# NJUVISION/PCGCv2

Hardware: AMD Instinct MI355X
Metric: encode+decode Mpoints/sec at fixed bpp (r3 ckpt), vox10 frame (higher is better)
Workload: dtype f32

## Files before the change

### include/pcgc_hip.h

```cpp
#ifndef PCGC_HIP_H
#define PCGC_HIP_H

#include <stddef.h>
#include <stdint.h>

#ifdef __cplusplus
extern "C" {
#endif

const char* pcgc_last_error(void);
int pcgc_version(void);

int64_t pcgc_hash_capacity(int64_t n);
int pcgc_hash_clear(uint64_t* keys , int32_t* vals , int64_t cap, void* stream);
int pcgc_hash_insert(const int32_t* coords , int64_t n, int32_t stride, uint64_t* keys, int32_t* vals,
                     int64_t cap, void* stream);
int pcgc_hash_insert_policy(const int32_t* coords, int64_t n, int32_t stride, uint64_t* keys, int32_t* vals, int64_t cap,
                            int keep_last, void* stream);
int pcgc_hash_first_mask(const int32_t* coords, int64_t n, int32_t stride, const uint64_t* keys, const int32_t* vals,
                         int64_t cap, uint8_t* keep , int32_t* first_row , void* stream);

int pcgc_coords_check_order(const int32_t* coords , int64_t n, int32_t* out2 , void* stream);

int pcgc_coords_quantize(const int32_t* coords, int64_t n, int32_t stride_out, int32_t* out , void* stream);
// ... 17 lines not shown
int pcgc_kmap_k3_prune(const int32_t* cand_nbr , int64_t n_cand, const uint8_t* mask, const int32_t* prefix,
                       const int32_t* orig , int64_t n_out, int32_t* nbr , void* stream);
int pcgc_kmap_k3_prune_parent(const int32_t* parent_nbr , int64_t n_parent, const uint8_t* mask,
                              const int32_t* prefix, const int32_t* orig, int64_t n_out, int32_t* nbr , void* stream);
int pcgc_kmap_k3_from_coarse(const int32_t* fine , int64_t n_fine, int32_t stride_fine,
                             const int32_t* parent_of , const int32_t* coarse_nbr ,
                             const int32_t* down , int64_t n_coarse, int32_t* nbr ,
                             void* stream);
int pcgc_down_maps(const int32_t* fine, const int32_t* first_row, const int32_t* prefix, int64_t n_fine, int32_t stride_fine,
                   int64_t n_coarse, int32_t* parent_of , int32_t* down , void* stream);
int pcgc_down_prepare(const int32_t* fine , int64_t n, int32_t stride_fine, int32_t* q ,
                      uint64_t* keys, int32_t* vals, int64_t cap, uint8_t* keep , int32_t* first_row ,
                      int32_t* prefix , int32_t* total , void* scan_ws, size_t scan_ws_bytes, void* stream);
int pcgc_down_finish(const int32_t* fine, const int32_t* q, const uint8_t* keep, const int32_t* first_row, const int32_t* prefix,
                     int64_t n, int32_t stride_fine, int64_t n_coarse, int32_t* coarse ,
                     int32_t* parent_of , int32_t* down , void* stream);
int pcgc_down_level(const int32_t* fine , int64_t n, int32_t stride_fine, int32_t* q, uint64_t* keys, int32_t* vals,
                    int64_t cap, uint8_t* keep, int32_t* first_row, int32_t* prefix, int32_t* total, void* scan_ws,
                    size_t scan_ws_bytes, int32_t* coarse , int32_t* parent_of ,
                    int32_t* down , int64_t* n_coarse_out , void* stream);
size_t pcgc_pyramid_scratch_bytes(int64_t n, int levels);
int pcgc_pyramid(const int32_t* fine , int64_t n, int32_t stride, int levels, void* scratch, size_t scratch_bytes,
                 int32_t* const* coarse, int32_t* const* parent_of, int32_t* const* down, int64_t* counts , void* stream);
int pcgc_compact_index(const uint8_t* mask, const int32_t* prefix, int64_t n, int32_t* orig , void* stream);

int pcgc_conv_gather(const int32_t* nbr, int K, int64_t n_out, const float* in, int64_t n_in , int Cin,
                     int in_ld, int in_coff, const float* W, const float* bias, const float* residual, int res_ld,
                     int res_coff, int relu, float* out, int Cout, int out_ld, int out_coff, void* stream);
int pcgc_last_conv_impl(void);
int pcgc_conv_gather_unit(const int32_t* nbr , int K, int64_t n_out, const float* W, const float* bias, int relu,
                          float* out, int Cout, int out_ld, void* stream);
int pcgc_conv_unit_from_coarse(const int32_t* fine , int64_t n_fine, int32_t stride_fine, const int32_t* parent_of,
                               const int32_t* coarse_nbr , const int32_t* down , int64_t n_coarse,
                               const float* W , const float* bias, int relu, float* out, int Cout, int out_ld, void* stream);
int pcgc_set_conv_impl(int impl);
int pcgc_set_up2_impl(int mfma);
int pcgc_irn_block(const int32_t* nbr , int64_t n, const float* x , int C, int x_ld,
                   const float* const* params, float* t_scratch, float* out, int out_ld, void* stream);
int pcgc_irn_pass(const int32_t* nbr, int64_t n, const float* x, int C, int x_ld, const float* const* params,
                  float* t_scratch, float* out, int out_ld, int pass, void* stream);
int pcgc_conv_up2(int64_t n_in, const float* in, int Cin, int in_ld, const float* W , const float* bias,
                  int relu, float* out , int Cout, void* stream);
int pcgc_conv_up2_gather(int64_t n_in, const float* in, int Cin, int in_ld, const int32_t* rows, const float* W ,
                         const float* bias, int relu, float* out , int Cout, void* stream);

int pcgc_conv_child(const int32_t* parent_nbr , int64_t n_parent, const float* in ,
                    int Cin, int in_ld, const float* table , int64_t table_bytes,
                    const float* bias, const float* residual, int res_ld, int relu, float* out, int Cout, int out_ld, void* stream);
int pcgc_irn_child_pass(const int32_t* parent_nbr, int64_t n_parent, int C, int pass, const float* in, int in_ld,
                        const float* table, int64_t table_bytes, const float* b0, const float* b1, const float* b2,
                        const float* x, int x_ld, float* out, int out_ld, void* stream);
int pcgc_irn_child_q4(const int32_t* parent_nbr, int64_t n_parent, int C, int pass, const float* in, int in_ld,
                      const float* table, int64_t table_bytes, const float* b0, const float* b1, const float* b2,
                      const float* x, int x_ld, float* out, int out_ld, void* stream);
int pcgc_cls_child_q4(const int32_t* parent_nbr, int64_t n_parent, const float* in, int Cin, int in_ld, const float* table,
                      int64_t table_bytes, const float* bias, float* out, void* stream);
int pcgc_irn_rows_pass(const int32_t* nbr, int64_t n, int C, int pass, const float* in, int in_ld, const float* table,
                       int64_t table_bytes, const float* b0, const float* b1, const float* b2, const float* x, int x_ld, float* out,
                       int out_ld, void* stream);
int pcgc_irn_rows_q4_pass(const int32_t* nbr, int64_t n, int C, int pass, const float* in, int in_ld, const float* table,
                          int64_t table_bytes, const float* b0, const float* b1, const float* b2, const float* x, int x_ld, float* out,
                          int out_ld, void* stream);
int pcgc_set_rows_q4_variant(int v);
int pcgc_conv_rows(const int32_t* nbr, int64_t n, const float* in, int Cin, int in_ld, const float* table, int64_t table_bytes,
                   const float* bias, const float* residual, int res_ld, int relu, float* out, int Cout, int out_ld, void* stream);
int pcgc_conv_down_rows(const int32_t* down, int64_t n_coarse, const float* in, int64_t n_in, int Cin, int in_ld, const float* table,
                        int64_t table_bytes, const float* bias, int relu, float* out, int Cout, int out_ld, void* stream);

int pcgc_conv_packed64(const int32_t* nbr, int64_t n, const float* in, int in_ld, const float* table, int64_t table_bytes,
                       const float* bias, int relu, float* out, int out_ld, void* stream);
int pcgc_set_packed_tuning(int rows, int waves);

int pcgc_set_convention(int what, int value);

size_t pcgc_topk_workspace_bytes(int64_t n);
int pcgc_topk_mask(const float* logits , int ld, int64_t n, int64_t k, uint8_t* mask ,
                   void* workspace, size_t workspace_bytes, void* stream);
int pcgc_topk_mask_segments(const float* logits, int ld, int nseg, const int64_t* seg_rows, const int64_t* seg_k, uint8_t* mask,
                            void* workspace, size_t workspace_bytes, void* stream);
size_t pcgc_topk_select_workspace_bytes(int64_t n);
int pcgc_topk_select(const float* logits , int ld, int nseg, const int64_t* seg_rows, const int64_t* seg_k,
                     const int32_t* coords, const int32_t* parent_coords, int32_t parent_stride,
                     uint8_t* bits, int32_t* wprefix, int32_t* orig, int32_t* out_coords, void* workspace, size_t workspace_bytes, void* stream);
int pcgc_kmap_k3_prune_sel(const int32_t* cand_nbr , int64_t n_cand, const uint8_t* bits, const int32_t* wprefix,
                           const int32_t* orig , int64_t n_out, int32_t* nbr , void* stream);
int pcgc_kmap_k3_prune_parent_sel(const int32_t* parent_nbr , int64_t n_parent, const uint8_t* bits, const int32_t* wprefix,
                                  const int32_t* orig, int64_t n_out, int32_t* nbr , void* stream);
int pcgc_gather_rows_f32_ld(const float* in, int C, int in_ld, const int32_t* orig, int64_t n_out, float* out , void* stream);
int pcgc_batch_counts(const int32_t* coords , int64_t n, int32_t* counts , void* stream);

size_t pcgc_sort_workspace_bytes(int64_t n);
int pcgc_sort_zyx(const int32_t* coords, int64_t n, int32_t* perm , void* workspace, size_t workspace_bytes,
                  void* stream);
int pcgc_sort_bzyx(const int32_t* coords, int64_t n, int32_t* perm , void* workspace, size_t workspace_bytes, void* stream);
int pcgc_gather_rows_i32x4(const int32_t* in, const int32_t* perm, int64_t n, int32_t* out, void* stream);
int pcgc_gather_rows_f32(const float* in, int C, const int32_t* perm, int64_t n, float* out, void* stream);

int pcgc_relu(const float* in, int64_t count, float* out, void* stream);
int pcgc_add(const float* a, const float* b, int64_t count, float* out, void* stream);

int pcgc_round_minmax(const float* feats, int64_t count, float* minmax , void* stream);
int pcgc_symbolize(const float* feats, int64_t count, float min_v, int16_t* sym , void* stream);
int pcgc_desymbolize(const int16_t* sym, int64_t count, float min_v, float* feats, void* stream);
int pcgc_quantize_symbols(const float* feats, int64_t count, float* minmax , int16_t* sym , void* stream);
int pcgc_quantize_symbols_segments(const float* feats, int C, int nseg, const int64_t* seg_rows, float* minmax, int16_t* sym, void* stream);
int pcgc_cdf_table(const float* params , int C, float min_v, float max_v, uint16_t* cdf_u16 ,
                   float* cdf_f32 , void* stream);


size_t pcgc_loss_workspace_bytes(int64_t elements);
int pcgc_hash_contains(const int32_t* coords , int64_t n, const uint64_t* keys, const int32_t* vals, int64_t cap,
                       const uint8_t* or_mask , uint8_t* mask , void* stream);
int pcgc_eb_likelihood(const float* feats, int ld, int64_t n, int C, const float* params , float bound, float* likelihood,
                       double* bits, void* workspace, size_t workspace_bytes, void* stream);
int pcgc_neg_log2_sum(const float* x, int ld, int64_t n, int C, double* bits , void* workspace, size_t workspace_bytes, void* stream);
int pcgc_bce_logits(const float* logits, int64_t ld, int64_t n, const uint8_t* truth , const uint8_t* pred ,
                    double* bce, int64_t* counts, void* workspace, size_t workspace_bytes, void* stream);

size_t pcgc_conv_wgrad_workspace_bytes(int K, int64_t n_rows, int Cin, int Cout);
int64_t pcgc_conv_wgrad_rows_per_group(int K, int64_t n_rows, int Cin, int Cout);
int pcgc_conv_wgrad(const int32_t* nbr, int K, int64_t n_out, const float* x, int64_t n_in, int Cin, int x_ld, const float* gy, int Cout,
                    int gy_ld, float* gW, float* gb, void* workspace, size_t workspace_bytes, void* stream);
int pcgc_conv_up2_wgrad(int64_t n_in, const float* x, int64_t x_rows, int Cin, int x_ld, const int32_t* rows, const float* gy, int Cout,
                        int gy_ld, float* gW, float* gb, void* workspace, size_t workspace_bytes, void* stream);
int pcgc_kmap_invert(const int32_t* nbr, int K, int64_t n_out, int64_t n_in, int32_t* inv , void* stream);
int pcgc_relu_bwd(const float* g, int g_ld, const float* y, int y_ld, int64_t n, int C, float* out, int out_ld, void* stream);
int pcgc_scatter_rows(const float* gy, int C, int gy_ld, const int32_t* orig, int64_t n_rows, float* gx, int64_t n_out, int gx_ld, void* stream);
int pcgc_bce_logits_bwd(const float* logits, int64_t ld, int64_t n, const uint8_t* truth, double scale, float* g , void* stream);
size_t pcgc_eb_bwd_workspace_bytes(int64_t n, int C);
int pcgc_eb_likelihood_bwd(const float* feats, int ld, int64_t n, int C, const float* params , float bound, double scale,
                           float* gy, float* gparams, void* workspace, size_t workspace_bytes, void* stream);

int64_t pcgc_rc_encode(const uint16_t* cdf , int C, int Lp, const int16_t* sym , int64_t n,
                       uint8_t* out , int64_t cap);
int pcgc_rc_decode(const uint16_t* cdf, int C, int Lp, const uint8_t* in, int64_t nbytes, int16_t* sym, int64_t n);
#define PCGC_RC_CKPT_WORDS 6
int64_t pcgc_rc_encode_indexed(const uint16_t* cdf, int C, int Lp, const int16_t* sym, int64_t n, uint8_t* out, int64_t cap, int n_ckpt,
                               uint32_t* ckpt );
int pcgc_rc_decode_indexed(const uint16_t* cdf, int C, int Lp, const uint8_t* in, int64_t nbytes, int16_t* sym, int64_t n, int n_ckpt,
                           const uint32_t* ckpt);
int pcgc_set_rc_threads(int threads);
int pcgc_set_rc_lanes(int mode);
int pcgc_set_rc_impl(int impl);

int64_t pcgc_oct_encode(const int32_t* xyz , int64_t n, uint8_t* out, int64_t cap);
int64_t pcgc_oct_decode_count(const uint8_t* in, int64_t nbytes);
int pcgc_oct_decode(const uint8_t* in, int64_t nbytes, int32_t* xyz , int64_t n);
int pcgc_set_oct_tiled(int on);
int pcgc_set_oct_model(int model);
int pcgc_oct_warm(void);

int pcgc_d1_nn(const int32_t* a , int64_t na, const uint64_t* b_keys, const int32_t* b_vals, int64_t b_cap,
               const int32_t* offsets , int n_offsets, double* sum , uint64_t* max_d2 ,
               int32_t* unresolved , void* stream);
int pcgc_d1_cell_masks(const int32_t* b , int64_t nb, const uint64_t* cell_keys, const int32_t* cell_vals, int64_t cell_cap,
                       uint64_t* masks , int64_t n_cells, void* stream);
int pcgc_d1_nn_cells(const int32_t* a , int64_t na, const uint64_t* cell_keys, const int32_t* cell_vals, int64_t cell_cap,
                     const uint64_t* masks, const int32_t* offsets , int n_offsets, int32_t reach2, double* sum, uint64_t* max_d2,
                     int32_t* unresolved, void* stream);

int pcgc_d2_runs(const int32_t* qs , int64_t nq, int32_t* runlen , void* stream);
int pcgc_d2_count(const int32_t* p , int64_t n, const int32_t* sel, const uint64_t* cell_keys, const int32_t* cell_vals,
                  int64_t cell_cap, const uint64_t* masks, const uint64_t* keys, const int32_t* vals, int64_t cap, const int32_t* runlen,
                  const int32_t* offsets , int n_offsets, int32_t reach2, int64_t* best , int32_t* cnt ,
                  int32_t* unresolved , int32_t* n_unresolved , void* stream);
int pcgc_d2_fill(const int32_t* p, int64_t n, const int32_t* sel, const uint64_t* cell_keys, const int32_t* cell_vals, int64_t cell_cap,
// ... 90 lines not shown
```

### pcgcv2_amd/_build.py

```python
import os
import subprocess
import sys
from concurrent.futures import ThreadPoolExecutor

HERE = os.path.dirname(os.path.abspath(__file__))
CSRC = os.path.join(HERE, 'csrc')
VARIANT = os.environ.get('PCGC_BUILD_VARIANT', '')
OBJ = os.path.join(CSRC, '_obj' + ('_' + VARIANT if VARIANT else ''))
LIB = os.path.join(HERE, 'libpcgc_hip' + ('_' + VARIANT if VARIANT else '') + '.so')
SOURCES = ['coords.hip', 'select.hip', 'conv.hip', 'child_conv.hip', 'child_conv32.hip', 'child_cls_w.hip', 'child_irn.hip', 'child_irn_a16.hip', 'child_irn_b16.hip',
           'child_irn_a32.hip', 'child_irn_b32.hip', 'child_q4.hip', 'rows_irn.hip', 'rows_q4.hip', 'conv_packed.hip', 'entropy.hip', 'loss.hip', 'grad.hip', 'metric.hip', 'colour.hip', 'normals.hip', 'mesh.hip', 'collate.hip', 'hostcodec.cpp', 'ply.cpp', 'mesh_io.cpp']
HEADERS = [os.path.join(CSRC, 'pcgc_common.h'), os.path.join(CSRC, 'mfma_util.h'), os.path.join(CSRC, 'child_kernels.h'), os.path.join(CSRC, 'child_q4.h'), os.path.join(CSRC, 'q4x.h'), os.path.join(CSRC, 'q4x_sched.h'), os.path.join(CSRC, 'rows_q4_policy.h'), os.path.join(CSRC, 'eb_logits.h'), os.path.join(HERE, '..', 'include', 'pcgc_hip.h')]
FLAGS = ['--offload-arch=gfx950', '-O3', '-std=c++17', '-ffp-contract=off', '-fPIC', '-Wall', '-Wno-unused-result'] + \
        os.environ.get('PCGC_EXTRA_HIPCC_FLAGS', '').split()


def _hipcc():
    for c in (os.environ.get('HIPCC'), '/opt/rocm/bin/hipcc', 'hipcc'):
        if c and (os.path.isabs(c) and os.path.exists(c) or not os.path.isabs(c)):
            return c
    return 'hipcc'


def _stale(target, deps):
    if not os.path.exists(target):
        return True
    t = os.path.getmtime(target)
    return any(os.path.getmtime(d) > t for d in deps)


def build(force=False, verbose=False):
    os.makedirs(OBJ, exist_ok=True)
    if VARIANT:
        import shutil
        base = os.path.join(CSRC, '_obj')
        for src in SOURCES:
            o = src.rsplit('.', 1)[0] + '.o'
            if 'child_kernels.h' not in open(os.path.join(CSRC, src)).read() and os.path.exists(os.path.join(base, o)) \
                    and not os.path.exists(os.path.join(OBJ, o)):
                shutil.copy2(os.path.join(base, o), os.path.join(OBJ, o))
    hipcc = _hipcc()
    jobs = []
    only = [t for t in os.environ.get('PCGC_BUILD_ONLY', '').split(',') if t]
    for src in SOURCES:
        s = os.path.join(CSRC, src)
        o = os.path.join(OBJ, src.rsplit('.', 1)[0] + '.o')
        if only and os.path.exists(o):
            if src.rsplit('.', 1)[0] in only:
                jobs.append((o, [hipcc] + FLAGS + (['-x', 'hip'] if src.endswith('.hip') else []) + ['-c', s, '-o', o]))
            continue
        if force or _stale(o, [s] + HEADERS):
            lang = ['-x', 'hip'] if src.endswith('.hip') else []
            jobs.append((o, [hipcc] + FLAGS + lang + ['-c', s, '-o', o]))

    def run(job):
        o, cmd = job
        if verbose:
            print(' '.join(cmd), file=sys.stderr)
        r = subprocess.run(cmd, capture_output=True, text=True)
        if r.returncode != 0:
            raise RuntimeError('hipcc failed:\n' + ' '.join(cmd) + '\n' + r.stderr[-4000:])
        return o

    with ThreadPoolExecutor(max_workers=max(2, min(8, os.cpu_count() or 4))) as ex:
        list(ex.map(run, jobs))
    objs = [os.path.join(OBJ, s.rsplit('.', 1)[0] + '.o') for s in SOURCES]
    if force or jobs or _stale(LIB, objs):
        cmd = [hipcc, '--offload-arch=gfx950', '-shared', '-fPIC', '-o', LIB] + objs + ['-lz']
        r = subprocess.run(cmd, capture_output=True, text=True)
        if r.returncode != 0:
            raise RuntimeError('link failed:\n' + r.stderr[-4000:])
    if not VARIANT:
        build_reftable(force=force)
    return LIB


REFTABLE_LIB = os.path.join(HERE, 'libpcgc_reftable.so')


def build_reftable(force=False):
    src = os.path.join(CSRC, 'reftable.cpp')
    if not (force or _stale(REFTABLE_LIB, [src])):
        return REFTABLE_LIB
    import torch
    tdir = os.path.dirname(torch.__file__)
    cmd = ['g++', '-O2', '-std=c++17', '-fPIC', '-shared', f'-D_GLIBCXX_USE_CXX11_ABI={int(torch._C._GLIBCXX_USE_CXX11_ABI)}',
           '-I' + os.path.join(tdir, 'include'), '-I' + os.path.join(tdir, 'include', 'torch', 'csrc', 'api', 'include'), src,
           '-o', REFTABLE_LIB, '-L' + os.path.join(tdir, 'lib'), '-ltorch_cpu', '-lc10', '-Wl,-rpath,' + os.path.join(tdir, 'lib')]
    r = subprocess.run(cmd, capture_output=True, text=True)
    if r.returncode != 0:
        raise RuntimeError('g++ failed:\n' + ' '.join(cmd) + '\n' + r.stderr[-4000:])
    return REFTABLE_LIB


if __name__ == '__main__':
# ... 2 lines not shown
```

### pcgcv2_amd/_lib.py

```python
import ctypes as C
import os

_HERE = os.path.dirname(os.path.abspath(__file__))
LIB_PATH = os.environ.get('PCGC_LIB') or os.path.join(_HERE, 'libpcgc_hip.so')

vp, i64, i32, f32, sz = C.c_void_p, C.c_int64, C.c_int32, C.c_float, C.c_size_t
ci = C.c_int

SIGNATURES = {
    'pcgc_last_error': (C.c_char_p, []),
    'pcgc_version': (ci, []),
    'pcgc_hash_capacity': (i64, [i64]),
    'pcgc_hash_clear': (ci, [vp, vp, i64, vp]),
    'pcgc_hash_insert': (ci, [vp, i64, i32, vp, vp, i64, vp]),
    'pcgc_hash_insert_policy': (ci, [vp, i64, i32, vp, vp, i64, ci, vp]),
    'pcgc_set_convention': (ci, [ci, ci]),
    'pcgc_hash_first_mask': (ci, [vp, i64, i32, vp, vp, i64, vp, vp, vp]),
    'pcgc_coords_check_order': (ci, [vp, i64, vp, vp]),
    'pcgc_coords_quantize': (ci, [vp, i64, i32, vp, vp]),
    'pcgc_coords_children': (ci, [vp, i64, i32, vp, vp]),
    'pcgc_coords_scale': (ci, [vp, i64, f32, vp, vp]),
    'pcgc_scan_workspace_bytes': (sz, [i64]),
    'pcgc_mask_scan': (ci, [vp, i64, vp, vp, vp, sz, vp]),
    'pcgc_mask_scan_zeroed': (ci, [vp, i64, vp, vp, vp, sz, vp]),
    'pcgc_compact_coords': (ci, [vp, vp, vp, i64, vp, vp]),
    'pcgc_compact_feats': (ci, [vp, ci, ci, vp, vp, i64, vp, vp]),
    'pcgc_kmap_k3': (ci, [vp, i64, i32, vp, vp, i64, vp, vp]),
    'pcgc_kmap_k3_children': (ci, [vp, i64, vp, vp]),
    'pcgc_kmap_k3_prune': (ci, [vp, i64, vp, vp, vp, i64, vp, vp]),
    'pcgc_kmap_k3_prune_parent': (ci, [vp, i64, vp, vp, vp, i64, vp, vp]),
    'pcgc_kmap_k3_from_coarse': (ci, [vp, i64, i32, vp, vp, vp, i64, vp, vp]),
    'pcgc_down_maps': (ci, [vp, vp, vp, i64, i32, i64, vp, vp, vp]),
    'pcgc_down_prepare': (ci, [vp, i64, i32, vp, vp, vp, i64, vp, vp, vp, vp, vp, sz, vp]),
    'pcgc_down_finish': (ci, [vp, vp, vp, vp, vp, i64, i32, i64, vp, vp, vp, vp]),
    'pcgc_down_level': (ci, [vp, i64, i32, vp, vp, vp, i64, vp, vp, vp, vp, vp, sz, vp, vp, vp, vp, vp]),
    'pcgc_pyramid_scratch_bytes': (sz, [i64, ci]),
    'pcgc_pyramid': (ci, [vp, i64, i32, ci, vp, sz, vp, vp, vp, vp, vp]),
    'pcgc_compact_index': (ci, [vp, vp, i64, vp, vp]),
    'pcgc_conv_gather': (ci, [vp, ci, i64, vp, i64, ci, ci, ci, vp, vp, vp, ci, ci, ci, vp, ci, ci, ci, vp]),
    'pcgc_conv_gather_unit': (ci, [vp, ci, i64, vp, vp, ci, vp, ci, ci, vp]),
    'pcgc_conv_unit_from_coarse': (ci, [vp, i64, i32, vp, vp, vp, i64, vp, vp, ci, vp, ci, ci, vp]),
    'pcgc_set_conv_impl': (ci, [ci]),
    'pcgc_last_conv_impl': (ci, []),
    'pcgc_set_up2_impl': (ci, [ci]),
    'pcgc_irn_block': (ci, [vp, i64, vp, ci, ci, vp, vp, vp, ci, vp]),
    'pcgc_irn_pass': (ci, [vp, i64, vp, ci, ci, vp, vp, vp, ci, ci, vp]),
    'pcgc_conv_child': (ci, [vp, i64, vp, ci, ci, vp, i64, vp, vp, ci, ci, vp, ci, ci, vp]),
    'pcgc_irn_child_pass': (ci, [vp, i64, ci, ci, vp, ci, vp, i64, vp, vp, vp, vp, ci, vp, ci, vp]),
    'pcgc_irn_child_q4': (ci, [vp, i64, ci, ci, vp, ci, vp, i64, vp, vp, vp, vp, ci, vp, ci, vp]),
    'pcgc_cls_child_q4': (ci, [vp, i64, vp, ci, ci, vp, i64, vp, vp, vp]),
    'pcgc_conv_down_rows': (ci, [vp, i64, vp, i64, ci, ci, vp, i64, vp, ci, vp, ci, ci, vp]),
    'pcgc_conv_rows': (ci, [vp, i64, vp, ci, ci, vp, i64, vp, vp, ci, ci, vp, ci, ci, vp]),
    'pcgc_irn_rows_pass': (ci, [vp, i64, ci, ci, vp, ci, vp, i64, vp, vp, vp, vp, ci, vp, ci, vp]),
    'pcgc_irn_rows_q4_pass': (ci, [vp, i64, ci, ci, vp, ci, vp, i64, vp, vp, vp, vp, ci, vp, ci, vp]),
    'pcgc_set_rows_q4_variant': (ci, [ci]),
    'pcgc_conv_packed64': (ci, [vp, i64, vp, ci, vp, i64, vp, ci, vp, ci, vp]),
    'pcgc_set_packed_tuning': (ci, [ci, ci]),
    'pcgc_conv_up2': (ci, [i64, vp, ci, ci, vp, vp, ci, vp, ci, vp]),
    'pcgc_conv_up2_gather': (ci, [i64, vp, ci, ci, vp, vp, vp, ci, vp, ci, vp]),
    'pcgc_topk_workspace_bytes': (sz, [i64]),
    'pcgc_topk_mask': (ci, [vp, ci, i64, i64, vp, vp, sz, vp]),
    'pcgc_topk_mask_segments': (ci, [vp, ci, ci, vp, vp, vp, vp, sz, vp]),
    'pcgc_topk_select_workspace_bytes': (sz, [i64]),
    'pcgc_topk_select': (ci, [vp, ci, ci, vp, vp, vp, vp, i32, vp, vp, vp, vp, vp, sz, vp]),
    'pcgc_kmap_k3_prune_sel': (ci, [vp, i64, vp, vp, vp, i64, vp, vp]),
    'pcgc_kmap_k3_prune_parent_sel': (ci, [vp, i64, vp, vp, vp, i64, vp, vp]),
    'pcgc_gather_rows_f32_ld': (ci, [vp, ci, ci, vp, i64, vp, vp]),
    'pcgc_batch_counts': (ci, [vp, i64, vp, vp]),
    'pcgc_sort_bzyx': (ci, [vp, i64, vp, vp, sz, vp]),
    'pcgc_quantize_symbols_segments': (ci, [vp, ci, ci, vp, vp, vp, vp]),
    'pcgc_sort_workspace_bytes': (sz, [i64]),
    'pcgc_sort_zyx': (ci, [vp, i64, vp, vp, sz, vp]),
    'pcgc_gather_rows_i32x4': (ci, [vp, vp, i64, vp, vp]),
    'pcgc_gather_rows_f32': (ci, [vp, ci, vp, i64, vp, vp]),
    'pcgc_relu': (ci, [vp, i64, vp, vp]),
    'pcgc_add': (ci, [vp, vp, i64, vp, vp]),
    'pcgc_round_minmax': (ci, [vp, i64, vp, vp]),
    'pcgc_symbolize': (ci, [vp, i64, f32, vp, vp]),
    'pcgc_desymbolize': (ci, [vp, i64, f32, vp, vp]),
    'pcgc_quantize_symbols': (ci, [vp, i64, vp, vp, vp]),
    'pcgc_cdf_table': (ci, [vp, ci, f32, f32, vp, vp, vp]),
    'pcgc_loss_workspace_bytes': (sz, [i64]),
    'pcgc_hash_contains': (ci, [vp, i64, vp, vp, i64, vp, vp, vp]),
    'pcgc_eb_likelihood': (ci, [vp, ci, i64, ci, vp, f32, vp, vp, vp, sz, vp]),
    'pcgc_neg_log2_sum': (ci, [vp, ci, i64, ci, vp, vp, sz, vp]),
    'pcgc_bce_logits': (ci, [vp, i64, i64, vp, vp, vp, vp, vp, sz, vp]),
    'pcgc_conv_wgrad_workspace_bytes': (sz, [ci, i64, ci, ci]),
    'pcgc_conv_wgrad_rows_per_group': (i64, [ci, i64, ci, ci]),
    'pcgc_conv_wgrad': (ci, [vp, ci, i64, vp, i64, ci, ci, vp, ci, ci, vp, vp, vp, sz, vp]),
    'pcgc_conv_up2_wgrad': (ci, [i64, vp, i64, ci, ci, vp, vp, ci, ci, vp, vp, vp, sz, vp]),
    'pcgc_kmap_invert': (ci, [vp, ci, i64, i64, vp, vp]),
    'pcgc_relu_bwd': (ci, [vp, ci, vp, ci, i64, ci, vp, ci, vp]),
    'pcgc_scatter_rows': (ci, [vp, ci, ci, vp, i64, vp, i64, ci, vp]),
    'pcgc_bce_logits_bwd': (ci, [vp, i64, i64, vp, C.c_double, vp, vp]),
    'pcgc_eb_bwd_workspace_bytes': (sz, [i64, ci]),
    'pcgc_eb_likelihood_bwd': (ci, [vp, ci, i64, ci, vp, f32, C.c_double, vp, vp, vp, sz, vp]),
    'pcgc_d1_cell_masks': (ci, [vp, i64, vp, vp, i64, vp, i64, vp]),
    'pcgc_d1_nn_cells': (ci, [vp, i64, vp, vp, i64, vp, vp, ci, i32, vp, vp, vp, vp]),
    'pcgc_d1_nn': (ci, [vp, i64, vp, vp, i64, vp, ci, vp, vp, vp, vp]),
    'pcgc_d2_runs': (ci, [vp, i64, vp, vp]),
    'pcgc_d2_count': (ci, [vp, i64, vp, vp, vp, i64, vp, vp, vp, i64, vp, vp, ci, i32, vp, vp, vp, vp, vp]),
    'pcgc_d2_fill': (ci, [vp, i64, vp, vp, vp, i64, vp, vp, vp, i64, vp, vp, vp, ci, i32, vp, vp, vp, vp]),
    'pcgc_d2_exhaustive': (ci, [vp, i64, vp, vp, i64, vp, ci, vp, vp, vp, vp, vp, vp]),
    'pcgc_d2_scan_workspace_bytes': (sz, [i64]),
    'pcgc_d2_scan': (ci, [vp, i64, vp, vp, sz, vp]),
    'pcgc_d2_segment_lowest': (ci, [vp, i64, vp, i32, vp, vp]),
    'pcgc_d2_recv_count': (ci, [vp, vp, i64, vp, i64, vp, vp]),
    'pcgc_d2_recv_fill': (ci, [vp, vp, i64, vp, i64, vp, vp, vp, vp]),
    'pcgc_d2_normals': (ci, [vp, vp, i64, vp, vp, vp, vp, vp, vp]),
    'pcgc_d2_c2p': (ci, [vp, i64, vp, vp, vp, vp, vp, vp, vp]),
    'pcgc_d2_reduce_workspace_bytes': (sz, []),
    'pcgc_d2_reduce': (ci, [vp, vp, i64, vp, vp, vp, sz, vp]),
    'pcgc_attr_transfer_workspace_bytes': (sz, [i64, i64, ci]),
    'pcgc_attr_transfer': (ci, [vp, vp, vp, i64, vp, vp, vp, i64, vp, ci, vp, vp, sz, vp]),
    'pcgc_colour_dist': (ci, [vp, i64, vp, i64, vp, vp, vp, vp, vp, vp]),
    'pcgc_colour_reduce_workspace_bytes': (sz, []),
    'pcgc_colour_reduce': (ci, [vp, vp, i64, vp, vp, sz, vp]),
    'pcgc_normals_ball_masks': (i64, [i32, vp]),
    'pcgc_normals_workspace_bytes': (sz, [i64]),
    'pcgc_normals_estimate': (ci, [vp, i64, vp, vp, vp, vp, i64, vp, vp, vp, i64, vp, vp, i32, ci, vp, vp, vp, vp, vp, vp, vp, sz, vp]),
    'pcgc_set_normals_mapping': (ci, [ci]),
    'pcgc_rc_encode': (i64, [vp, ci, ci, vp, i64, vp, i64]),
    'pcgc_rc_decode': (ci, [vp, ci, ci, vp, i64, vp, i64]),
    'pcgc_set_rc_impl': (ci, [ci]),
    'pcgc_rc_encode_indexed': (i64, [vp, ci, ci, vp, i64, vp, i64, ci, vp]),
    'pcgc_rc_decode_indexed': (ci, [vp, ci, ci, vp, i64, vp, i64, ci, vp]),
    'pcgc_set_rc_threads': (ci, [ci]),
    'pcgc_set_rc_lanes': (ci, [ci]),
    'pcgc_set_oct_tiled': (ci, [ci]),
    'pcgc_set_oct_model': (ci, [ci]),
    'pcgc_oct_warm': (ci, []),
    'pcgc_oct_encode': (i64, [vp, i64, vp, i64]),
    'pcgc_oct_decode_count': (i64, [vp, i64]),
    'pcgc_oct_decode': (ci, [vp, i64, vp, i64]),
    'pcgc_items_encode': (ci, [ci, vp, vp, vp, vp, vp, ci, vp, vp, vp, ci, ci, ci]),
    'pcgc_items_probe': (ci, [ci, vp, vp, vp, vp, vp, vp]),
    'pcgc_items_decode': (ci, [ci, vp, vp, ci, vp, vp, vp, vp, ci, vp, vp, ci, ci, ci]),
    'pcgc_level_prepare_children': (ci, [vp, i64, i32, vp, vp, i64, vp, vp, vp, vp]),
    'pcgc_frame_decode': (ci, [C.c_char_p, ci, vp, vp, ci, ci, i64, vp, vp, vp, vp, ci]),
    'pcgc_frame_decode_begin': (ci, [C.c_char_p, ci, vp, vp, ci, ci, i64, vp, vp, vp, vp, ci]),
    'pcgc_frame_decode_end': (ci, []),
    'pcgc_frame_worker_test': (ci, [ci]),
    'pcgc_table_cache': (ci, [ci]),
    'pcgc_crc32': (C.c_uint32, [C.c_uint32, vp, i64]),
    'pcgc_ply_read_ascii_geo': (i64, [C.c_char_p, vp, i64]),
    'pcgc_ply_write_ascii_geo': (ci, [C.c_char_p, vp, i64]),
    'pcgc_ply_write_ascii_geo_rgb': (ci, [C.c_char_p, vp, vp, i64]),
# ... 58 lines not shown
```

### pcgcv2_amd/autoencoder.py

```python
import torch

from . import dispatch, ops
from .nn import MinkowskiConvolution as Conv, MinkowskiGenerativeConvolutionTranspose as UpConv, MinkowskiPruning
from .sparse import CoordMap, SparseTensor


class InceptionResNet(torch.nn.Module):

    def __init__(self, channels):
        super().__init__()
        c = channels
        self.conv0_0 = Conv(c, c // 4, 3)
        self.conv0_1 = Conv(c // 4, c // 2, 3)
        self.conv1_0 = Conv(c, c // 4, 1)
        self.conv1_1 = Conv(c // 4, c // 4, 3)
        self.conv1_2 = Conv(c // 4, c // 2, 1)

    def forward(self, x):
        c = x.F.shape[1]
        children = x.cmap.origin is not None and x.cmap.origin[0] == 'children'
        fam = dispatch.select('irn', (c,), x.F.shape[0], 'children' if children else 'plain', extent=x.F.shape[0] * max(c, x.F.stride(0)) * 4,
                              contiguous=x.F.is_contiguous()).family
        if fam != 'unfused':
            params = [p for m in (self.conv0_0, self.conv0_1, self.conv1_0, self.conv1_1, self.conv1_2) for p in (m.kernel, m.bias)]
            if fam == 'rows64':
                y = ops.irn_block_rows64(x.cmap.k3, x.F, params, self._tables('child', ops.child_irn_tables, params))
            elif fam == 'child':
                big = x.F.shape[0] >= 8 * ops.PATH.CHILD_Q4_MIN_PARENTS
                q4 = self._tables('q4', ops.child_q4_tables, params) if (c == 16 and ops.PATH.CHILD_Q4 and big) else None
                y = ops.irn_block_child(x.cmap.origin[1].k3, x.F, params, self._tables('child', ops.child_irn_tables, params), q4_table=q4)
            elif fam == 'rows32q4':
                y = ops.irn_block_rows32_q4(x.cmap.k3, x.F, params, self._tables('rows_q4', ops.rows_q4_tables, params))
            elif fam == 'rows32':
                y = ops.irn_block_rows32(x.cmap.k3, x.F, params, self._tables('rows32', ops.rows_irn32_tables, params))
            else:
                y = ops.irn_block(x.cmap.k3, x.F, params)
            return SparseTensor(y, coordinate_map=x.cmap)
        out = torch.empty_like(x.F)
        a = self.conv0_0(x, relu=True)
        self.conv0_1(a, out=out[:, :c // 2], residual=x.F[:, :c // 2])
        b = self.conv1_1(self.conv1_0(x, relu=True), relu=True)
        self.conv1_2(b, out=out[:, c // 2:], residual=x.F[:, c // 2:])
        return SparseTensor(out, coordinate_map=x.cmap)

    def _tables(self, kind, build, params):
        stamp = tuple((p.data_ptr(), p._version) for p in params)
        cache = self.__dict__.setdefault('_derived', {})
        if cache.get(kind, (None, None))[0] != stamp:
            cache[kind] = (stamp, build(params))
        return cache[kind][1]


def make_layer(block, block_layers, channels):
    return torch.nn.Sequential(*[block(channels=channels) for _ in range(block_layers)])


class Encoder(torch.nn.Module):

    def __init__(self, channels=[1, 16, 32, 64, 32, 8]):
        super().__init__()
        ch = channels
        self.conv0 = Conv(ch[0], ch[1], 3)
        self.down0 = Conv(ch[1], ch[2], 2, 2)
        self.block0 = make_layer(InceptionResNet, 3, ch[2])
        self.conv1 = Conv(ch[2], ch[2], 3)
        self.down1 = Conv(ch[2], ch[3], 2, 2)
        self.block1 = make_layer(InceptionResNet, 3, ch[3])
        self.conv2 = Conv(ch[3], ch[3], 3)
        self.down2 = Conv(ch[3], ch[4], 2, 2)
        self.block2 = make_layer(InceptionResNet, 3, ch[4])
        self.conv3 = Conv(ch[4], ch[5], 3)

    def forward(self, x):
        out0 = self.block0(self.down0(self.conv0(x, relu=True), relu=True))
        out1 = self.block1(self.down1(self.conv1(out0, relu=True), relu=True))
        out2 = self.block2(self.down2(self.conv2(out1, relu=True), relu=True))
        out2 = self.conv3(out2)
        return [out2, out1, out0]


class Decoder(torch.nn.Module):

    def __init__(self, channels=[8, 64, 32, 16]):
        super().__init__()
        ch = channels
        for l in range(3):
            setattr(self, f'up{l}', UpConv(ch[l], ch[l + 1], 2, 2))
            setattr(self, f'conv{l}', Conv(ch[l + 1], ch[l + 1], 3))
            setattr(self, f'block{l}', make_layer(InceptionResNet, 3, ch[l + 1]))
            setattr(self, f'conv{l}_cls', Conv(ch[l + 1], 1, 3))
        self.pruning = MinkowskiPruning()

    def prune_voxel(self, data, data_cls, nums, ground_truth=None, training=False):
        if training:
            return self._prune_voxel_training(data, data_cls, nums, ground_truth)
        cand = data.cmap
        rows = [len(data_cls)] if len(nums) == 1 else cand.batch_rows
        if len(rows) != len(nums):
            raise ValueError(f'prune_voxel: {len(nums)} budgets for a batch of {len(rows)} items')
        keep = [int(min(r, max(int(n), 0))) for r, n in zip(rows, nums)]
        if dispatch.select('prune', (data.F.shape[1],), len(data_cls)).family != 'select':
            mask = ops.topk_mask(data_cls.F, keep[0]) if len(nums) == 1 else ops.topk_mask_segments(data_cls.F, rows, keep)
            return self.pruning(data, mask, n_keep=sum(keep), keep_per_item=None if len(nums) == 1 else keep)
        if cand._C is None and cand.origin is not None and cand.origin[0] == 'children':
            parent = cand.origin[1]
            bits, wprefix, orig, coords = ops.topk_select(data_cls.F, rows, keep, parent_coords=parent.C, parent_stride=parent.stride)
        else:
            bits, wprefix, orig, coords = ops.topk_select(data_cls.F, rows, keep, coords=cand.C)
        cmap = CoordMap(coords, cand.stride, unique=True, origin=('selected', cand, bits, wprefix, orig))
        if len(nums) > 1:
            cmap._batch_rows = list(keep)
        src = data.F
        out = SparseTensor(lambda: ops.gather_rows(src, orig), coordinate_map=cmap)
        out._F_rows = (src, orig)
        return out

    def _prune_voxel_training(self, data, data_cls, nums, ground_truth):
        if ground_truth is None:
            raise ValueError('prune_voxel(training=True) needs the ground truth of the level')
        from .data_utils import isin_mask
        cand = data.cmap
        rows = [len(data_cls)] if len(nums) == 1 else cand.batch_rows
        if len(rows) != len(nums):
            raise ValueError(f'prune_voxel: {len(nums)} budgets for a batch of {len(rows)} items')
        keep = [int(min(r, max(int(n), 0))) for r, n in zip(rows, nums)]
        topk = ops.topk_mask(data_cls.F, keep[0]) if len(nums) == 1 else ops.topk_mask_segments(data_cls.F, rows, keep)
        mask = isin_mask(cand.C, ground_truth, or_mask=topk)
        return self.pruning(data, mask)

    def forward(self, x, nums_list, ground_truth_list=(None, None, None), training=False):
        out, cls_list = x, []
        for l in range(3):
            out = getattr(self, f'up{l}')(out, relu=True)
            out = getattr(self, f'conv{l}')(out, relu=True)
            out = getattr(self, f'block{l}')(out)
            cls = getattr(self, f'conv{l}_cls')(out)
            cls_list.append(cls)
            out = self.prune_voxel(out, cls, nums_list[l], ground_truth_list[l], training)
        return cls_list, out
```

### pcgcv2_amd/csrc/child_cls_w.hip

```cpp
#include "child_kernels.h"

#define DEF_CONV_LAUNCH(NAME) int NAME(const int32_t* parent_nbr, int64_t n_parent, const float* in, int in_ld, const float* table, \
                                       int table_bytes, const ChildEpi& ep, hipStream_t s)
DEF_CONV_LAUNCH(pcgc_child_cls32) { return launch_child_cls<2, 16, 4>(parent_nbr, n_parent, in, in_ld, table, table_bytes, ep, s); }
DEF_CONV_LAUNCH(pcgc_child_cls64) { return launch_child_cls<4, 7, 4>(parent_nbr, n_parent, in, in_ld, table, table_bytes, ep, s); }
CHILD_TIMING_READER(pcgc_child_timing_cls_w)
```

### pcgcv2_amd/csrc/child_conv.hip

```cpp
#include "child_kernels.h"


#define DECL_CONV_LAUNCH(NAME) int NAME(const int32_t* parent_nbr, int64_t n_parent, const float* in, int in_ld, const float* table, \
                                        int table_bytes, const ChildEpi& ep, hipStream_t s)
DECL_CONV_LAUNCH(pcgc_child_conv32); DECL_CONV_LAUNCH(pcgc_child_cls32); DECL_CONV_LAUNCH(pcgc_child_cls64);


extern "C" int pcgc_conv_child(const int32_t* parent_nbr, int64_t n_parent, const float* in, int Cin, int in_ld,
                               const float* table, int64_t table_bytes, const float* bias,
                               const float* residual, int res_ld, int relu, float* out, int Cout, int out_ld, void* stream) {
    CHILD_COMMON_CHECKS(in_ld)
    PCGC_REQUIRE(out != nullptr, "null output");
    PCGC_REQUIRE(Cout == 1 || ((out_ld & 3) == 0 && (((uintptr_t)out) & 15) == 0), "output rows must be 16-byte aligned");
    PCGC_REQUIRE(residual == nullptr, "conv_child: no residual form");
    (void)res_ld;
    hipStream_t s = S(stream);
    int rc = -2;
    const int tb = (int)table_bytes;
    if (Cout == 1 && (Cin == 16 || Cin == 32 || Cin == 64)) {
        PCGC_REQUIRE(table_bytes == (int64_t)(125 * ((Cin / 16) * 64 + 16) + 1023) / 1024 * 1024, "cls table size");
        PCGC_REQUIRE(residual == nullptr && !relu, "cls head has no fused epilogue");
        ChildEpi ep{bias, nullptr, 0, 0, out, out_ld, 0};
        if (Cin == 64) rc = pcgc_child_cls64(parent_nbr, n_parent, in, in_ld, table, tb, ep, s);
        else if (Cin == 16) rc = launch_child_cls<1, 8, 4>(parent_nbr, n_parent, in, in_ld, table, tb, ep, s);
        else rc = pcgc_child_cls32(parent_nbr, n_parent, in, in_ld, table, tb, ep, s);
    } else {
        PCGC_REQUIRE(table_bytes == (int64_t)27 * Cin * Cout * 4, "table size");
        ChildEpi ep{bias, nullptr, 0, relu, out, out_ld, Cout / 16};
        if (Cin == 16 && Cout == 16) {
            rc = launch_child_conv<1, 1, 4, 4>(parent_nbr, n_parent, in, in_ld, table, tb, ep, s);
        } else if (Cin == 32 && Cout == 32) {
            rc = pcgc_child_conv32(parent_nbr, n_parent, in, in_ld, table, tb, ep, s);
        } else {
            pcgc_set_error("conv_child: unsupported shape %d -> %d (16->16, 32->32, 16->1, 32->1, 64->1)", Cin, Cout);
            return -2;
        }
    }
    if (rc) return rc;
    PCGC_CHECK_LAUNCH("conv_child");
    return 0;
}


#ifdef PCGC_CHILD_TIMING
extern "C" int pcgc_child_timing(unsigned long long* out8, int reset) {
    hipDeviceSynchronize();
    if (out8) hipMemcpyFromSymbol(out8, HIP_SYMBOL(g_child_dbg), 8 * sizeof(unsigned long long));
    if (reset) { unsigned long long z[8] = {0}; hipMemcpyToSymbol(HIP_SYMBOL(g_child_dbg), z, sizeof(z)); }
    return 0;
}
#endif
```

### pcgcv2_amd/csrc/child_kernels.h

```cpp
#pragma once
#include "pcgc_common.h"
#include "mfma_util.h"
#include <type_traits>

#ifdef PCGC_CHILD_TIMING
static __device__ unsigned long long g_child_dbg[8];
#define CHILD_T(var) const unsigned long long var = __builtin_amdgcn_s_memtime()
#define CHILD_TADD(slot, a, b) do { child_dbg[slot] += (b) - (a); } while (0)
#define CHILD_DBG_DECL unsigned long long child_dbg[8] = {0, 0, 0, 0, 0, 0, 0, 0};
#define CHILD_DBG_PARAM , unsigned long long (&child_dbg)[8]
#define CHILD_DBG_ARG , child_dbg
#define CHILD_TFLUSH do { if ((threadIdx.x & 63) == 0) { for (int q_ = 0; q_ < 8; ++q_) if (child_dbg[q_]) atomicAdd(&g_child_dbg[q_], child_dbg[q_]); } } while (0)
#define CHILD_TIMING_READER(NAME)                                                                                      \
    extern "C" int NAME(unsigned long long* out8, int reset) {                                                         \
        (void)hipDeviceSynchronize();                                                                                  \
        if (out8) (void)hipMemcpyFromSymbol(out8, HIP_SYMBOL(g_child_dbg), 8 * sizeof(unsigned long long));           \
        if (reset) { unsigned long long z[8] = {0}; (void)hipMemcpyToSymbol(HIP_SYMBOL(g_child_dbg), z, sizeof(z)); }  \
        return 0;                                                                                                      \
    }
#else
#define CHILD_T(var)
#define CHILD_TADD(slot, a, b)
#define CHILD_DBG_DECL
#define CHILD_DBG_PARAM
#define CHILD_DBG_ARG
#define CHILD_TFLUSH
#define CHILD_TIMING_READER(NAME)
#endif

struct ChildEpi {
    const float* bias;
    const float* res;
    int res_ld;
    int relu;
    float* out;
    int out_ld;
    int nt;
};
struct IrnEpi {
    const float* b0;
    const float* b1;
    const float* b2;
    const float* x;
    int x_ld;
    float* out;
    int out_ld;
};
namespace {


constexpr int halo_p1(int c) { return c == 0 ? 0 : (c == 3 ? 2 : 1); }
constexpr int halo_bit(int c) { return (c == 0 || c == 2) ? 1 : 0; }
constexpr int cell_kp(int c) { return halo_p1(c >> 4) * 9 + halo_p1((c >> 2) & 3) * 3 + halo_p1(c & 3); }
constexpr int cell_child(int c) { return halo_bit(c & 3) + 2 * halo_bit((c >> 2) & 3) + 4 * halo_bit(c >> 4); }
constexpr bool axis_reach(int c, int jb) { return c - jb >= 0 && c - jb <= 2; }
constexpr unsigned cell_reach(int c) {
    unsigned m = 0;
    for (int j = 0; j < 8; ++j)
        if (axis_reach(c & 3, j & 1) && axis_reach((c >> 2) & 3, (j >> 1) & 1) && axis_reach(c >> 4, j >> 2)) m |= 1u << j;
    return m;
}
constexpr int cell_k(int c, int j) {
    return ((c >> 4) - (j >> 2)) * 9 + (((c >> 2) & 3) - ((j >> 1) & 1)) * 3 + ((c & 3) - (j & 1));
}
constexpr int cz_of(int c) { return c >> 4; }
constexpr int cy_of(int c) { return (c >> 2) & 3; }
constexpr int cx_of(int c) { return c & 3; }
constexpr bool in02(int v) { return v >= 0 && v <= 2; }

struct HaloGeometry {
    static constexpr int NCELLS = 64, ROW_MUL = 8, NMAP = 27;
    static constexpr int kp(int c) { return cell_kp(c); }
    static constexpr int child(int c) { return cell_child(c); }
    static constexpr int byte_off(int) { return 0; }
};

template <int NB_, int NT, int HZ = -1>
struct PlainConv : HaloGeometry {
    static constexpr int NB = NB_, ROWCHUNKS = 4, T = 8 * NT, KS = 4;
    static constexpr int Z_HALF = HZ;
    static constexpr bool HALF = false;
    static constexpr int kfirst(int) { return 0; }
    static constexpr bool active(int c, int t) { return (HZ < 0 || (((t / NT) >> 2) & 1) == HZ) && ((cell_reach(c) >> (t / NT)) & 1); }
    static constexpr int frag(int c, int t) { return cell_k(c, t / NT) * NT + t % NT; }
    static constexpr bool uses_block(int, int) { return true; }
// ... 366 lines not shown
        if (res) {
            const float4 x = *(const float4*)(res + row * res_ld + 4 * c4);
            v.x = v.x + x.x; v.y = v.y + x.y; v.z = v.z + x.z; v.w = v.w + x.w;
        }
        if (relu) { v.x = fmaxf(v.x, 0.0f); v.y = fmaxf(v.y, 0.0f); v.z = fmaxf(v.z, 0.0f); v.w = fmaxf(v.w, 0.0f); }
        *(float4*)(out + row * out_ld + 4 * c4) = v;
    }
}

#define CHILD_IN_ROWS(V, n_p) (V::ROW_MUL * (n_p))
#define CHILD_KERNEL_PROLOGUE(V, NW, D, RING_FLOAT4)                                                                          \
    CHILD_DBG_DECL                                                                                                            \
    extern __shared__ __attribute__((aligned(16))) unsigned char lds_raw[];                                                   \
    const int lane = threadIdx.x & 63, mi = lane & 15, mq = lane >> 4;                                                        \
    const int wave = __builtin_amdgcn_readfirstlane(threadIdx.x >> 6);                                                        \
    float4* ring = (float4*)(lds_raw + table_bytes) + wave * (RING_FLOAT4);                                                   \
    child_stage_table<NW>(table, table_bytes, lds_raw);                                                                        \
    const __amdgpu_buffer_rsrc_t rs_in = __builtin_amdgcn_make_buffer_rsrc((void*)in, 0, (int)(CHILD_IN_ROWS(V, n_p) * in_ld * 4), 0x00020000); \
    const int64_t ntiles = (n_p + 15) >> 4;

template <class T_> struct child_type_tag { using type = T_; };
template <int NB, int NT, int NW, int D, bool SPLIT = false, int MT = 1, bool RES = false>
__global__ void __launch_bounds__(NW * 64)
k_child_conv(const int32_t* __restrict__ pnbr, int64_t n_p, const float* __restrict__ in, int in_ld,
             const float* __restrict__ table, int table_bytes, ChildEpi ep) {
    using V = PlainConv<NB, NT>;
    CHILD_KERNEL_PROLOGUE(V, NW, D, D * NB * 64 * MT)
    float bvs[NT];
#pragma unroll
    for (int n = 0; n < NT; ++n) bvs[n] = ep.bias ? ep.bias[16 * n + mi] : 0.0f;
    auto unit = [&](auto tag, const int64_t pu) {
        using VV = typename decltype(tag)::type;
        constexpr int HZ = VV::Z_HALF;
        f32x4 acc[MT][VV::T];
        child_tile_mainloop_mt<VV, D, MT>(pnbr, n_p, pu, rs_in, in_ld, lds_raw, ring, acc CHILD_DBG_ARG);
        constexpr int W = 16 * NT, CH = (64 * W * 4 <= D * NB * 1024 * MT) ? 64 : 32, PPC = CH / 8, MQC = PPC / 4;
        float* scratch = (float*)ring;
#pragma unroll
        for (int m = 0; m < MT; ++m) {
            const int64_t p0 = pu + 16 * m;
            if (m > 0 && p0 >= n_p) break;
#pragma unroll
            for (int h = 0; h < 128 / CH; ++h) {
                ChildResidual<W, RES ? CH : 1> rr;
                if constexpr (RES) child_flush_prefetch<W, CH>(rr, 8 * p0 + h * CH, 8 * n_p, ep.res, ep.res_ld, lane, HZ);
                if (mq / MQC == h) {
#pragma unroll
                    for (int t = 0; t < VV::T; ++t) {
                        const int j = t / NT, n = t % NT;
                        if (HZ >= 0 && ((j >> 2) & 1) != HZ) continue;
#pragma unroll
                        for (int r = 0; r < 4; ++r) {
                            float v = acc[m][t][r];
                            if (ep.bias) v = v + bvs[n];
                            scratch[(8 * (4 * (mq % MQC) + r) + j) * W + 16 * n + mi] = v;
                        }
                    }
                }
                wave_lds_sync();
                if constexpr (RES) child_flush<W, CH>(scratch, rr, true, 8 * p0 + h * CH, 8 * n_p, ep.out, ep.out_ld, ep.relu, lane, HZ);
                else child_flush<W, CH>(scratch, 8 * p0 + h * CH, 8 * n_p, ep.out, ep.out_ld, ep.relu, lane, HZ);
                wave_lds_sync();
            }
        }
    };
    const int64_t nunits = (SPLIT ? 2 : 1) * ((n_p + 16 * MT - 1) / (16 * MT));
    for (int i = 0;; ++i) {
        const int64_t u = child_tile<NW>(i, wave, nunits);
        if (u < 0) break;
        CHILD_T(t_it0);
        if constexpr (SPLIT) {
            if (u & 1) unit(child_type_tag<PlainConv<NB, NT, 1>>{}, (u >> 1) * (16 * MT));
            else unit(child_type_tag<PlainConv<NB, NT, 0>>{}, (u >> 1) * (16 * MT));
        } else {
            unit(child_type_tag<V>{}, u * (16 * MT));
        }
#ifdef PCGC_CHILD_TIMING
        { CHILD_T(t_dr0); asm volatile("s_waitcnt vmcnt(0)" ::: "memory"); CHILD_T(t_it1); CHILD_TADD(5, t_dr0, t_it1); CHILD_TADD(4, t_it0, t_it1); }
#endif
    }
    CHILD_TFLUSH;
}

template <int NB, int NW, int D, int MT = 1>
__global__ void __launch_bounds__(NW * 64)
k_child_cls(const int32_t* __restrict__ pnbr, int64_t n_p, const float* __restrict__ in, int in_ld,
            const float* __restrict__ table, int table_bytes, ChildEpi ep) {
    using V = ClsHead<NB>;
    CHILD_KERNEL_PROLOGUE(V, NW, D, D * NB * 64 * MT)
    const float bv = ep.bias ? ep.bias[0] : 0.0f;
    const int64_t nunits = (n_p + 16 * MT - 1) / (16 * MT);
    for (int i = 0;; ++i) {
        const int64_t tile = child_tile<NW>(i, wave, nunits);
        if (tile < 0) break;
        const int64_t pu = tile * (16 * MT);
        CHILD_T(t_it0);
        f32x4 acc[MT][1];
        child_tile_mainloop_mt<V, D, MT>(pnbr, n_p, pu, rs_in, in_ld, lds_raw, ring, acc CHILD_DBG_ARG);
        if (mi < 8) {
#pragma unroll
            for (int m = 0; m < MT; ++m) {
#pragma unroll
                for (int r = 0; r < 4; ++r) {
                    const int64_t p = pu + 16 * m + 4 * mq + r;
                    if (p >= n_p) continue;
                    float v = acc[m][0][r];
                    if (ep.bias) v = v + bv;
                    ep.out[(8 * p + mi) * ep.out_ld] = v;
                }
            }
        }
#ifdef PCGC_CHILD_TIMING
        { CHILD_T(t_dr0); asm volatile("s_waitcnt vmcnt(0)" ::: "memory"); CHILD_T(t_it1); CHILD_TADD(5, t_dr0, t_it1); CHILD_TADD(4, t_it0, t_it1); }
#endif
    }
    CHILD_TFLUSH;
}



template <int C, int NW, int D, bool SPLIT = false, int MT = 1>
__global__ void __launch_bounds__(NW * 64)
k_child_irn_a(const int32_t* __restrict__ pnbr, int64_t n_p, const float* __restrict__ in, int in_ld,
              const float* __restrict__ table, int table_bytes, IrnEpi ep) {
    using V = PassA<C>;
    constexpr int Q = V::Q, CPT = V::CPT, TH = V::TH;
    static_assert(!SPLIT || CPT <= 2, "half units: tiles of one or two children");
    CHILD_KERNEL_PROLOGUE(V, NW, D, D * V::NB * 64 * MT)
    const int co = mi % Q, sub = mi / Q;
    const float b00 = ep.b0[co], b10 = ep.b1[co];
    auto unit = [&](auto tag, const int64_t pu) {
        using VV = typename decltype(tag)::type;
        constexpr int HZ = VV::Z_HALF;
        f32x4 acc[MT][VV::T];
        child_tile_mainloop_mt<VV, D, MT>(pnbr, n_p, pu, rs_in, in_ld, lds_raw, ring, acc CHILD_DBG_ARG);
        constexpr int W = 2 * Q, CH = (64 * W * 4 <= D * V::NB * 1024 * MT) ? 64 : 32, MQC = CH / 32;
        float* scratch = (float*)ring;
#pragma unroll
        for (int m = 0; m < MT; ++m) {
            const int64_t p0 = pu + 16 * m;
            if (m > 0 && p0 >= n_p) break;
#pragma unroll
            for (int h = 0; h < 128 / CH; ++h) {
                if (mq / MQC == h) {
#pragma unroll
                    for (int t = 0; t < TH; ++t) {
                        if (HZ >= 0 && (((t * CPT) >> 2) & 1) != HZ) continue;
                        const int j = t * CPT + sub;
#pragma unroll
                        for (int r = 0; r < 4; ++r) {
                            float* y = scratch + (8 * (4 * (mq % MQC) + r) + j) * W;
                            y[co] = fmaxf(acc[m][t][r] + b00, 0.0f);
                            y[Q + co] = fmaxf(acc[m][TH + t][r] + b10, 0.0f);
                        }
                    }
                }
                wave_lds_sync();
                child_flush<W, CH>(scratch, 8 * p0 + h * CH, 8 * n_p, ep.out, W, 0, lane, HZ);
                wave_lds_sync();
            }
        }
    };
    const int64_t nunits = (SPLIT ? 2 : 1) * ((n_p + 16 * MT - 1) / (16 * MT));
    for (int i = 0;; ++i) {
        const int64_t u = child_tile<NW>(i, wave, nunits);
        if (u < 0) break;
        CHILD_T(t_it0);
        if constexpr (SPLIT) {
            if (u & 1) unit(child_type_tag<PassA<C, 1>>{}, (u >> 1) * (16 * MT));
            else unit(child_type_tag<PassA<C, 0>>{}, (u >> 1) * (16 * MT));
        } else {
            unit(child_type_tag<V>{}, u * (16 * MT));
        }
#ifdef PCGC_CHILD_TIMING
        { CHILD_T(t_dr0); asm volatile("s_waitcnt vmcnt(0)" ::: "memory"); CHILD_T(t_it1); CHILD_TADD(5, t_dr0, t_it1); CHILD_TADD(4, t_it0, t_it1); }
#endif
    }
    CHILD_TFLUSH;
}

template <int C, int NW, int D, bool SPLIT = false, int MT = 1, bool T2 = false>
__global__ void __launch_bounds__(NW * 64)
k_child_irn_b(const int32_t* __restrict__ pnbr, int64_t n_p, const float* __restrict__ in , int in_ld,
              const float* __restrict__ table, int table_bytes, IrnEpi ep) {
    using V = PassB<C, -1, T2>;
    constexpr int Q = V::Q, H = 2 * Q, KQ = Q / 4, T0 = V::T0, T1 = V::T1, CPT0 = V::CPT0, CPT1 = V::CPT1;
    constexpr int CH = ((128 * Q + 64 * C) * 4 <= D * 1024 * MT) ? 64 : 32, MQC = CH / 32;
    constexpr int NEEDF4 = (128 * Q + CH * C) / 4;
    constexpr int RINGF4 = (D * 64 * MT > NEEDF4) ? D * 64 * MT : NEEDF4;
    CHILD_KERNEL_PROLOGUE(V, NW, D, RINGF4)
    float* us = (float*)ring;
    float* stage = us + 128 * Q;
    float w12[KQ];
#pragma unroll
    for (int jj = 0; jj < KQ; ++jj) w12[jj] = ((const float*)lds_raw)[V::FRAG_W12 * frag_floats<V>() + lane * KQ + jj];
    const int c1 = mi % Q, sub1 = mi / Q, c0 = mi % H, sub0 = mi / H;
    const float b11 = ep.b1[c1], b01 = ep.b0[c0], b12 = mi < H ? ep.b2[mi] : 0.0f;
    auto unit = [&](auto tag, const int64_t pu) {
// ... 44 lines not shown
                if (mi < H) {
#pragma unroll
                    for (int gg = 0; gg < CH / 16; ++gg)
#pragma unroll
                        for (int r = 0; r < 4; ++r) stage[(16 * gg + 4 * mq + r) * C + H + mi] = d[gg][r] + b12;
                }
                wave_lds_sync();
                child_flush<C, CH>(stage, rr, ep.x != nullptr, 8 * p0 + h * CH, 8 * n_p, ep.out, ep.out_ld, 0, lane, HZ);
                wave_lds_sync();
            }
        }
        }
    };
    const int64_t nunits = (SPLIT ? 2 : 1) * ((n_p + 16 * MT - 1) / (16 * MT));
    for (int i = 0;; ++i) {
        const int64_t u = child_tile<NW>(i, wave, nunits);
        if (u < 0) break;
        CHILD_T(t_it0);
        if constexpr (SPLIT) {
            if (u & 1) unit(child_type_tag<PassB<C, 1, T2>>{}, (u >> 1) * (16 * MT));
            else unit(child_type_tag<PassB<C, 0, T2>>{}, (u >> 1) * (16 * MT));
        } else {
            unit(child_type_tag<V>{}, u * (16 * MT));
        }
#ifdef PCGC_CHILD_TIMING
        { CHILD_T(t_dr0); asm volatile("s_waitcnt vmcnt(0)" ::: "memory"); CHILD_T(t_it1); CHILD_TADD(5, t_dr0, t_it1); CHILD_TADD(4, t_it0, t_it1); }
#endif
    }
    CHILD_TFLUSH;
}

struct ChildLdsGrant { size_t bytes[16] = {0}; };
template <typename K>
int child_lds_limit(K kern, size_t lds, ChildLdsGrant& granted) {
    if (lds > 160 * 1024) { pcgc_set_error("child kernel: %zu bytes of LDS needed", lds); return -2; }
    int dev = 0;
    (void)hipGetDevice(&dev);
    size_t& g = granted.bytes[dev & 15];
    if (lds > 48 * 1024 && lds > g) {
        hipError_t e = hipFuncSetAttribute((const void*)kern, hipFuncAttributeMaxDynamicSharedMemorySize, (int)lds);
        if (e != hipSuccess) { pcgc_set_error("child kernel: cannot raise the LDS limit to %zu: %s", lds, hipGetErrorString(e)); return -1; }
        g = lds;
    }
    return 0;
}
static unsigned child_grid_units(int64_t n_units, int nw, size_t lds, int max_waves_per_cu = 16) {
    static int cus = 0;
    if (!cus) { hipDeviceProp_t p; int dev = 0; (void)hipGetDevice(&dev); cus = (hipGetDeviceProperties(&p, dev) == hipSuccess && p.multiProcessorCount > 0) ? p.multiProcessorCount : 256; }
    int per_cu = (int)((160 * 1024) / (lds ? lds : 1));
    if (per_cu > max_waves_per_cu / nw) per_cu = max_waves_per_cu / nw;
    if (per_cu < 1) per_cu = 1;
    int64_t want = (n_units + nw - 1) / nw;
    int64_t g = (int64_t)cus * per_cu;
    if (g > want) g = want;
    g = (g + 7) / 8 * 8;
    return (unsigned)g;
}
static unsigned child_grid(int64_t n_p, int nw, size_t lds, int units_per_tile = 1) {
    return child_grid_units(((n_p + 15) / 16) * units_per_tile, nw, lds);
}
#define CHILD_LAUNCH_EX(KERN, NW, RINGBYTES, EP, MT_, UPT)                                                                     \
    do {                                                                                                                       \
        const size_t lds = (size_t)table_bytes + (size_t)(NW) * (RINGBYTES);                                                   \
        auto kern = KERN;                                                                                                      \
        static ChildLdsGrant granted;                                                                                          \
        if (int rc = child_lds_limit(kern, lds, granted)) return rc;                                                           \
        const int64_t units = ((n_p + 16 * (MT_) - 1) / (16 * (MT_))) * (UPT);                                                 \
        hipLaunchKernelGGL(kern, dim3(child_grid_units(units, NW, lds)), dim3((NW) * 64), lds, s, pnbr, n_p, in, in_ld, table, table_bytes, EP); \
        return 0;                                                                                                              \
    } while (0)
#define CHILD_LAUNCH(KERN, NW, RINGBYTES, EP) CHILD_LAUNCH_EX(KERN, NW, RINGBYTES, EP, 1, 1)
#define CHILD_LAUNCH_SPLIT(KERN, NW, RINGBYTES, EP) CHILD_LAUNCH_EX(KERN, NW, RINGBYTES, EP, 1, 2)

template <int NB, int NT, int NW, int D, int MT = 1>
int launch_child_conv(const int32_t* pnbr, int64_t n_p, const float* in, int in_ld, const float* table, int table_bytes,
                      const ChildEpi& ep, hipStream_t s) {
    CHILD_LAUNCH_EX((k_child_conv<NB, NT, NW, D, false, MT, false>), NW, D * NB * 1024 * MT, ep, MT, 1);
}
template <int NB, int NT, int NW, int D>
int launch_child_conv_split(const int32_t* pnbr, int64_t n_p, const float* in, int in_ld, const float* table, int table_bytes,
                            const ChildEpi& ep, hipStream_t s) {
    CHILD_LAUNCH_EX((k_child_conv<NB, NT, NW, D, true, 1, false>), NW, D * NB * 1024, ep, 1, 2);
}
template <int NB, int NW, int D, int MT = 1, int WPC = 16>
int launch_child_cls(const int32_t* pnbr, int64_t n_p, const float* in, int in_ld, const float* table, int table_bytes,
                     const ChildEpi& ep, hipStream_t s) {
    const size_t lds = (size_t)table_bytes + (size_t)NW * (D * NB * 1024 * MT);
    auto kern = k_child_cls<NB, NW, D, MT>;
    static ChildLdsGrant granted;
    if (int rc = child_lds_limit(kern, lds, granted)) return rc;
    const int64_t units = (n_p + 16 * MT - 1) / (16 * MT);
    hipLaunchKernelGGL(kern, dim3(child_grid_units(units, NW, lds, WPC)), dim3(NW * 64), lds, s, pnbr, n_p, in, in_ld, table, table_bytes, ep);
    return 0;
}
template <int C, int NW, int D, int MT = 1>
int launch_child_irn_a(const int32_t* pnbr, int64_t n_p, const float* in, int in_ld, const float* table, int table_bytes,
                       const IrnEpi& ep, hipStream_t s) {
    CHILD_LAUNCH_EX((k_child_irn_a<C, NW, D, false, MT>), NW, D * (C / 16) * 1024 * MT, ep, MT, 1);
}
template <int C, int NW, int D>
int launch_child_irn_a_split(const int32_t* pnbr, int64_t n_p, const float* in, int in_ld, const float* table, int table_bytes,
                             const IrnEpi& ep, hipStream_t s) {
    CHILD_LAUNCH_SPLIT((k_child_irn_a<C, NW, D, true>), NW, D * (C / 16) * 1024, ep);
}
template <int C, int NW, int D, int MT = 1, bool T2 = false>
int launch_child_irn_b(const int32_t* pnbr, int64_t n_p, const float* in, int in_ld, const float* table, int table_bytes,
                       const IrnEpi& ep, hipStream_t s) {
    constexpr int Q = C / 4, CH = ((128 * Q + 64 * C) * 4 <= D * 1024 * MT) ? 64 : 32;
    constexpr int need = (128 * Q + CH * C) * 4;
    constexpr int ringb = (D * 1024 * MT > need) ? D * 1024 * MT : need;
    CHILD_LAUNCH_EX((k_child_irn_b<C, NW, D, false, MT, T2>), NW, ringb, ep, MT, 1);
}
template <int C, int NW, int D>
int launch_child_irn_b_split(const int32_t* pnbr, int64_t n_p, const float* in, int in_ld, const float* table, int table_bytes,
                             const IrnEpi& ep, hipStream_t s) {
    constexpr int Q = C / 4, CH = ((128 * Q + 64 * C) * 4 <= D * 1024) ? 64 : 32;
    constexpr int need = (128 * Q + CH * C) * 4;
    constexpr int ringb = (D * 1024 > need) ? D * 1024 : need;
    CHILD_LAUNCH_SPLIT((k_child_irn_b<C, NW, D, true>), NW, ringb, ep);
}

}

#define CHILD_COMMON_CHECKS(ROWS_LD)                                                                                           \
    PCGC_REQUIRE(parent_nbr && in && table, "null argument");                                                                  \
    PCGC_REQUIRE(((ROWS_LD) & 3) == 0 && (((uintptr_t)in | (uintptr_t)table) & 15) == 0, "unaligned input");                 \
    PCGC_REQUIRE(8 * n_parent * (int64_t)(ROWS_LD) * 4 < (int64_t)0xF0000000, "tensor too large for 32-bit buffer offsets"); \
    PCGC_REQUIRE(table_bytes % 16 == 0, "table size");                                                                         \
    if (n_parent == 0) return 0;
```

### pcgcv2_amd/csrc/child_q4.h

```cpp
#pragma once
#include "child_kernels.h"

namespace {

struct Q4Group {
    int cell, child, kind;
    int k;
    bool first, last;
    bool fin;
};
struct Q4Sched {
    int n;
    Q4Group g[232];
    int vm_wait[232];
    int pend[232];
};
constexpr int Q4_PASS_A = 0, Q4_CLS = 1;
template <int KIND, int MT, int D = 2>
constexpr Q4Sched q4_sched() {
    Q4Sched S{};
    for (int c = 0; c < 64; ++c) {
        const int n0 = S.n;
        if (KIND == Q4_CLS) {
            for (int h = 0; h < 2; ++h)
                if (in02(cz_of(c) - h)) { S.g[S.n] = Q4Group{c, h, 0, S.n, false, false, false}; S.n++; }
        } else {
            for (int j = 0; j < 8; ++j) {
                if (!((cell_reach(c) >> j) & 1)) continue;
                const int k = cell_k(c, j);
                S.g[S.n++] = Q4Group{c, j, 0, k, false, false, k == 26};
                if (k == 13) S.g[S.n++] = Q4Group{c, j, 1, 27, false, false, false};
            }
        }
        S.g[n0].first = true;
        S.g[S.n - 1].last = true;
    }
    int ops = 0, pending = 0;
    int gather_end[64 + 16] = {};
    for (int c = 0; c < D; ++c) { ops += 4 * MT; gather_end[c] = ops; }
    for (int n = 0; n < S.n; ++n) {
        const Q4Group& G = S.g[n];
        if (G.last && G.cell + 1 < 64) S.vm_wait[n] = ops - gather_end[G.cell + 1];
        if (G.first && G.cell + D < 64) { ops += 4 * MT; gather_end[G.cell + D] = ops; }
        S.pend[n] = pending;
        ops += pending;
        pending = (KIND == Q4_PASS_A && ((G.kind == 1) || G.fin) && (G.child & 3) == 3) ? 4 * MT : 0;
    }
    return S;
}

typedef unsigned u32x4 __attribute__((ext_vector_type(4)));
__device__ __forceinline__ void q4_store(const f32x4& v, const __amdgpu_buffer_rsrc_t& rs, unsigned voff) {
    u32x4 u = {__float_as_uint(v[0]), __float_as_uint(v[1]), __float_as_uint(v[2]), __float_as_uint(v[3])};
#ifndef Q4_STORE_AUX
#define Q4_STORE_AUX 0
#endif
    __builtin_amdgcn_raw_buffer_store_b128(u, rs, (int)voff, 0, Q4_STORE_AUX);
}

template <int KIND, int NW, int MT, int D = 2>
__global__ void __launch_bounds__(NW * 64)
k_child_q4(const int32_t* __restrict__ pnbr, int64_t n_p, const float* __restrict__ in, int in_ld,
           const float* __restrict__ table, int table_bytes, IrnEpi ep) {
    constexpr int TP = 64 * MT, SLOT_F4 = MT * 256;
    constexpr Q4Sched S = q4_sched<KIND, MT, D>();
    constexpr int NACC = KIND == Q4_CLS ? 2 : 8, OUT_ROW_BYTES = KIND == Q4_CLS ? 4 : 32;
    extern __shared__ __attribute__((aligned(16))) unsigned char lds_raw[];
    const int lane = threadIdx.x & 63;
    const int wave = __builtin_amdgcn_readfirstlane(threadIdx.x >> 6);
    float4* ring = (float4*)(lds_raw + table_bytes) + wave * (D * SLOT_F4);
    child_stage_table<NW>(table, table_bytes, lds_raw);
    const __amdgpu_buffer_rsrc_t rs_in = __builtin_amdgcn_make_buffer_rsrc((void*)in, 0, (int)(8 * n_p * in_ld * 4), 0x00020000);
    const __amdgpu_buffer_rsrc_t rs_out = __builtin_amdgcn_make_buffer_rsrc((void*)ep.out, 0, (int)(8 * n_p * OUT_ROW_BYTES), 0x00020000);
    const int co = lane & 3;
    float b00[4], b10[4];
#pragma unroll
    for (int r = 0; r < 4; ++r) { b00[r] = KIND == Q4_CLS ? (ep.b0 ? ep.b0[0] : 0.0f) : ep.b0[r]; b10[r] = KIND == Q4_CLS ? 0.0f : ep.b1[r]; }
    const unsigned tab_lane = (unsigned)(uintptr_t)(lds_void_ptr)((const float*)lds_raw + co * 16);
    const unsigned a_row = (unsigned)(uintptr_t)(lds_void_ptr)((const float*)ring + lane * 16 + (((lane >> 2) & 3) << 2));
    const unsigned row_bytes = (unsigned)in_ld * 4u;
    const unsigned lane_off = (unsigned)(((lane & 3) ^ ((lane >> 4) & 3)) * 16);
    constexpr unsigned ABSENT = 0xF0000000u;
    const int64_t ntiles = (n_p + TP - 1) / TP;

    for (int it = 0;; ++it) {
#ifdef Q4_EXP_TILE_ORDER
        int64_t tile;
        {
            const int64_t S = (ntiles + 7) >> 3;
            const int64_t l = ((int64_t)(blockIdx.x >> 3) + (int64_t)(gridDim.x >> 3) * it) * NW + wave;
            tile = (blockIdx.x & 7) * S + l;
            if (!(l < S && tile < ntiles)) tile = -1;
        }
#else
        const int64_t tile = child_tile<NW>(it, wave, ntiles);
#endif
        if (tile < 0) break;
        const int64_t p_base = tile * TP;
        unsigned rowb[MT][27];
        bool ok[MT];
#pragma unroll
        for (int m = 0; m < MT; ++m) {
            const int64_t rho = p_base + 64 * m + 16 * (lane & 3) + (lane >> 2);
            ok[m] = rho < n_p;
#pragma unroll
            for (int kp = 0; kp < 27; ++kp) rowb[m][kp] = (unsigned)pnbr[(int64_t)kp * n_p + (ok[m] ? rho : 0)];
        }
        asm volatile("s_waitcnt vmcnt(0)" ::: "memory");
#pragma unroll
        for (int m = 0; m < MT; ++m)
#pragma unroll
            for (int kp = 0; kp < 27; ++kp)
#ifdef Q4_KO_GATHER
                rowb[m][kp] = ((int)rowb[m][kp] == 0x7FFFFFF1) ? rowb[m][kp] * (8u * row_bytes) : ABSENT;
#else
                rowb[m][kp] = (ok[m] && (int)rowb[m][kp] >= 0) ? rowb[m][kp] * (8u * row_bytes) : ABSENT;
#endif
        auto ovq = [&](int m) { return (unsigned)((p_base + 64 * m + (lane & ~3)) * 256 + (lane & 3) * 16); };
#ifdef Q4_KO_STORE
        f32x4 sink = (f32x4){0.f, 0.f, 0.f, 0.f};
#endif

        f32x4 acc0[MT][NACC], c1[MT][KIND == Q4_CLS ? 1 : 4];
#pragma unroll
        for (int m = 0; m < MT; ++m)
#pragma unroll
            for (int j = 0; j < NACC; ++j) acc0[m][j] = (f32x4){0.f, 0.f, 0.f, 0.f};
        f32x4 a[MT][4], b[2][4];

        auto gather = [&](auto ic) {
            constexpr int c = decltype(ic)::value, kp = cell_kp(c), ch = cell_child(c), slot = c % D;
            const unsigned cell_off = (unsigned)ch * row_bytes + lane_off;
#pragma unroll
            for (int m = 0; m < MT; ++m) {
                const int rb = (int)rowb[m][kp];
                const unsigned v0 = (unsigned)__builtin_amdgcn_update_dpp(0, rb, 0x00, 0xF, 0xF, true) + cell_off;
                const unsigned v1 = (unsigned)__builtin_amdgcn_update_dpp(0, rb, 0x55, 0xF, 0xF, true) + cell_off;
                const unsigned v2 = (unsigned)__builtin_amdgcn_update_dpp(0, rb, 0xAA, 0xF, 0xF, true) + cell_off;
                const unsigned v3 = (unsigned)__builtin_amdgcn_update_dpp(0, rb, 0xFF, 0xF, 0xF, true) + cell_off;
                float4* dst = ring + slot * SLOT_F4 + m * 256;
                __builtin_amdgcn_raw_ptr_buffer_load_lds(rs_in, (lds_void_ptr)(dst), 16, (int)v0, 0, 0, 0);
                __builtin_amdgcn_raw_ptr_buffer_load_lds(rs_in, (lds_void_ptr)(dst + 64), 16, (int)v1, 0, 0, 0);
                __builtin_amdgcn_raw_ptr_buffer_load_lds(rs_in, (lds_void_ptr)(dst + 128), 16, (int)v2, 0, 0, 0);
                __builtin_amdgcn_raw_ptr_buffer_load_lds(rs_in, (lds_void_ptr)(dst + 192), 16, (int)v3, 0, 0, 0);
            }
            asm volatile("" ::: "memory");
        };
        auto load_a = [&](auto ic, auto ie) {
            constexpr int c = decltype(ic)::value, e = decltype(ie)::value, slot = c % D;
            static_for<0, MT>([&](auto im) {
                constexpr int m = decltype(im)::value;
                a[m][e] = lds_ld128_off<(slot * MT + m) * 4096>(a_row ^ (unsigned)(e << 4));
            });
// ... 32 lines not shown
                        }
                    }
#pragma unroll
                    for (int r = 0; r < 4; ++r) W[r] = (f32x4){0.f, 0.f, 0.f, 0.f};
#pragma unroll
                    for (int k = 0; k < 4; ++k)
#pragma unroll
                        for (int r = 0; r < 4; ++r) W[r] = __builtin_amdgcn_mfma_f32_4x4x1f32(V[k][r], onehot[k], W[r], 0, 0, 0);
#pragma unroll
                    for (int t = 0; t < 4; ++t) {
                        const f32x4 v = {W[0][t], W[1][t], W[2][t], W[3][t]};
#ifdef Q4_KO_STORE
                        sink = sink + v;
#else
                        q4_store(v, rs_out, ovq(m) + (unsigned)(t * 256 + h * 128 + (G.kind == 1 ? 64 : 0)));
#endif
                    }
                });
            }
        };

        using I0 = std::integral_constant<int, 0>;
        static_for<0, D>(gather);
        wait_vmcnt<4 * MT * (D - 1)>();
        load_b(I0{}, I0{});
        static_for<0, 4>([&](auto ie) { load_a(I0{}, ie); });

        static_for<0, S.n>([&](auto in_) {
            constexpr int n = decltype(in_)::value, cur = n & 1;
            constexpr Q4Group G = S.g[n];
            constexpr bool has_next = n + 1 < S.n, next_cell = G.cell + 1 < 64;
            if constexpr (G.first) wait_lgkmcnt<3 * MT>(); else wait_lgkmcnt<0>();
            static_for<0, 4>([&](auto ie) { lds_tie(b[cur][decltype(ie)::value]); });
            if constexpr (G.first) static_for<0, MT>([&](auto im) { lds_tie(a[decltype(im)::value][0]); });
            if constexpr (has_next) load_b(std::integral_constant<int, has_next ? n + 1 : n>{}, std::integral_constant<int, cur ^ 1>{});
            if constexpr (G.last && next_cell) wait_vmcnt<S.vm_wait[n]>();
            if constexpr (G.kind == 1) static_for<0, MT>([&](auto im) { c1[decltype(im)::value][G.child & 3] = (f32x4){0.f, 0.f, 0.f, 0.f}; });
            static_for<0, 4>([&](auto ie) {
                constexpr int e = decltype(ie)::value;
                if constexpr (G.first && e > 0) {
                    __builtin_amdgcn_sched_barrier(0);
                    wait_lgkmcnt<(3 - e) * MT + (has_next ? 4 : 0) + ((G.last && next_cell) ? e * MT : 0)>();
                    static_for<0, MT>([&](auto im) { lds_tie(a[decltype(im)::value][e]); });
                }
                static_for<0, 4>([&](auto iu) {
                    constexpr int u = decltype(iu)::value;
                    static_for<0, MT>([&](auto im) {
                        constexpr int m = decltype(im)::value;
#ifdef Q4_KO_MFMA
                        if constexpr (u == 0) { if constexpr (G.kind == 1) c1[m][G.child & 3][0] += a[m][e][0] * b[cur][e][0]; else acc0[m][G.child][0] += a[m][e][0] * b[cur][e][0]; }
#else
                        if constexpr (G.kind == 1) c1[m][G.child & 3] = __builtin_amdgcn_mfma_f32_4x4x1f32(b[cur][e][u], a[m][e][u], c1[m][G.child & 3], 0, 0, 0);
                        else acc0[m][G.child] = __builtin_amdgcn_mfma_f32_4x4x1f32(b[cur][e][u], a[m][e][u], acc0[m][G.child], 0, 0, 0);
#endif
                    });
                });
                if constexpr (G.last && next_cell) {
                    __builtin_amdgcn_sched_barrier(0);
                    load_a(std::integral_constant<int, next_cell ? G.cell + 1 : G.cell>{}, ie);
                }
            });
            __builtin_amdgcn_sched_barrier(0);
            if constexpr (G.first && G.cell + D < 64) gather(std::integral_constant<int, (G.cell + D < 64) ? G.cell + D : 0>{});
            if constexpr (KIND == Q4_PASS_A && n > 0) epi(std::integral_constant<int, (n > 0 ? n - 1 : 0)>{});
        });
        if constexpr (KIND == Q4_PASS_A) {
            epi(std::integral_constant<int, S.n - 1>{});
        } else {
            static_for<0, MT>([&](auto im) {
                constexpr int m = decltype(im)::value;
                const unsigned ov = (unsigned)((p_base + 64 * m + lane) * 32);
#pragma unroll
                for (int h = 0; h < 2; ++h) {
                    f32x4 v = acc0[m][h];
                    if (ep.b0) {
#pragma unroll
                        for (int r = 0; r < 4; ++r) v[r] = v[r] + b00[r];
                    }
#ifdef Q4_KO_STORE
                    sink = sink + v;
#else
                    q4_store(v, rs_out, ov + (unsigned)(h * 16));
#endif
                }
            });
        }
#ifdef Q4_KO_STORE
        q4_store(sink, rs_out, ovq(0));
#endif
    }
}

template <int KIND, int NW, int MT, int D = 2>
int launch_child_q4(const int32_t* pnbr, int64_t n_p, const float* in, int in_ld, const float* table, int table_bytes,
                    const IrnEpi& ep, hipStream_t s) {
    const size_t lds = (size_t)table_bytes + (size_t)NW * (D * MT * 4096);
    auto kern = k_child_q4<KIND, NW, MT, D>;
    static ChildLdsGrant granted;
    if (int rc = child_lds_limit(kern, lds, granted)) return rc;
    const int64_t units = (n_p + 64 * MT - 1) / (64 * MT);
    hipLaunchKernelGGL(kern, dim3(child_grid_units(units, NW, lds)), dim3(NW * 64), lds, s, pnbr, n_p, in, in_ld, table, table_bytes, ep);
    return 0;
}

}
```

### pcgcv2_amd/csrc/child_q4.hip

```cpp
#include "child_q4.h"

extern "C" int pcgc_irn_child_q4(const int32_t* parent_nbr, int64_t n_parent, int C, int pass, const float* in, int in_ld,
                                 const float* table, int64_t table_bytes, const float* b0, const float* b1, const float* b2,
                                 const float* x, int x_ld, float* out, int out_ld, void* stream) {
    CHILD_COMMON_CHECKS(in_ld)
    PCGC_REQUIRE(C == 16, "the quad-block kernels serve C = 16");
    PCGC_REQUIRE(pass == 1 || pass == 2, "pass must be 1 (A) or 2 (B)");
    PCGC_REQUIRE(out && b0 && b1 && (pass == 1 || (b2 && x)), "null argument");
    PCGC_REQUIRE((out_ld & 3) == 0 && (((uintptr_t)out) & 15) == 0 && (pass == 1 || ((x_ld & 3) == 0 && (((uintptr_t)x) & 15) == 0)),
                 "rows must be 16-byte aligned");
    hipStream_t s = S(stream);
    IrnEpi ep{b0, b1, b2, x, x_ld, out, out_ld};
    int rc;
    if (pass == 1) {
        PCGC_REQUIRE(out_ld == C / 2, "pass A writes a dense [rows, C/2] tensor");
        PCGC_REQUIRE(table_bytes == 28 * 64 * 4, "pass A table size");
        rc = launch_child_q4<Q4_PASS_A, 8, 2>(parent_nbr, n_parent, in, in_ld, table, (int)table_bytes, ep, s);
    } else {
        PCGC_REQUIRE(in_ld == C / 2, "pass B reads the dense [rows, C/2] tensor of pass A");
        PCGC_REQUIRE(table_bytes == 85 * 64 * 4, "pass B table size");
        rc = launch_child_irn_b<16, 16, 8, 1, true>(parent_nbr, n_parent, in, in_ld, table, (int)table_bytes, ep, s);
    }
    if (rc) return rc;
    PCGC_CHECK_LAUNCH("irn_child_q4");
    return 0;
}

extern "C" int pcgc_cls_child_q4(const int32_t* parent_nbr, int64_t n_parent, const float* in, int Cin, int in_ld,
                                 const float* table, int64_t table_bytes, const float* bias, float* out, void* stream) {
    CHILD_COMMON_CHECKS(in_ld)
    PCGC_REQUIRE(Cin == 16, "the quad-block classification head serves C = 16");
    PCGC_REQUIRE(out && (((uintptr_t)out) & 15) == 0, "the output must be 16-byte aligned");
    PCGC_REQUIRE(table_bytes == 96 * 64 * 4, "cls table size");
    IrnEpi ep{bias, nullptr, nullptr, nullptr, 0, out, 1};
    const int rc = launch_child_q4<Q4_CLS, 8, 2>(parent_nbr, n_parent, in, in_ld, table, (int)table_bytes, ep, S(stream));
    if (rc) return rc;
    PCGC_CHECK_LAUNCH("cls_child_q4");
    return 0;
}
```

### pcgcv2_amd/csrc/select.hip

```cpp
#include <algorithm>
#include <cstring>
#include "pcgc_common.h"
#include <rocprim/rocprim.hpp>

constexpr int SCAN_TILE = 2048;

__device__ static inline int block_exclusive_scan_256(int v, int* total_out) {
    __shared__ int wave_sums[4];
    int lane = threadIdx.x & 63, w = threadIdx.x >> 6;
    int incl = v;
#pragma unroll
    for (int d = 1; d < 64; d <<= 1) { int t = __shfl_up(incl, d, 64); if (lane >= d) incl += t; }
    if (lane == 63) wave_sums[w] = incl;
    __syncthreads();
    int base = 0, tot = 0;
#pragma unroll
    for (int i = 0; i < 4; ++i) { int s = wave_sums[i]; if (i < w) base += s; tot += s; }
    __syncthreads();
    if (total_out) *total_out = tot;
    return base + incl - v;
}

__device__ static inline int load_mask8(const uint8_t* mask, int64_t n, int64_t base, uint8_t m[8]) {
    int cnt = 0;
    if (base + 8 <= n && ((uintptr_t)(mask + base) & 7) == 0) {
        uint64_t w = *(const uint64_t*)(mask + base);
#pragma unroll
        for (int j = 0; j < 8; ++j) { m[j] = ((w >> (8 * j)) & 0xff) ? 1 : 0; cnt += m[j]; }
    } else {
#pragma unroll
        for (int j = 0; j < 8; ++j) { m[j] = (base + j < n && mask[base + j]) ? 1 : 0; cnt += m[j]; }
    }
    return cnt;
}

constexpr uint64_t SCAN_AGG = 1ull << 62, SCAN_INCL = 2ull << 62;
__global__ void __launch_bounds__(256) k_scan_lookback(const uint8_t* __restrict__ mask, int64_t n, int64_t n_tiles,
                                                       unsigned long long* desc, int32_t* ticket, int32_t* __restrict__ prefix,
                                                       int32_t* total, const uint32_t* enable) {
    if (enable && *enable == 0) return;
    __shared__ int tile_s, excl_s;
    if (threadIdx.x == 0) tile_s = atomicAdd(ticket, 1);
    __syncthreads();
    const int64_t tile = tile_s;
    uint8_t m[8];
    const int64_t base = tile * SCAN_TILE + threadIdx.x * 8;
    const int cnt = load_mask8(mask, n, base, m);
    int tot;
    int ex = block_exclusive_scan_256(cnt, &tot);
    if (threadIdx.x < 64) {
        const int lane = threadIdx.x;
        int excl = 0;
        if (tile == 0) {
            if (lane == 0) __hip_atomic_store(&desc[0], SCAN_INCL | (uint64_t)(uint32_t)tot, __ATOMIC_RELAXED, __HIP_MEMORY_SCOPE_AGENT);
        } else {
            if (lane == 0) __hip_atomic_store(&desc[tile], SCAN_AGG | (uint64_t)(uint32_t)tot, __ATOMIC_RELAXED, __HIP_MEMORY_SCOPE_AGENT);
            for (int64_t j = tile - 1;; j -= 64) {
                const int64_t idx = j - lane;
                unsigned long long d = SCAN_INCL;
                if (idx >= 0) {
                    do { d = __hip_atomic_load(&desc[idx], __ATOMIC_RELAXED, __HIP_MEMORY_SCOPE_AGENT); } while ((d >> 62) == 0);
                }
                const unsigned long long incl = __ballot((d >> 62) == 2);
                const int first = incl ? (int)__ffsll((long long)incl) - 1 : 63;
                int v = lane <= first ? (int)(uint32_t)d : 0;
#pragma unroll
                for (int o = 32; o > 0; o >>= 1) v += __shfl_xor(v, o, 64);
                excl += v;
                if (incl) break;
            }
            if (lane == 0) __hip_atomic_store(&desc[tile], SCAN_INCL | (uint64_t)(uint32_t)(excl + tot), __ATOMIC_RELAXED, __HIP_MEMORY_SCOPE_AGENT);
        }
        if (lane == 0) { excl_s = excl; if (tile == n_tiles - 1) *total = excl + tot; }
    }
    __syncthreads();
    ex += excl_s;
#pragma unroll
    for (int j = 0; j < 8; ++j) { if (base + j < n) prefix[base + j] = ex; ex += m[j]; }
}

static int64_t scan_tiles(int64_t n) { return (n + SCAN_TILE - 1) / SCAN_TILE; }
extern "C" size_t pcgc_scan_workspace_bytes(int64_t n) { return (size_t)(scan_tiles(n) + 2) * sizeof(uint64_t); }

static void launch_scan(const uint8_t* mask, int64_t n, int32_t* prefix, int32_t* total, void* workspace, const uint32_t* enable, hipStream_t s) {
    const int64_t tiles = scan_tiles(n);
    unsigned long long* desc = (unsigned long long*)workspace;
    hipLaunchKernelGGL(k_scan_lookback, dim3((unsigned)tiles), dim3(256), 0, s, mask, n, tiles, desc, (int32_t*)(desc + tiles), prefix, total, enable);
}
extern "C" int pcgc_mask_scan_zeroed(const uint8_t* mask, int64_t n, int32_t* prefix, int32_t* total, void* workspace,
                                     size_t workspace_bytes, void* stream) {
    PCGC_REQUIRE(workspace_bytes >= pcgc_scan_workspace_bytes(n), "workspace too small");
    PCGC_REQUIRE(((uintptr_t)workspace & 7) == 0, "workspace must be 8-byte aligned");
    if (n == 0) return 0;
    launch_scan(mask, n, prefix, total, workspace, nullptr, S(stream));
    PCGC_CHECK_LAUNCH("mask_scan");
    return 0;
}
extern "C" int pcgc_mask_scan(const uint8_t* mask, int64_t n, int32_t* prefix, int32_t* total, void* workspace,
                              size_t workspace_bytes, void* stream) {
    PCGC_REQUIRE(workspace_bytes >= pcgc_scan_workspace_bytes(n), "workspace too small");
    PCGC_REQUIRE(((uintptr_t)workspace & 7) == 0, "workspace must be 8-byte aligned");
    if (n == 0) { (void)hipMemsetAsync(total, 0, 4, S(stream)); return 0; }
    (void)hipMemsetAsync(workspace, 0, pcgc_scan_workspace_bytes(n), S(stream));
    launch_scan(mask, n, prefix, total, workspace, nullptr, S(stream));
    PCGC_CHECK_LAUNCH("mask_scan");
    return 0;
}

__global__ void k_compact_coords(const int4* __restrict__ in, const uint8_t* __restrict__ mask,
                                 const int32_t* __restrict__ prefix, int64_t n, int4* __restrict__ out) {
    int64_t i = (int64_t)blockIdx.x * blockDim.x + threadIdx.x;
    if (i < n && mask[i]) out[prefix[i]] = in[i];
}
__global__ void k_compact_feats4(const float* __restrict__ in, int C4, int in_ld, const uint8_t* __restrict__ mask,
                                 const int32_t* __restrict__ prefix, int64_t n, float* __restrict__ out) {
    int64_t t = (int64_t)blockIdx.x * blockDim.x + threadIdx.x;
    int64_t i = t / C4; int c = (int)(t % C4);
    if (i < n && mask[i])
        *(float4*)(out + (int64_t)prefix[i] * (C4 * 4) + 4 * c) = *(const float4*)(in + i * in_ld + 4 * c);
}
__global__ void k_compact_feats1(const float* __restrict__ in, int C, int in_ld, const uint8_t* __restrict__ mask,
                                 const int32_t* __restrict__ prefix, int64_t n, float* __restrict__ out) {
    int64_t t = (int64_t)blockIdx.x * blockDim.x + threadIdx.x;
    int64_t i = t / C; int c = (int)(t % C);
    if (i < n && mask[i]) out[(int64_t)prefix[i] * C + c] = in[i * in_ld + c];
}
extern "C" int pcgc_compact_coords(const int32_t* coords, const uint8_t* mask, const int32_t* prefix, int64_t n,
                                   int32_t* out, void* stream) {
    if (n == 0) return 0;
    hipLaunchKernelGGL(k_compact_coords, dim3(grid_for(n, 256)), dim3(256), 0, S(stream), (const int4*)coords, mask, prefix,
                       n, (int4*)out);
    PCGC_CHECK_LAUNCH("compact_coords");
    return 0;
}
extern "C" int pcgc_compact_feats(const float* in, int C, int in_ld, const uint8_t* mask, const int32_t* prefix, int64_t n,
                                  float* out, void* stream) {
    if (n == 0) return 0;
    if (C % 4 == 0 && in_ld % 4 == 0 && (((uintptr_t)in | (uintptr_t)out) & 15) == 0)
        hipLaunchKernelGGL(k_compact_feats4, dim3(grid_for(n * (C / 4), 256)), dim3(256), 0, S(stream), in, C / 4, in_ld, mask,
                           prefix, n, out);
    else
        hipLaunchKernelGGL(k_compact_feats1, dim3(grid_for(n * C, 256)), dim3(256), 0, S(stream), in, C, in_ld, mask, prefix,
                           n, out);
    PCGC_CHECK_LAUNCH("compact_feats");
    return 0;
}

struct TopkState { uint32_t prefix; uint32_t tie; int64_t k_remaining; uint32_t done; uint32_t count_eq; };
constexpr int TOPK_MAX_SEGS = 16;
struct TopkSegs { int n; long long off[TOPK_MAX_SEGS + 1]; long long k[TOPK_MAX_SEGS]; };

__device__ static inline uint32_t order_key(float f) {
    f = f + 0.0f;
    uint32_t b = __float_as_uint(f);
    return (b & 0x80000000u) ? ~b : (b | 0x80000000u);
}
constexpr int TOPK_PASSES = 3, TOPK_BINS = 2048;
__host__ __device__ static inline int topk_shift(int pass) { return pass == 0 ? 21 : (pass == 1 ? 10 : 0); }
__host__ __device__ static inline int topk_bits(int pass) { return pass == 2 ? 10 : 11; }
__global__ void __launch_bounds__(256) k_topk_init(TopkState* st, uint32_t* hist, TopkSegs segs, unsigned long long* scan_ws, int64_t scan_words, uint32_t* any_tie) {
    const int y = blockIdx.x;
    if (threadIdx.x == 0) { st[y].prefix = 0; st[y].tie = 0; st[y].k_remaining = segs.k[y]; st[y].done = 0; st[y].count_eq = 0; }
    for (int b = threadIdx.x; b < TOPK_BINS; b += blockDim.x) hist[TOPK_BINS * y + b] = 0;
    if (y == 0) {
        if (threadIdx.x == 0) *any_tie = 0;
        for (int64_t i = threadIdx.x; i < scan_words; i += blockDim.x) scan_ws[i] = 0;
    }
}
__global__ void __launch_bounds__(256) k_topk_hist(const float* __restrict__ v_all, int ld, TopkSegs segs, TopkState* st_all,
                                                   int pass, uint32_t* hist_all, uint32_t* any_tie) {
    __shared__ uint32_t h[TOPK_BINS];
    __shared__ int64_t S[257];
    __shared__ bool last_s;
    __shared__ int pick_s;
    const int t = threadIdx.x, y = blockIdx.y;
    const float* __restrict__ v = v_all + segs.off[y] * ld;
    const int64_t n = segs.off[y + 1] - segs.off[y];
    TopkState* st = st_all + y;
    uint32_t* hist = hist_all + TOPK_BINS * y;
    const int shift = topk_shift(pass), nb = 1 << topk_bits(pass);
    const uint32_t dmask = (uint32_t)nb - 1u;
    for (int b = t; b < nb; b += 256) h[b] = 0;
    __syncthreads();
    const uint32_t prefix = st->prefix;
    const uint32_t pmask = pass == 0 ? 0u : (0xFFFFFFFFu << (shift + topk_bits(pass)));
    const int64_t step = (int64_t)gridDim.x * blockDim.x;
    int64_t i = (int64_t)blockIdx.x * blockDim.x + t;
    for (; i + 7 * step < n; i += 8 * step) {
        float f[8];
#pragma unroll
        for (int u = 0; u < 8; ++u) f[u] = v[(i + u * step) * ld];
#pragma unroll
        for (int u = 0; u < 8; ++u) {
            const uint32_t key = order_key(f[u]);
            if ((key & pmask) == prefix) atomicAdd(&h[(key >> shift) & dmask], 1u);
        }
    }
    for (; i < n; i += step) {
        uint32_t key = order_key(v[i * ld]);
        if ((key & pmask) == prefix) atomicAdd(&h[(key >> shift) & dmask], 1u);
    }
    __syncthreads();
    uint32_t seen = 0;
    for (int b = t; b < nb; b += 256) if (h[b]) seen += atomicAdd(&hist[b], h[b]);
    asm volatile("s_waitcnt vmcnt(0)" : "+v"(seen) :: "memory");
    __syncthreads();
    if (t == 0) last_s = atomicAdd(&st->done, 1u) == gridDim.x - 1;
    __syncthreads();
    if (!last_s) return;
    const int PER = nb >> 8;
    uint32_t mine[TOPK_BINS / 256];
    int64_t gsum = 0;
#pragma unroll
    for (int e = 0; e < TOPK_BINS / 256; ++e) {
        mine[e] = e < PER ? __hip_atomic_load(&hist[t * PER + e], __ATOMIC_RELAXED, __HIP_MEMORY_SCOPE_AGENT) : 0u;
        gsum += mine[e];
    }
    S[t] = gsum;
    if (t == 0) { S[256] = 0; pick_s = -1; }
    __syncthreads();
    for (int off = 1; off < 256; off <<= 1) {
        const int64_t add = t + off < 256 ? S[t + off] : 0;
        __syncthreads();
        S[t] += add;
        __syncthreads();
    }
    const int64_t need = st->k_remaining;
    __syncthreads();
    const bool group_hit = t == 0 ? (S[1] < need) : (S[t] >= need && (S[t + 1] < need || t == 255));
    if (group_hit) {
        int64_t above = S[t + 1];
        int d = t * PER;
        uint32_t cnt = mine[0];
        bool found = false;
#pragma unroll
        for (int e = TOPK_BINS / 256 - 1; e >= 0; --e) {
            if (e < PER && !found) {
                if (above + mine[e] >= need || (t == 0 && e == 0)) { d = t * PER + e; cnt = mine[e]; found = true; }
                else above += mine[e];
            }
        }
        const int64_t rem = need - above;
        st->prefix = prefix | ((uint32_t)d << shift);
        st->k_remaining = rem;
        st->done = 0;
        if (pass == TOPK_PASSES - 1) {
            st->count_eq = cnt;
            st->tie = rem < (int64_t)cnt ? 1u : 0u;
            if (rem < (int64_t)cnt) atomicOr(any_tie, 1u);
        }
    }
    for (int b = t; b < nb; b += 256) hist[b] = 0;
}
__global__ void k_topk_mask(const float* __restrict__ v, int ld, TopkSegs segs, const TopkState* st_all, uint8_t* mask, uint8_t* eq) {
    const int y = blockIdx.y;
    const int64_t i = (int64_t)blockIdx.x * blockDim.x + threadIdx.x, n = segs.off[y + 1] - segs.off[y];
    if (i >= n) return;
    const int64_t g = segs.off[y] + i;
    const TopkState* st = st_all + y;
    const uint32_t key = order_key(v[g * ld]), T = st->prefix;
    const bool tie = st->tie != 0;
    mask[g] = (key > T) || (key == T && !tie);
    eq[g] = tie && key == T;
}
__global__ void k_topk_tie_fix(const TopkState* st_all, TopkSegs segs, const uint8_t* __restrict__ eq, const int32_t* __restrict__ eq_rank,
                               int tie_high, uint8_t* mask) {
    const int y = blockIdx.y;
    const TopkState* st = st_all + y;
    if (st->tie == 0) return;
    const int64_t i = (int64_t)blockIdx.x * blockDim.x + threadIdx.x, n = segs.off[y + 1] - segs.off[y];
    if (i >= n) return;
    const int64_t g = segs.off[y] + i;
    if (!eq[g]) return;
    const int64_t need = st->k_remaining, r = (int64_t)eq_rank[g] - (int64_t)eq_rank[segs.off[y]];
    mask[g] = tie_high ? r >= (int64_t)st->count_eq - need : r < need;
}
static int g_topk_tie_high = 0;
extern "C" int pcgc_set_convention(int what, int value) {
    if (what == 0) { g_topk_tie_high = value ? 1 : 0; return 0; }
    pcgc_set_error("set_convention: unknown convention %d", what);
    return -2;
}
static size_t align256(size_t v) { return (v + 255) & ~(size_t)255; }
extern "C" size_t pcgc_topk_workspace_bytes(int64_t n) {
    return 1024 + (size_t)TOPK_MAX_SEGS * TOPK_BINS * 4 + align256((size_t)n) + align256((size_t)n * 4) + 256 + align256(pcgc_scan_workspace_bytes(n));
}
static int topk_segments(const float* logits, int ld, const TopkSegs& segs, uint8_t* mask, void* workspace, size_t workspace_bytes, void* stream) {
    const int64_t n = segs.off[segs.n];
    PCGC_REQUIRE(workspace_bytes >= pcgc_topk_workspace_bytes(n), "workspace too small");
    PCGC_REQUIRE(((uintptr_t)workspace & 7) == 0, "workspace must be 8-byte aligned");
    if (n == 0) return 0;
    char* ws = (char*)workspace;
    TopkState* st = (TopkState*)ws;
    uint32_t* any_tie = (uint32_t*)(ws + 768); ws += 1024;
    uint32_t* hist = (uint32_t*)ws; ws += (size_t)TOPK_MAX_SEGS * TOPK_BINS * 4;
    uint8_t* eq = (uint8_t*)ws; ws += align256((size_t)n);
    int32_t* rank = (int32_t*)ws; ws += align256((size_t)n * 4);
    int32_t* total = (int32_t*)ws; ws += 256;
    void* scan_ws = ws;
    int64_t nmax = 0;
    for (int b = 0; b < segs.n; ++b) nmax = std::max<int64_t>(nmax, segs.off[b + 1] - segs.off[b]);
    unsigned g = grid_for(nmax, 256 * 8); if (g > 256) g = 256; if (g < 1) g = 1;
    hipLaunchKernelGGL(k_topk_init, dim3(segs.n), dim3(256), 0, S(stream), st, hist, segs, (unsigned long long*)scan_ws,
                       (int64_t)(pcgc_scan_workspace_bytes(n) / 8), any_tie);
    for (int pass = 0; pass < TOPK_PASSES; ++pass)
        hipLaunchKernelGGL(k_topk_hist, dim3(g, segs.n), dim3(256), 0, S(stream), logits, ld, segs, st, pass, hist, any_tie);
    hipLaunchKernelGGL(k_topk_mask, dim3(grid_for(nmax, 256), segs.n), dim3(256), 0, S(stream), logits, ld, segs, st, mask, eq);
    launch_scan(eq, n, rank, total, scan_ws, any_tie, S(stream));
    hipLaunchKernelGGL(k_topk_tie_fix, dim3(grid_for(nmax, 256), segs.n), dim3(256), 0, S(stream), st, segs, eq, rank, g_topk_tie_high, mask);
    PCGC_CHECK_LAUNCH("topk_mask");
    return 0;
}
extern "C" int pcgc_topk_mask(const float* logits, int ld, int64_t n, int64_t k, uint8_t* mask, void* workspace,
                              size_t workspace_bytes, void* stream) {
    if (n == 0) return 0;
    if (k >= n) { (void)hipMemsetAsync(mask, 1, (size_t)n, S(stream)); return 0; }
    if (k <= 0) { (void)hipMemsetAsync(mask, 0, (size_t)n, S(stream)); return 0; }
    TopkSegs segs{};
    segs.n = 1; segs.off[0] = 0; segs.off[1] = n; segs.k[0] = k;
    return topk_segments(logits, ld, segs, mask, workspace, workspace_bytes, stream);
}

extern "C" int pcgc_topk_mask_segments(const float* logits, int ld, int nseg, const int64_t* seg_rows, const int64_t* seg_k,
                                       uint8_t* mask, void* workspace, size_t workspace_bytes, void* stream) {
    PCGC_REQUIRE(nseg >= 0 && nseg <= TOPK_MAX_SEGS && (nseg == 0 || (seg_rows && seg_k)), "at most 16 segments");
    if (nseg == 0) return 0;
    TopkSegs segs{};
    segs.n = nseg; segs.off[0] = 0;
    for (int b = 0; b < nseg; ++b) {
        PCGC_REQUIRE(seg_rows[b] >= 0, "negative segment");
        segs.off[b + 1] = segs.off[b] + seg_rows[b];
        segs.k[b] = seg_k[b] < 0 ? 0 : (seg_k[b] > seg_rows[b] ? seg_rows[b] : seg_k[b]);
    }
    return topk_segments(logits, ld, segs, mask, workspace, workspace_bytes, stream);
}

struct SelSeg { uint32_t T; int64_t need, thr, K0, G0, E0; };
__device__ static inline int4 child_coords(const int4* __restrict__ parent, int64_t g, int32_t h) {
    const int4 c = parent[g >> 3]; const int k = (int)(g & 7);
    return make_int4(c.x, c.y + (k & 1) * h, c.z + ((k >> 1) & 1) * h, c.w + (k >> 2) * h);
}
__global__ void __launch_bounds__(256) k_topk_select(const float* __restrict__ v, int ld, TopkSegs segs, const TopkState* __restrict__ st_all,
                                                     const int4* __restrict__ coords, const int4* __restrict__ parent, int32_t half,
                                                     int tie_high, int64_t n, int64_t n_tiles, unsigned long long* desc, int32_t* ticket,
                                                     uint8_t* __restrict__ bits, int32_t* __restrict__ wprefix,
                                                     int32_t* __restrict__ orig, int4* __restrict__ out_coords) {
    __shared__ SelSeg seg[TOPK_MAX_SEGS];
    __shared__ int tile_s, exg_s, exe_s;
    const int t = threadIdx.x;
    if (t == 0) {
        tile_s = atomicAdd(ticket, 1);
        int64_t K0 = 0, G0 = 0, E0 = 0;
        for (int b = 0; b < segs.n; ++b) {
            const TopkState s = st_all[b];
            const int64_t need = s.k_remaining < (int64_t)s.count_eq ? s.k_remaining : (int64_t)s.count_eq;
            seg[b].T = s.prefix; seg[b].need = need; seg[b].thr = (int64_t)s.count_eq - need;
            seg[b].K0 = K0; seg[b].G0 = G0; seg[b].E0 = E0;
            K0 += segs.k[b]; G0 += segs.k[b] - need; E0 += s.count_eq;
        }
    }
    __syncthreads();
    const int64_t tile = tile_s;
    const int64_t base = tile * SCAN_TILE + t * 8;
    uint32_t key[8];
    if (ld == 1 && base + 8 <= n && ((uintptr_t)(v + base) & 15) == 0) {
        const float4 a = *(const float4*)(v + base), b4 = *(const float4*)(v + base + 4);
        key[0] = order_key(a.x); key[1] = order_key(a.y); key[2] = order_key(a.z); key[3] = order_key(a.w);
        key[4] = order_key(b4.x); key[5] = order_key(b4.y); key[6] = order_key(b4.z); key[7] = order_key(b4.w);
    } else {
#pragma unroll
        for (int j = 0; j < 8; ++j) key[j] = base + j < n ? order_key(v[(base + j) * ld]) : 0u;
    }
    int b0 = 0;
    while (b0 + 1 < segs.n && base >= segs.off[b0 + 1]) ++b0;
    uint32_t gt = 0, eq = 0;
    {
        int b = b0;
#pragma unroll
        for (int j = 0; j < 8; ++j) {
            const int64_t g = base + j;
            while (b + 1 < segs.n && g >= segs.off[b + 1]) ++b;
            if (g < n) {
                const uint32_t T = seg[b].T;
                gt |= (uint32_t)(key[j] > T) << j;
                eq |= (uint32_t)(key[j] == T) << j;
            }
        }
    }
    int tot;
// ... 11 lines not shown
                const int64_t idx = j - lane;
                unsigned long long d = SCAN_INCL;
                if (idx >= 0) {
                    do { d = __hip_atomic_load(&desc[idx], __ATOMIC_RELAXED, __HIP_MEMORY_SCOPE_AGENT); } while ((d >> 62) == 0);
                }
                const unsigned long long incl = __ballot((d >> 62) == 2);
                const int first = incl ? (int)__ffsll((long long)incl) - 1 : 63;
                int vg = lane <= first ? (int)((d >> 31) & 0x7FFFFFFFull) : 0, ve = lane <= first ? (int)(d & 0x7FFFFFFFull) : 0;
#pragma unroll
                for (int o = 32; o > 0; o >>= 1) { vg += __shfl_xor(vg, o, 64); ve += __shfl_xor(ve, o, 64); }
                exg += vg; exe += ve;
                if (incl) break;
            }
            if (lane == 0) {
                const unsigned long long inc = ((unsigned long long)(uint32_t)(exg + (tot & 0xFFFF)) << 31) | (unsigned long long)(uint32_t)(exe + (tot >> 16));
                __hip_atomic_store(&desc[tile], SCAN_INCL | inc, __ATOMIC_RELAXED, __HIP_MEMORY_SCOPE_AGENT);
            }
        }
        if (lane == 0) { exg_s = exg; exe_s = exe; }
    }
    __syncthreads();
    int64_t G = (int64_t)exg_s + (ex & 0xFFFF), E = (int64_t)exe_s + (ex >> 16);
    uint32_t keep = 0;
    int b = b0;
    int64_t first_out = 0;
#pragma unroll
    for (int j = 0; j < 8; ++j) {
        const int64_t g = base + j;
        while (b + 1 < segs.n && g >= segs.off[b + 1]) ++b;
        const SelSeg sg = seg[b];
        const int64_t r = E - sg.E0;
        const int64_t eq_kept = tie_high ? (r > sg.thr ? r - sg.thr : 0) : (r < sg.need ? r : sg.need);
        const int64_t out = sg.K0 + (G - sg.G0) + eq_kept;
        if (j == 0) first_out = out;
        const bool is_gt = (gt >> j) & 1u, is_eq = (eq >> j) & 1u;
        const bool kept = is_gt || (is_eq && (tie_high ? r >= sg.thr : r < sg.need));
        if (kept) {
            keep |= 1u << j;
            orig[out] = (int32_t)g;
            out_coords[out] = coords ? coords[g] : child_coords(parent, g, half);
        }
        G += is_gt; E += is_eq;
    }
    const int64_t n64 = (n + 63) & ~(int64_t)63;
    if (base < n64) {
        bits[base >> 3] = (uint8_t)keep;
        if ((t & 7) == 0) wprefix[base >> 6] = (int32_t)first_out;
    }
}
extern "C" size_t pcgc_topk_select_workspace_bytes(int64_t n) {
    return 1024 + (size_t)TOPK_MAX_SEGS * TOPK_BINS * 4 + align256(pcgc_scan_workspace_bytes(n));
}
extern "C" int pcgc_topk_select(const float* logits, int ld, int nseg, const int64_t* seg_rows, const int64_t* seg_k,
                                const int32_t* coords, const int32_t* parent_coords, int32_t parent_stride,
                                uint8_t* bits, int32_t* wprefix, int32_t* orig, int32_t* out_coords,
                                void* workspace, size_t workspace_bytes, void* stream) {
    PCGC_REQUIRE(nseg >= 1 && nseg <= TOPK_MAX_SEGS && seg_rows && seg_k, "1 to 16 segments");
    PCGC_REQUIRE((coords != nullptr) != (parent_coords != nullptr), "exactly one of coords / parent_coords");
    PCGC_REQUIRE(!parent_coords || (parent_stride >= 2 && (parent_stride & 1) == 0), "parent stride must be even");
    PCGC_REQUIRE(((uintptr_t)bits & 7) == 0 && ((uintptr_t)workspace & 7) == 0, "bits and workspace must be 8-byte aligned");
    TopkSegs segs{};
    segs.n = nseg; segs.off[0] = 0;
    for (int b = 0; b < nseg; ++b) {
        PCGC_REQUIRE(seg_rows[b] >= 0, "negative segment");
        segs.off[b + 1] = segs.off[b] + seg_rows[b];
        segs.k[b] = seg_k[b] < 0 ? 0 : (seg_k[b] > seg_rows[b] ? seg_rows[b] : seg_k[b]);
    }
    const int64_t n = segs.off[nseg];
    PCGC_REQUIRE(n < (1ll << 31), "too many rows");
    PCGC_REQUIRE(!parent_coords || (n & 7) == 0, "a children level has 8 rows per parent");
    PCGC_REQUIRE(workspace_bytes >= pcgc_topk_select_workspace_bytes(n), "workspace too small");
    if (n == 0) return 0;
    char* ws = (char*)workspace;
    TopkState* st = (TopkState*)ws;
    uint32_t* any_tie = (uint32_t*)(ws + 768); ws += 1024;
    uint32_t* hist = (uint32_t*)ws; ws += (size_t)TOPK_MAX_SEGS * TOPK_BINS * 4;
    unsigned long long* desc = (unsigned long long*)ws;
    const int64_t tiles = scan_tiles(n);
    int64_t nmax = 0;
    for (int b = 0; b < nseg; ++b) nmax = std::max<int64_t>(nmax, segs.off[b + 1] - segs.off[b]);
    unsigned g = grid_for(nmax, 256 * 8); if (g > 256) g = 256; if (g < 1) g = 1;
    hipLaunchKernelGGL(k_topk_init, dim3(nseg), dim3(256), 0, S(stream), st, hist, segs, desc, (int64_t)(pcgc_scan_workspace_bytes(n) / 8), any_tie);
    for (int pass = 0; pass < TOPK_PASSES; ++pass)
        hipLaunchKernelGGL(k_topk_hist, dim3(g, nseg), dim3(256), 0, S(stream), logits, ld, segs, st, pass, hist, any_tie);
    hipLaunchKernelGGL(k_topk_select, dim3((unsigned)tiles), dim3(256), 0, S(stream), logits, ld, segs, st, (const int4*)coords,
                       (const int4*)parent_coords, parent_stride / 2, g_topk_tie_high, n, tiles, desc, (int32_t*)(desc + tiles),
                       bits, wprefix, orig, (int4*)out_coords);
    PCGC_CHECK_LAUNCH("topk_select");
    return 0;
}
__global__ void k_gather_rows_f32x4(const float* __restrict__ in, int C4, int in_ld, const int32_t* __restrict__ orig, int64_t n_out,
                                    float* __restrict__ out) {
    const int64_t t = (int64_t)blockIdx.x * blockDim.x + threadIdx.x;
    const int64_t r = t / C4; const int c = (int)(t % C4);
    if (r < n_out) *(float4*)(out + r * (C4 * 4) + 4 * c) = *(const float4*)(in + (int64_t)orig[r] * in_ld + 4 * c);
}
extern "C" int pcgc_gather_rows_f32_ld(const float* in, int C, int in_ld, const int32_t* orig, int64_t n_out, float* out, void* stream) {
    PCGC_REQUIRE(C > 0 && (C & 3) == 0 && (in_ld & 3) == 0 && ((uintptr_t)in & 15) == 0 && ((uintptr_t)out & 15) == 0, "rows of 4-float chunks, 16-byte aligned");
    if (n_out == 0) return 0;
    hipLaunchKernelGGL(k_gather_rows_f32x4, dim3(grid_for(n_out * (C / 4), 256)), dim3(256), 0, S(stream), in, C / 4, in_ld, orig, n_out, out);
    PCGC_CHECK_LAUNCH("gather_rows_f32_ld");
    return 0;
}

__global__ void k_batch_counts(const int4* __restrict__ coords, int64_t n, int32_t* __restrict__ counts) {
    __shared__ int h[16];
    if (threadIdx.x < 16) h[threadIdx.x] = 0;
    __syncthreads();
    for (int64_t i = (int64_t)blockIdx.x * blockDim.x + threadIdx.x; i < n; i += (int64_t)gridDim.x * blockDim.x) {
        const int b = coords[i].x;
        if ((unsigned)b < 16u) atomicAdd(&h[b], 1);
    }
    __syncthreads();
    if (threadIdx.x < 16 && h[threadIdx.x]) atomicAdd(&counts[threadIdx.x], h[threadIdx.x]);
}
extern "C" int pcgc_batch_counts(const int32_t* coords, int64_t n, int32_t* counts, void* stream) {
    PCGC_REQUIRE(counts != nullptr, "null argument");
    hipError_t e = hipMemsetAsync(counts, 0, 16 * sizeof(int32_t), S(stream));
    if (e != hipSuccess) { pcgc_set_error("batch_counts: %s", hipGetErrorString(e)); return -1; }
    if (n == 0) return 0;
    unsigned g = grid_for(n, 256 * 16); if (g > 512) g = 512; if (g < 1) g = 1;
    hipLaunchKernelGGL(k_batch_counts, dim3(g), dim3(256), 0, S(stream), (const int4*)coords, n, counts);
    PCGC_CHECK_LAUNCH("batch_counts");
    return 0;
}

__global__ void k_zyx_keys(const int4* __restrict__ coords, int64_t n, uint64_t* keys, int32_t* idx, int batch_major) {
    int64_t i = (int64_t)blockIdx.x * blockDim.x + threadIdx.x;
    if (i >= n) return;
    int4 c = coords[i];
    keys[i] = batch_major ? (((uint64_t)(uint32_t)c.x << 60) | ((uint64_t)(uint32_t)c.w << 40) | ((uint64_t)(uint32_t)c.z << 20) | (uint64_t)(uint32_t)c.y)
                          : (((uint64_t)(uint32_t)c.w << 44) | ((uint64_t)(uint32_t)c.z << 24) | ((uint64_t)(uint32_t)c.y << 4) | (uint64_t)(uint32_t)c.x);
    idx[i] = (int32_t)i;
}
static size_t sort_temp_bytes(int64_t n) {
    size_t tmp = 0;
    (void)rocprim::radix_sort_pairs((void*)nullptr, tmp, (uint64_t*)nullptr, (uint64_t*)nullptr, (int32_t*)nullptr, (int32_t*)nullptr,
                              (size_t)n, 0, 64, (hipStream_t)0);
    return tmp;
}
extern "C" size_t pcgc_sort_workspace_bytes(int64_t n) {
    if (n < 1) n = 1;
    return align256((size_t)n * 8) * 2 + align256((size_t)n * 4) + align256(sort_temp_bytes(n));
}
static int sort_coords(const int32_t* coords, int64_t n, int32_t* perm, void* workspace, size_t workspace_bytes, void* stream, int batch_major);
extern "C" int pcgc_sort_zyx(const int32_t* coords, int64_t n, int32_t* perm, void* workspace, size_t workspace_bytes,
                             void* stream) {
    return sort_coords(coords, n, perm, workspace, workspace_bytes, stream, 0);
}
extern "C" int pcgc_sort_bzyx(const int32_t* coords, int64_t n, int32_t* perm, void* workspace, size_t workspace_bytes,
                              void* stream) {
    return sort_coords(coords, n, perm, workspace, workspace_bytes, stream, 1);
}
static int sort_coords(const int32_t* coords, int64_t n, int32_t* perm, void* workspace, size_t workspace_bytes, void* stream, int batch_major) {
    PCGC_REQUIRE(workspace_bytes >= pcgc_sort_workspace_bytes(n), "workspace too small");
    if (n == 0) return 0;
    char* ws = (char*)workspace;
    uint64_t* kin = (uint64_t*)ws; ws += align256((size_t)n * 8);
    uint64_t* kout = (uint64_t*)ws; ws += align256((size_t)n * 8);
    int32_t* idx = (int32_t*)ws; ws += align256((size_t)n * 4);
    size_t tmp = sort_temp_bytes(n);
    hipLaunchKernelGGL(k_zyx_keys, dim3(grid_for(n, 256)), dim3(256), 0, S(stream), (const int4*)coords, n, kin, idx, batch_major);
    hipError_t e = rocprim::radix_sort_pairs((void*)ws, tmp, kin, kout, idx, perm, (size_t)n, 0, 64, S(stream));
    if (e != hipSuccess) { pcgc_set_error("sort_zyx: %s", hipGetErrorString(e)); return -1; }
    PCGC_CHECK_LAUNCH("sort_zyx");
    return 0;
}

__global__ void k_gather_i32x4(const int4* __restrict__ in, const int32_t* __restrict__ perm, int64_t n, int4* out) {
    int64_t i = (int64_t)blockIdx.x * blockDim.x + threadIdx.x;
    if (i < n) out[i] = in[perm[i]];
// ... 19 lines not shown
```

### pcgcv2_amd/dispatch.py

```python
from collections import namedtuple

from . import ops

LIMIT = 0xF0000000

Rule = namedtuple('Rule', 'op shape level rows_min rows_max switch family kernel why')
INF = 1 << 62

TABLE = (
    Rule('conv3', ((16, 16), (32, 32), (16, 1), (32, 1), (64, 1)), 'children', 8192, INF, 'CHILD_MFMA', 'child',
         'k_child_conv<1,1> / k_child_conv<2,2,split> / k_child_cls<NB>; 16->1 with CHILD_Q4: k_child_q4<cls> (quad-block 4x4x1 MFMA)',
         'halo gather through the parent map, packed-N fp32 MFMA: conv 16->16 436 -> 259 us on 2.05 M rows, cls 16->1 209 -> 85 (quad-block form: 83)'),
    Rule('conv3', ((1, 16),), None, 0, INF, 'UNIT_INPUT_CONV', 'unit', 'k_conv_unit<16> / k_conv_unit_coarse<16>',
         'all-ones occupancy input (x.has_unit_features()): sum of kernel slices over the present offsets, no feature gathers: 88 -> 55 us'),
    Rule('conv3', ((32, 32),), None, 'ROWS_CONV_MIN', INF, 'ROWS_CONV', 'rows', 'k_rows_conv<2,2>',
         'LDS-resident fragment table, one wave per 16-row tile: 34 vs 51 us at 1-18 k rows, 127 vs 159 at 256 k'),
    Rule('conv3', ((64, 64),), None, 'PACKED_CONV64_MIN', INF, 'PACKED_CONV64', 'packed', 'k_conv_packed64',
         'present rows packed per workgroup tile and offset, accumulators in LDS, B fragments in registers: conv2 (71 k rows) 215 -> 118 us, conv0 (150 k) 335 -> 306 (profiles/r04_conv_packed.md)'),
    Rule('conv3', None, None, 0, INF, None, 'gather', 'pcgc_conv_gather (see GATHER below)', 'every other shape / size'),
    Rule('irn', (16, 32), 'children', 8192, INF, 'CHILD_MFMA', 'child',
         'k_child_irn_a<C> + k_child_irn_b<C> (C = 32: half units); C = 16 with CHILD_Q4: k_child_q4<pass A> (quad-block 4x4x1 MFMA) + k_child_irn_b<16, T2 gather>',
         'packed-N MFMA passes through the parent map: C = 16 212/170 -> 118/102 us on 2.05 M rows (quad-block pass A: 97/110), C = 32 174/130 -> 100/81 on 570 k'),
    Rule('irn', (64,), None, 'ROWS_IRN64_MIN', INF, 'ROWS_IRN64', 'rows64', 'k_rows_irn_a64<.., RowsPassA64H> + k_rows_irn_b64',
         "through the level's own map, plain or children level (the decoder's 64 -> 64 conv has built it): 65 vs 135 us per block at 1-18 k rows, 103 vs 198 at 71 k; "
         'on the 150 k-row children level 171 vs 197 us for the parent-map form (removed in round 5)'),
    Rule('irn', (32,), None, 'ROWS_Q4_MIN', 'ROWS_IRN32_MAX+1', 'ROWS_Q4', 'rows32q4', 'k_rows_q4_a32 + k_rows_q4_b32',
         'quad-block form (4x4x1 fp32 MFMA, lane = row, no zero column: issued / algorithmic 3.9 -> 2.1 in pass A): 120 -> 88 us per block at 256 k rows; '
         'below ~150 k rows the 64-row tiles are one round of lone waves and the packed-N kernels stay ahead (40 vs 46 us at 71 k)'),
    Rule('irn', (32,), None, 'ROWS_IRN32_MIN', 'ROWS_IRN32_MAX+1', 'ROWS_IRN32', 'rows32', 'k_rows_irn_a32 + k_rows_irn_b32',
         'plain level: 47 vs 74 us per block at 49 k rows, 119 vs 127 at 256 k'),
    Rule('irn', (16, 32, 64), None, 0, INF, 'FUSE_IRN', 'valu', 'k_irn_a_split<C> + k_irn_b_split<C> (C = 16, 32), k_irn_a<64,16> + k_irn_b<64,16>',
         'two fused gather passes on the VALU, 16-row tiles: levels below 1024 rows, children levels below 8192'),
    Rule('irn', None, None, 0, INF, None, 'unfused', 'five MinkowskiConvolution calls + fused epilogues', 'any other channel count'),
    Rule('down', ((16, 32), (32, 64), (64, 32)), None, 'ROWS_DOWN_MIN', INF, 'ROWS_DOWN', 'rows_down', 'k_rows_down<NB,NT>',
         'tile = 16 coarse rows walking the 8 child offsets: 121 -> ~65 us for the three down convs of a vox10 frame (rows = COARSE rows)'),
    Rule('down', None, None, 0, INF, None, 'gather', 'pcgc_conv_gather, K = 8', 'other shapes / tiny levels'),
    Rule('conv1', None, None, 0, INF, None, 'gather', 'pcgc_conv_gather, K = 1 (k_conv_gather_valu)', 'k1 convs outside fused blocks'),
    Rule('prune', (8, 16, 32, 64), None, 0, INF, 'ONE_SWEEP_PRUNE', 'select', 'k_topk_init + 3 x k_topk_hist + k_topk_select',
         'thresholds by radix select, then ONE scan writes coordinates, survivor rows and a rank bitmap: 10 -> 5 launches per decoder stage'),
    Rule('prune', None, None, 0, INF, None, 'mask', 'pcgc_topk_mask(_segments) + pcgc_mask_scan + pcgc_compact_*', 'byte mask + int32 prefix per row'),
    Rule('up', None, None, 0, INF, None, 'up2', 'k_conv_up2_mfma<64,32> / <32,16>, k_conv_up2_rows otherwise', 'generative transpose, one kernel per shape'),
)

GATHER_IMPL_NAMES = {0: 'k_conv_gather_valu', 2: 'k_conv_gather_mfma', 6: 'k_conv_gather_split (row-split)'}
GATHER_GATES = {'mfma_min_rows': 512, 'split_below_cout16': 40000}


def gather_impl(K, cin, cout, rows, aligned=True):
    g = GATHER_GATES
    dma = aligned and K <= 27 and cin in (8, 16, 32, 64)
    split_shape = dma and K == 27 and cin <= 32 and cout in (4, 8, 16)
    split_first = split_shape and (cout <= 8 or rows < g['split_below_cout16'])
    if dma and cin in (16, 32, 64) and cout in (16, 32, 64) and not split_first and rows >= g['mfma_min_rows']:
        return 2
    if split_first:
        return 6
    return 0


def _value(v, cfg):
    if isinstance(v, str):
        name, plus, inc = v.partition('+')
        return getattr(cfg, name) + (int(inc) if plus else 0)
    return v


def _switch_on(rule, cfg):
    if rule.switch is None:
        return True
    return bool(getattr(cfg, rule.switch))


def select(op, shape, rows, level='plain', extent=None, contiguous=True, unit_input=False, plain_output=True, cfg=None):
    cfg = ops.PATH if cfg is None else cfg
    width = shape[0]
    extent = rows * 4 * width if extent is None else extent
    key = tuple(shape) if len(shape) > 1 else shape[0]
    for rule in TABLE:
        if rule.op != op or (rule.shape is not None and key not in rule.shape):
            continue
        if not (_value(rule.rows_min, cfg) <= rows < _value(rule.rows_max, cfg)) or not _switch_on(rule, cfg):
            continue
        if rule.level is not None and level != 'children':
            continue
        fam = rule.family
        if fam in ('packed', 'child') and op == 'conv3' and not plain_output:
            continue
        if fam in ('child', 'rows', 'rows64', 'rows32', 'rows32q4', 'rows_down', 'packed') and extent >= LIMIT:
            continue
        if op == 'irn' and fam != 'unfused' and (not cfg.FUSE_IRN or rows * 4 * width >= 0xFFFFFFF0):
            continue
        if fam == 'child' and op == 'irn' and not contiguous:
            continue
        if fam == 'unit' and not (unit_input and plain_output):
            continue
        if fam == 'rows_down' and not plain_output:
            continue
        return rule
    raise ops.PcgcError(f'dispatch: no kernel for {op} {shape} on a {level} level of {rows} rows')


def entries(cfg=None):
    cfg = ops.PATH if cfg is None else cfg
    out = []
    for rule in TABLE:
        lo, hi = _value(rule.rows_min, cfg), _value(rule.rows_max, cfg)
        out.append((rule, [r for r in (lo, hi - 1) if 0 < r < INF]))
    return out


def describe(cfg=None):
    cfg = ops.PATH if cfg is None else cfg
    lines = []
    for r in TABLE:
        lo, hi = _value(r.rows_min, cfg), _value(r.rows_max, cfg)
        rng = f'{lo}..' + ('' if hi >= INF else str(hi - 1))
        lines.append(f'{r.op:6s} {str(r.shape or "any"):48s} {str(r.level or "any"):18s} rows {rng:16s} -> {r.family:9s} {r.kernel}')
    return '\n'.join(lines)
```

### pcgcv2_amd/nn.py

```python
import math
import torch

from . import dispatch, ops
from .sparse import SparseTensor


class _ConvBase(torch.nn.Module):
    def __init__(self, in_channels, out_channels, kernel_size, stride=1, bias=True, dimension=3):
        super().__init__()
        assert dimension == 3
        self.in_channels, self.out_channels = in_channels, out_channels
        self.kernel_size, self.stride = kernel_size, stride
        vol = kernel_size ** 3
        shape = (in_channels, out_channels) if vol == 1 else (vol, in_channels, out_channels)
        self.kernel = torch.nn.Parameter(torch.empty(shape, dtype=torch.float32))
        self.bias = torch.nn.Parameter(torch.empty((1, out_channels), dtype=torch.float32)) if bias else None
        bound = 1.0 / math.sqrt(vol * in_channels)
        with torch.no_grad():
            self.kernel.uniform_(-bound, bound)
            if self.bias is not None:
                self.bias.zero_()

    def extra_repr(self):
        return f'in={self.in_channels}, out={self.out_channels}, kernel_size={self.kernel_size}, stride={self.stride}'


class MinkowskiConvolution(_ConvBase):

    def forward(self, x, relu=False, out=None, residual=None):
        k, s = self.kernel_size, self.stride
        cin, cout = self.in_channels, self.out_channels
        plain_out = out is None and residual is None
        if k == 3 and s == 1:
            level = 'children' if x.cmap.origin is not None and x.cmap.origin[0] == 'children' else 'plain'
            fam = dispatch.select('conv3', (cin, cout), x.F.shape[0], level, extent=x.F.shape[0] * x.F.stride(0) * 4,
                                  unit_input=cin == 1 and x.has_unit_features(), plain_output=plain_out).family
            if fam == 'child':
                if cout == 1 and cin == 16 and ops.PATH.CHILD_Q4 and plain_out and not relu and x.F.shape[0] >= 8 * ops.PATH.CHILD_Q4_MIN_PARENTS:
                    y = ops.cls_child_q4(x.cmap.origin[1].k3, x.F, self._table(ops.child_q4_cls_table), self.bias)
                    return SparseTensor(y, coordinate_map=x.cmap)
                table = self._table(ops.child_cls_table if cout == 1 else ops.child_conv_table)
                y = ops.conv_child(x.cmap.origin[1].k3, x.F, table, self.bias, cout, out=out, residual=residual, relu=relu)
                return SparseTensor(y, coordinate_map=x.cmap)
            if fam == 'unit':
                cm = x.cmap
                if cm.mapless_unit_conv() and cout in (4, 8, 16) and not ops.PROFILE.counting:
                    coarse, down = cm.down()
                    y = ops.conv_unit_from_coarse(cm.C, cm.stride, cm._parent_of, coarse.k3, down, self.kernel, self.bias, relu=relu)
                    return SparseTensor(y, coordinate_map=cm)
                return SparseTensor(ops.conv_gather_unit(cm.k3, self.kernel, self.bias, relu=relu), coordinate_map=cm)
            if fam == 'packed':
                y = ops.conv_packed64(x.cmap.k3, x.F, self._table(ops.child_conv_table), self.bias, relu=relu)
                return SparseTensor(y, coordinate_map=x.cmap)
            if fam == 'rows':
                y = ops.conv_rows(x.cmap.k3, x.F, self._table(ops.child_conv_table), self.bias, cout, out=out, residual=residual, relu=relu)
                return SparseTensor(y, coordinate_map=x.cmap)
            cmap, nbr = x.cmap, x.cmap.k3
        elif k == 1 and s == 1:
            cmap, nbr = x.cmap, None
        elif k == 2 and s == 2:
            cmap, nbr = x.cmap.down()
            fam = dispatch.select('down', (cin, cout), nbr.shape[1], extent=max(x.F.shape[0] * x.F.stride(0), nbr.shape[1] * cout) * 4,
                                  plain_output=plain_out).family
            if fam == 'rows_down':
                y = ops.conv_down_rows(nbr, x.F, self._table(ops.child_conv_table), self.bias, cout, relu=relu)
                return SparseTensor(y, coordinate_map=cmap)
        else:
            raise NotImplementedError(f'MinkowskiConvolution(kernel_size={k}, stride={s}) is not on the PCGCv2 path')
        y = ops.conv_gather(nbr, x.F, self.kernel, self.bias, out=out, residual=residual, relu=relu)
        return SparseTensor(y, coordinate_map=cmap)

    def _table(self, build):
        stamp = (self.kernel.data_ptr(), self.kernel._version)
        slots = self.__dict__.setdefault('_child_tables', {})
        hit = slots.get(build.__name__)
        if hit is None or hit[0] != stamp:
            hit = slots[build.__name__] = (stamp, build(self.kernel))
        return hit[1]


class MinkowskiGenerativeConvolutionTranspose(_ConvBase):
    def forward(self, x, relu=False):
        assert self.kernel_size == 2 and self.stride == 2
        src = x.pending_rows()
        if src is not None:
            y = ops.conv_up2(src[0], self.kernel, self.bias, relu=relu, rows=src[1])
        else:
            y = ops.conv_up2(x.F, self.kernel, self.bias, relu=relu)
        return SparseTensor(y, coordinate_map=x.cmap.up())


class MinkowskiPruning(torch.nn.Module):

    def forward(self, x, mask, n_keep=None, keep_per_item=None):
        from .sparse import CoordMap
        prefix, total = ops.mask_scan(mask)
        n = int(total.item()) if n_keep is None else int(n_keep)
        coords = ops.compact_coords(x.C, mask, prefix, n)
        src = x.F
        feats = lambda: ops.compact_feats(src, mask, prefix, n)
        cmap = CoordMap(coords, x.cmap.stride, unique=True, origin=('pruned', x.cmap, mask, prefix))
        if keep_per_item is not None:
            cmap._batch_rows = [int(k) for k in keep_per_item]
        return SparseTensor(feats, coordinate_map=cmap)
```

### pcgcv2_amd/ops.py

```python
import os as _os

import numpy as np
import torch

from ._lib import lib, check, PcgcError


def _stream(t=None):
    if t is None:
        return torch.cuda.current_stream().cuda_stream
    return torch.cuda.current_stream(t.device).cuda_stream


def _p(t):
    return None if t is None else t.data_ptr()


def _dev(t, dtype, what):
    if not t.is_cuda:
        raise PcgcError(f'{what}: expected a ROCm device tensor, got {t.device} (no CPU fallback exists)')
    if t.dtype != dtype:
        raise PcgcError(f'{what}: expected {dtype}, got {t.dtype}')
    if not t.is_contiguous():
        raise PcgcError(f'{what}: tensor must be contiguous')
# ... 720 lines not shown
                cells.append((kp, jc, reach))
    assert sum(len(r) for _, _, r in cells) == 216
    return cells


def child_conv_table(W):
    K, Cin, Cout = W.shape
    NB, NT = Cin // 16, Cout // 16
    return W.detach().reshape(K, NB, 4, 4, NT, 16).permute(0, 4, 1, 3, 5, 2).contiguous().reshape(-1)


def _fragment(col_weights, NB, KS=4, k0=0, half=False):
    ncol = 8 if half else 16
    out = np.full((NB, 4, ncol, KS), -1, np.int64)
    for mi, w in enumerate(col_weights):
        if w is None:
            continue
        for cb in range(NB):
            for jj in range(KS):
                for mq in range(4):
                    ch = 16 * cb + 4 * (k0 + jj) + mq
                    if ch < len(w):
                        out[cb, mq, mi, jj] = w[ch]
    return out.reshape(NB, -1)


_TABLE_INDEX = {}


def _gather_table(index, flat):
    return torch.where(index >= 0, flat[index.clamp(min=0)], torch.zeros((), dtype=flat.dtype, device=flat.device)).contiguous()


def _cls_index(C):
    nb = C // 16
    rowf = nb * 16 + 4
    idx = np.full(((125 * rowf * 4 + 1023) // 1024 * 256,), -1, np.int64)
    for kz in range(3):
        for ky in range(3):
            for kx in range(3):
                r = 25 * (kz + 1) + 5 * (ky + 1) + (kx + 1)
                k = 9 * kz + 3 * ky + kx
                for cb in range(nb):
                    for mq in range(4):
                        for jj in range(4):
                            idx[r * rowf + cb * 16 + mq * 4 + jj] = k * C + 16 * cb + 4 * jj + mq
    return idx


def child_cls_table(W):
    C = W.shape[1]
    key = ('cls', C, W.device)
    if key not in _TABLE_INDEX:
        _TABLE_INDEX[key] = torch.from_numpy(_cls_index(C)).to(W.device)
    return _gather_table(_TABLE_INDEX[key], W.detach().reshape(-1))


def _q4_cls_index(C):
    W = np.arange(27 * C, dtype=np.int64).reshape(27, C)
    frags = []
    for c, (kp, jc, reach) in enumerate(_halo_cells()):
        cz = c >> 4
        kof = dict(reach)
        for h in range(2):
            if not 0 <= cz - h <= 2:
                continue
            f = np.full((4, C), -1, np.int64)
            for sidx in range(4):
                if 4 * h + sidx in kof:
                    f[sidx] = W[kof[4 * h + sidx]]
            frags.append(f.reshape(-1))
    assert len(frags) == 96
    return np.concatenate(frags)


def child_q4_cls_table(W):
    C = W.shape[1]
    key = ('q4cls', C, W.device)
    if key not in _TABLE_INDEX:
        _TABLE_INDEX[key] = torch.from_numpy(_q4_cls_index(C)).to(W.device)
    return _gather_table(_TABLE_INDEX[key], W.detach().reshape(-1))


def cls_child_q4(parent_nbr, x, table, bias):
    _f32(x, 'x')
    n_p = parent_nbr.shape[1]
    if x.shape[0] != 8 * n_p:
        raise PcgcError('cls_child_q4: feature rows must be 8 x the parent level')
    Cin = x.shape[1]
    n = 8 * n_p
    out = torch.empty((n, 1), dtype=torch.float32, device=x.device)
    key = ('child_conv', Cin, 1, n)
    prof = PROFILE.want(key)
    if prof:
        e0, e1 = PROFILE.bracket(key, f'k_child_q4<1, 8, 2> (k3 {Cin}->1 on a children level, parent-map halo gather + quad-block 4x4x1 fp32 MFMA)', n,
                                 lambda P, a=Cin: P * a * 4 + P * 8 + n * 4, lambda P, a=Cin: 2 * P * a,
                                 compulsory=n * Cin * 4 + 27 * n_p * 4 + n * 4, mfma_issued=((n_p + 63) // 64) * 96 * 16 * 512)
        e0.record()
    check(lib().pcgc_cls_child_q4(_p(parent_nbr), n_p, _p(x), Cin, _ld(x), _p(table), table.numel() * 4, _p(bias), _p(out), _stream(x)), 'cls_child_q4')
    if prof:
        e1.record()
    elif PROFILE.counting:
        PROFILE.count_children(parent_nbr)
    return out


def _irn_index(C):
    Q, NB = C // 4, C // 16
    shapes = [(27, C, Q), (27, Q, 2 * Q), (C, Q), (27, Q, Q), (Q, 2 * Q)]
    off, Ws = 0, []
    for shp in shapes:
        n = int(np.prod(shp))
        Ws.append(np.arange(off, off + n, dtype=np.int64).reshape(shp))
        off += n
    W00, W01, W10, W11, W12 = Ws
    cpt = 16 // Q

    def packed(Wk3, width, kz, ky, cy, cx):
        cols = []
        nchild = 16 // width
        for sub in range(nchild):
            if ky is None:
                jy, jx = sub >> 1, sub & 1
                kyy = cy - jy
            else:
                jx, kyy = sub, ky
            kxx = cx - jx
            ok = 0 <= kyy <= 2 and 0 <= kxx <= 2
            for co in range(width):
                cols.append(Wk3[kz * 9 + kyy * 3 + kxx][:, co] if ok else None)
        return cols

    fa = []
    if cpt == 1:
        for k in range(27):
            fa.append(_fragment([W00[k][:, co] for co in range(16)], NB))
        fa.append(_fragment([W10[:, co] for co in range(16)], NB))
        fb = []
        for k in range(27):
            for n2 in range(2):
                fb.append(_fragment([W01[k][:, 16 * n2 + co] for co in range(16)], 1))
        for k in range(27):
            fb.append(_fragment([W11[k][:, co] for co in range(16)], 1))
        for n2 in range(2):
            fb.append(_fragment([W12[:, 16 * n2 + co] for co in range(16)], 1))
        return np.concatenate([f.reshape(-1) for f in fa]), np.concatenate([f.reshape(-1) for f in fb])
    if cpt == 4:
        for kz in range(3):
            for cy in range(4):
                for cx in range(4):
                    fa.append(_fragment(packed(W00, Q, kz, None, cy, cx), NB))
        for vy in range(2):
            for vx in range(2):
                fa.append(_fragment([W10[:, co] if sub == vy * 2 + vx else None for sub in range(4) for co in range(Q)], NB))
    else:
        for kz in range(3):
            for ky in range(3):
                for cx in range(4):
                    fa.append(_fragment(packed(W00, Q, kz, ky, None, cx), NB))
        for vx in range(2):
            fa.append(_fragment([W10[:, co] if sub == vx else None for sub in range(2) for co in range(Q)], NB))
    table_a = np.concatenate([f.reshape(-1) for f in fa])
    KS = Q // 4
    H = 2 * Q
    fb = []
    pad = lambda w, lo: np.concatenate([np.full(lo, -1, np.int64), w])
    if H == 16:
        for k in range(27):
            fb.append(_fragment([W01[k][:, co] for co in range(16)], 1, KS=KS, k0=0))
    else:
        for kz in range(3):
            for ky in range(3):
                for cx in range(4):
                    fb.append(_fragment(packed(W01, H, kz, ky, None, cx), 1, KS=KS, k0=0))
    W11p = np.stack([np.stack([pad(W11[k][:, co], Q) for co in range(Q)], 1) for k in range(27)])
    if cpt == 2:
        for kz in range(3):
            for ky in range(3):
                for cx in range(4):
                    fb.append(_fragment(packed(W11p, Q, kz, ky, None, cx), 1, KS=KS, k0=KS))
    else:
        for kz in range(3):
            for cy in range(4):
                for cx in range(4):
                    fb.append(_fragment(packed(W11p, Q, kz, None, cy, cx), 1, KS=KS, k0=KS))
    fb.append(_fragment([W12[:, co] if co < H else None for co in range(16)], 1, KS=KS, k0=0))
    table_b = np.concatenate([f.reshape(-1) for f in fb])
    return table_a, table_b


def child_irn_tables(params):
    W00, b00, W01, b01, W10, b10, W11, b11, W12, b12 = params
    C = W00.shape[1]
    key = ('irn', C, W00.device)
    if key not in _TABLE_INDEX:
        ia, ib = _irn_index(C)
        _TABLE_INDEX[key] = (torch.from_numpy(ia).to(W00.device), None if ib is None else torch.from_numpy(ib).to(W00.device))
    flat = torch.cat([w.detach().reshape(-1) for w in (W00, W01, W10, W11, W12)])
    ia, ib = _TABLE_INDEX[key]
    return _gather_table(ia, flat), (None if ib is None else _gather_table(ib, flat))




def child_q4_tables(params):
    W00, W10 = params[0], params[4]
    C = W00.shape[1]
    return torch.cat([W00.detach().reshape(27, C, C // 4).permute(0, 2, 1).reshape(-1),
                      W10.detach().reshape(C, C // 4).t().reshape(-1)]).contiguous()




def irn_block_child(parent_nbr, x, params, tables, q4_table=None):
    _f32(x, 'x')
    n_p = parent_nbr.shape[1]
    n, C = x.shape
    if n != 8 * n_p:
        raise PcgcError('irn_block_child: feature rows must be 8 x the parent level')
    ta, tb = tables
    t = torch.empty((n, C // 2), dtype=torch.float32, device=x.device)
    out = torch.empty((n, C), dtype=torch.float32, device=x.device)
    P = [p.data_ptr() for p in params]
    s = _stream(x)
    if PROFILE.counting:
        PROFILE.count_children(parent_nbr)
    tiles = (n_p + 15) // 16
    per_tile = {16: (416, 248), 32: (1216, 736)}[C]
    names = (f'k_child_irn_a<{C}>', f'k_child_irn_b<{C}>')
    q4 = PATH.CHILD_Q4 and C == 16 and q4_table is not None
    if q4:
        per_tile = ((216 + 8) * 16 // 4 // 4 + 128 // 8 // 4, per_tile[1])
        names = ('k_child_q4<0, 8, 2>', 'k_child_irn_b<16>')
    forms = _irn_pass_formulas(n, C, 27 * n_p * 4, names)
    if q4:
        calls = (lambda: lib().pcgc_irn_child_q4(_p(parent_nbr), n_p, C, 1, _p(x), _ld(x), _p(q4_table), q4_table.numel() * 4, P[1], P[5], None,
                                                 None, 0, _p(t), C // 2, s),
                 lambda: lib().pcgc_irn_child_q4(_p(parent_nbr), n_p, C, 2, _p(t), C // 2, _p(tb), tb.numel() * 4, P[3], P[7], P[9], _p(x), _ld(x),
                                                 _p(out), C, s))
    else:
        calls = (lambda: lib().pcgc_irn_child_pass(_p(parent_nbr), n_p, C, 1, _p(x), _ld(x), _p(ta), ta.numel() * 4, P[1], P[5], None, None, 0,
                                                   _p(t), C // 2, s),
                 lambda: lib().pcgc_irn_child_pass(_p(parent_nbr), n_p, C, 2, _p(t), C // 2, _p(tb), tb.numel() * 4, P[3], P[7], P[9], _p(x), _ld(x),
                                                   _p(out), C, s))
    for (ps, name, bf, ff, comp), call, mf in zip(forms, calls, per_tile):
        prof = PROFILE.want((name, n))
        if prof:
            e0, e1 = PROFILE.bracket((name, n), name + ' (fused InceptionResNet pass on a children level, packed-N fp32 MFMA)', n, bf, ff,
                                     compulsory=comp, mfma_issued=tiles * mf * 2048)
            e0.record()
        check(call(), 'irn_child_pass')
        if prof:
            e1.record()
    return out


def conv_child(parent_nbr, x, table, bias, Cout, out=None, residual=None, relu=False):
    _f32(x, 'x')
    n_p = parent_nbr.shape[1]
    if x.shape[0] != 8 * n_p:
        raise PcgcError('conv_child: feature rows must be 8 x the parent level')
    Cin = x.shape[1]
    if out is None:
        out = torch.empty((8 * n_p, Cout), dtype=torch.float32, device=x.device)
    res_p, res_ld = (None, 0) if residual is None else (_p(_f32(residual)), _ld(residual))
    n = 8 * n_p
    key = ('child_conv', Cin, Cout, n)
    prof = PROFILE.want(key)
    if prof:
        tiles = (n_p + 15) // 16
        per_tile = 64 * (Cin // 16) * 4 if Cout == 1 else 216 * (Cin // 16) * (Cout // 16) * 4
        name = f'k_child_cls<{Cin // 16}>' if Cout == 1 else f'k_child_conv<{Cin // 16}, {Cout // 16}>'
        e0, e1 = PROFILE.bracket(key, name + f' (k3 {Cin}->{Cout} on a children level, parent-map halo gather + fp32 MFMA)', n,
                                 lambda P, a=Cin, b=Cout: P * a * 4 + P * 8 + n * b * 4, lambda P, a=Cin, b=Cout: 2 * P * a * b,
                                 compulsory=n * Cin * 4 + 27 * n_p * 4 + n * Cout * 4 + (0 if residual is None else n * Cout * 4),
                                 mfma_issued=tiles * per_tile * 2048)
        e0.record()
    check(lib().pcgc_conv_child(_p(parent_nbr), n_p, _p(x), Cin, _ld(x), _p(table), table.numel() * 4, _p(bias), res_p, res_ld,
                                int(relu), _p(out), Cout, _ld(out), _stream(x)), 'conv_child')
    if prof:
        e1.record()
    elif PROFILE.counting:
        PROFILE.count_children(parent_nbr)
    return out




def conv_rows(nbr, x, table, bias, Cout, out=None, residual=None, relu=False):
    _f32(x, 'x')
    n, Cin = x.shape
    if out is None:
        out = torch.empty((n, Cout), dtype=torch.float32, device=x.device)
    res_p, res_ld = (None, 0) if residual is None else (_p(_f32(residual)), _ld(residual))
    key = ('conv', Cin, Cout, n)
    prof = PROFILE.want(key)
    if prof:
        e0, e1 = PROFILE.bracket(key, f'k_rows_conv<{Cin // 16}, {Cout // 16}> (k3 {Cin}->{Cout} on a plain level, LDS-resident table + per-wave row ring, fp32 MFMA)', n,
                                 lambda P, a=Cin, b=Cout: P * a * 4 + P * 8 + n * b * 4, lambda P, a=Cin, b=Cout: 2 * P * a * b,
                                 compulsory=n * Cin * 4 + 27 * n * 4 + n * Cout * 4 + (0 if residual is None else n * Cout * 4),
                                 mfma_issued=2 * 27 * ((n + 15) // 16 * 16) * Cin * Cout)
        e0.record()
    check(lib().pcgc_conv_rows(_p(nbr), n, _p(x), Cin, _ld(x), _p(table), table.numel() * 4, _p(bias), res_p, res_ld, int(relu), _p(out), Cout,
                               _ld(out), _stream(x)), 'conv_rows')
    if prof:
        e1.record()
    elif PROFILE.counting:
        PROFILE.count(nbr)
    return out




def conv_packed64(nbr, x, table, bias, relu=False):
    _f32(x, 'x')
    n = x.shape[0]
    out = torch.empty((n, 64), dtype=torch.float32, device=x.device)
    key = ('conv', 64, 64, n)
    prof = PROFILE.want(key)
    if prof:
        e0, e1 = PROFILE.bracket(key, 'k_conv_packed64 (k3 64->64, present-row packing: accumulators in LDS, B fragments in registers, fp32 MFMA)', n,
                                 lambda P, n=n: P * 64 * 4 + P * 8 + n * 64 * 4, lambda P: 2 * P * 64 * 64,
                                 compulsory=n * 64 * 4 + 27 * n * 4 + n * 64 * 4,
                                 mfma_issued=lambda P, n=n: 2 * (P + 8 * 27 * ((n + 95) // 96)) * 64 * 64)
        e0.record()
    check(lib().pcgc_conv_packed64(_p(nbr), n, _p(x), _ld(x), _p(table), table.numel() * 4, _p(bias), int(relu), _p(out), 64, _stream(x)),
          'conv_packed64')
    if prof:
        e1.record()
    elif PROFILE.counting:
        PROFILE.count(nbr)
    return out




def conv_down_rows(down, x, table, bias, Cout, relu=False):
    _f32(x, 'x')
    n_in, Cin = x.shape
    n_c = down.shape[1]
    out = torch.empty((n_c, Cout), dtype=torch.float32, device=x.device)
    key = ('down', Cin, Cout, n_c)
    prof = PROFILE.want(key)
    if prof:
        e0, e1 = PROFILE.bracket(key, f'k_rows_down<{Cin // 16}, {Cout // 16}> (k2 s2 {Cin}->{Cout} through the down map, LDS-resident table, fp32 MFMA)', n_c,
                                 lambda P, a=Cin, b=Cout: P * a * 4 + n_c * b * 4, lambda P, a=Cin, b=Cout: 2 * P * a * b,
                                 compulsory=n_in * Cin * 4 + 8 * n_c * 4 + n_c * Cout * 4,
                                 mfma_issued=2 * 8 * ((n_c + 15) // 16 * 16) * Cin * Cout, pairs=n_in)
        e0.record()
    check(lib().pcgc_conv_down_rows(_p(down), n_c, _p(x), n_in, Cin, _ld(x), _p(table), table.numel() * 4, _p(bias), int(relu), _p(out), Cout,
                                    _ld(out), _stream(x)), 'conv_down_rows')
    if prof:
        e1.record()
    return out


def conv_up2(x, W, bias, relu=False, rows=None):
    _f32(x, 'x'); _f32(W, 'W')
    K, Cin, Cout = W.shape
    n_in = x.shape[0] if rows is None else rows.shape[0]
    key = ('up2', Cin, Cout, 8 * n_in)
    prof = PROFILE.want(key)
    if prof:
        mfma = (Cin, Cout) in ((64, 32), (32, 16))
        e0, e1 = PROFILE.bracket(key, f'k_conv_up2<{Cin}, {Cout}> (generative transpose k2 s2, ' + ('eight GEMMs sharing the A fragments, fp32 MFMA)' if mfma else
                                 'one thread per (row, 16-byte chunk), VALU)'), 8 * n_in,
                                 lambda P, a=Cin, b=Cout: P * (a + b) * 4, lambda P, a=Cin, b=Cout: 2 * P * a * b,
                                 compulsory=n_in * Cin * 4 + 8 * n_in * Cout * 4 + (0 if rows is None else n_in * 4),
                                 mfma_issued=(2 * 8 * ((n_in + 15) // 16 * 16) * Cin * Cout) if mfma else None, pairs=8 * n_in)
        e0.record()
    try:
        if rows is not None:
            out = torch.empty((8 * rows.shape[0], Cout), dtype=torch.float32, device=x.device)
            rc = lib().pcgc_conv_up2_gather(rows.shape[0], _p(x), Cin, _ld(x), _p(rows), _p(W), _p(bias), int(relu), _p(out), Cout, _stream(x))
            if rc == 0:
                return out
            if rc != -3:
                check(rc, 'conv_up2_gather')
            x = gather_rows(x, rows)
        out = torch.empty((8 * x.shape[0], Cout), dtype=torch.float32, device=x.device)
        check(lib().pcgc_conv_up2(x.shape[0], _p(x), Cin, _ld(x), _p(W), _p(bias), int(relu), _p(out), Cout, _stream(x)), 'conv_up2')
        return out
    finally:
        if prof:
            e1.record()


def topk_mask(logits, k):
    _f32(logits, 'logits')
    n = logits.shape[0]
    ld = logits.stride(0)
    mask = torch.empty(n, dtype=torch.uint8, device=logits.device)
    ws_bytes = int(lib().pcgc_topk_workspace_bytes(n))
    ws = torch.empty(ws_bytes, dtype=torch.uint8, device=logits.device)
    check(lib().pcgc_topk_mask(_p(logits), ld, n, int(k), _p(mask), _p(ws), ws_bytes, _stream(logits)), 'topk_mask')
    return mask


def sort_zyx(coords, batch_major=False):
    n = coords.shape[0]
    perm = torch.empty(n, dtype=torch.int32, device=coords.device)
    ws_bytes = int(lib().pcgc_sort_workspace_bytes(n))
    ws = torch.empty(ws_bytes, dtype=torch.uint8, device=coords.device)
    fn = lib().pcgc_sort_bzyx if batch_major else lib().pcgc_sort_zyx
    check(fn(_p(_i32(coords)), n, _p(perm), _p(ws), ws_bytes, _stream(coords)), 'sort_zyx')
    return perm


def batch_counts(coords):
    counts = torch.empty(16, dtype=torch.int32, device=coords.device)
    check(lib().pcgc_batch_counts(_p(_i32(coords)), coords.shape[0], _p(counts), _stream(coords)), 'batch_counts')
    c = counts.cpu().tolist()
    while len(c) > 1 and c[-1] == 0:
        c.pop()
    return c


def _i64_array(values):
    import ctypes
    return (ctypes.c_int64 * len(values))(*[int(v) for v in values])


def topk_mask_segments(logits, seg_rows, seg_k):
    _f32(logits, 'logits')
    n = logits.shape[0]
    if sum(seg_rows) != n:
        raise PcgcError(f'topk_mask_segments: segments cover {sum(seg_rows)} of {n} rows')
    mask = torch.empty(n, dtype=torch.uint8, device=logits.device)
    ws_bytes = int(lib().pcgc_topk_workspace_bytes(n))
    ws = torch.empty(ws_bytes, dtype=torch.uint8, device=logits.device)
    check(lib().pcgc_topk_mask_segments(_p(logits), logits.stride(0), len(seg_rows), _i64_array(seg_rows), _i64_array(seg_k), _p(mask), _p(ws),
                                        ws_bytes, _stream(logits)), 'topk_mask_segments')
    return mask




def topk_select(logits, seg_rows, seg_k, coords=None, parent_coords=None, parent_stride=0):
    _f32(logits, 'logits')
    n = logits.shape[0]
    if sum(seg_rows) != n:
        raise PcgcError(f'topk_select: segments cover {sum(seg_rows)} of {n} rows')
    if len(seg_rows) > 16:
        raise PcgcError('topk_select: at most 16 segments')
    K = sum(int(min(max(k, 0), r)) for r, k in zip(seg_rows, seg_k))
    dev = logits.device
    words = (n + 63) // 64
    bits = torch.empty(words * 8, dtype=torch.uint8, device=dev)
    wprefix = torch.empty(words, dtype=torch.int32, device=dev)
    orig = torch.empty(K, dtype=torch.int32, device=dev)
    out = torch.empty((K, 4), dtype=torch.int32, device=dev)
    ws_bytes = int(lib().pcgc_topk_select_workspace_bytes(n))
    ws = torch.empty(ws_bytes, dtype=torch.uint8, device=dev)
    check(lib().pcgc_topk_select(_p(logits), logits.stride(0), len(seg_rows), _i64_array(seg_rows), _i64_array(seg_k),
                                 _p(None if coords is None else _i32(coords)), _p(None if parent_coords is None else _i32(parent_coords)),
                                 int(parent_stride), _p(bits), _p(wprefix), _p(orig), _p(out), _p(ws), ws_bytes, _stream(logits)), 'topk_select')
    return bits, wprefix, orig, out


def kmap_k3_prune_sel(cand_nbr, bits, wprefix, orig):
    n_out = orig.shape[0]
    nbr = torch.empty((27, n_out), dtype=torch.int32, device=cand_nbr.device)
    check(lib().pcgc_kmap_k3_prune_sel(_p(cand_nbr), cand_nbr.shape[1], _p(bits), _p(wprefix), _p(orig), n_out, _p(nbr), _stream(cand_nbr)),
          'kmap_k3_prune_sel')
    return nbr


def kmap_k3_prune_parent_sel(parent_nbr, bits, wprefix, orig):
    n_out = orig.shape[0]
    nbr = torch.empty((27, n_out), dtype=torch.int32, device=parent_nbr.device)
    check(lib().pcgc_kmap_k3_prune_parent_sel(_p(parent_nbr), parent_nbr.shape[1], _p(bits), _p(wprefix), _p(orig), n_out, _p(nbr),
                                              _stream(parent_nbr)), 'kmap_k3_prune_parent_sel')
    return nbr


def gather_rows(feats, orig):
    _f32(feats)
    C = feats.shape[1]
    out = torch.empty((orig.shape[0], C), dtype=torch.float32, device=feats.device)
    check(lib().pcgc_gather_rows_f32_ld(_p(feats), C, _ld(feats), _p(orig), orig.shape[0], _p(out), _stream(feats)), 'gather_rows_f32_ld')
    return out


def gather_coords(coords, perm):
    out = torch.empty_like(coords)
    check(lib().pcgc_gather_rows_i32x4(_p(_i32(coords)), _p(perm), coords.shape[0], _p(out), _stream(coords)), 'gather_rows_i32x4')
    return out


def gather_feats(feats, perm):
    feats = _f32(feats).contiguous()
    out = torch.empty_like(feats)
    check(lib().pcgc_gather_rows_f32(_p(feats), feats.shape[1], _p(perm), feats.shape[0], _p(out), _stream(feats)), 'gather_rows_f32')
    return out


def relu(x, inplace=False):
    x = _f32(x).contiguous()
    out = x if inplace else torch.empty_like(x)
    check(lib().pcgc_relu(_p(x), x.numel(), _p(out), _stream(x)), 'relu')
    return out


def add(a, b):
    a, b = _f32(a).contiguous(), _f32(b).contiguous()
    if a.shape != b.shape:
        raise PcgcError(f'add: shapes {tuple(a.shape)} and {tuple(b.shape)} differ')
    out = torch.empty_like(a)
    check(lib().pcgc_add(_p(a), _p(b), a.numel(), _p(out), _stream(a)), 'add')
    return out


def round_minmax(feats):
    feats = _f32(feats).contiguous()
    mm = torch.empty(2, dtype=torch.float32, device=feats.device)
    check(lib().pcgc_round_minmax(_p(feats), feats.numel(), _p(mm), _stream(feats)), 'round_minmax')
    return mm


def symbolize(feats, min_v):
    feats = _f32(feats).contiguous()
    sym = torch.empty(feats.shape, dtype=torch.int16, device=feats.device)
    check(lib().pcgc_symbolize(_p(feats), feats.numel(), float(min_v), _p(sym), _stream(feats)), 'symbolize')
    return sym


def desymbolize(sym, min_v):
    out = torch.empty(sym.shape, dtype=torch.float32, device=sym.device)
    check(lib().pcgc_desymbolize(_p(_dev(sym, torch.int16, 'sym')), sym.numel(), float(min_v), _p(out), _stream(sym)), 'desymbolize')
    return out


def check_symbol_range(min_v, max_v, what='latent'):
    lo, hi = float(min_v), float(max_v)
    if not (np.isfinite(lo) and np.isfinite(hi)):
        raise PcgcError(f'{what}: the rounded values range from {lo} to {hi}: a latent that is not finite cannot be coded')
# ... 770 lines not shown
```

### pcgcv2_amd/pathconfig.py

```python
import dataclasses
import os


def _env(name, default='1'):
    return os.environ.get(name, default) != '0'


@dataclasses.dataclass(frozen=True)
class PathConfig:
    UNIT_INPUT_CONV: bool = True
    UNIT_CONV_MAPLESS: bool = True
    FUSE_IRN: bool = True
    ROWS_IRN64: bool = True
    ROWS_IRN64_MIN: int = 1024
    ROWS_IRN32: bool = True
    ROWS_IRN32_MIN: int = 1024
    ROWS_IRN32_MAX: int = 0xF0000000 // (32 * 4) - 1
    ROWS_Q4: bool = True
    ROWS_Q4_MIN: int = 150_000
    CHILD_MFMA: bool = True
    CHILD_Q4: bool = True
    CHILD_Q4_MIN_PARENTS: int = 200_000
    ROWS_CONV: bool = True
    ROWS_CONV_MIN: int = 1024
    PACKED_CONV64: bool = True
    PACKED_CONV64_MIN: int = 512
    ROWS_DOWN: bool = True
    ROWS_DOWN_MIN: int = 1024
    ONE_SWEEP_PRUNE: bool = True
    D1_CELLS: bool = True

    @classmethod
    def from_env(cls):
        off = {f.name: False for f in dataclasses.fields(cls) if f.type in (bool, 'bool') and not _env('PCGC_' + f.name)}
        return cls(**off)

    def replace(self, **changes):
        unknown = set(changes) - FIELDS
        if unknown:
            raise AttributeError(f'PathConfig has no field(s) {sorted(unknown)}')
        return dataclasses.replace(self, **changes)

    def switches(self):
        return {f.name: getattr(self, f.name) for f in dataclasses.fields(self) if isinstance(getattr(self, f.name), bool)}


FIELDS = frozenset(f.name for f in dataclasses.fields(PathConfig))
```

Measured before the change: 141.2.

## Fuse first top-k radix histogram into classification head epilogue

The classification head kernels (child cls 32/64 and q4 cls) gain a templated epilogue that builds the first-digit radix histogram of the logits in LDS and flushes it to a persistent per-stream state buffer. A new topk_select_hist0 entry point starts from that histogram, so the decoder skips the init pass and one histogram pass over the logits for single-cloud inference. The cost is extra LDS and atomics in the head kernels, plus a state buffer that must be zeroed and reused correctly across calls.

After: 142.0 (median of 2 runs). No clear change (+0.5%).

```diff
diff --git a/include/pcgc_hip.h b/include/pcgc_hip.h
--- a/include/pcgc_hip.h
+++ b/include/pcgc_hip.h
@@ -123,6 +123,19 @@
 int pcgc_topk_select(const float* logits , int ld, int nseg, const int64_t* seg_rows, const int64_t* seg_k,
                      const int32_t* coords, const int32_t* parent_coords, int32_t parent_stride,
                      uint8_t* bits, int32_t* wprefix, int32_t* orig, int32_t* out_coords, void* workspace, size_t workspace_bytes, void* stream);
+int pcgc_set_topk_fused(int on);
+int pcgc_topk_fused_enabled(void);
+size_t pcgc_topk_fused_state_bytes(void);
+size_t pcgc_topk_fused_hist0_offset(void);
+size_t pcgc_topk_select_hist0_workspace_bytes(int64_t n);
+int pcgc_topk_select_hist0(const float* logits , int ld, int64_t n, int64_t k,
+                           const int32_t* coords, const int32_t* parent_coords, int32_t parent_stride,
+                           uint8_t* bits, int32_t* wprefix, int32_t* orig, int32_t* out_coords,
+                           void* state, size_t state_bytes, void* workspace, size_t workspace_bytes, void* stream);
+int pcgc_cls_child_hist(const int32_t* parent_nbr, int64_t n_parent, const float* in, int Cin, int in_ld, const float* table,
+                        int64_t table_bytes, const float* bias, float* out, int out_ld, uint32_t* hist0, void* stream);
+int pcgc_cls_child_q4_hist(const int32_t* parent_nbr, int64_t n_parent, const float* in, int Cin, int in_ld, const float* table,
+                           int64_t table_bytes, const float* bias, float* out, uint32_t* hist0, void* stream);
 int pcgc_kmap_k3_prune_sel(const int32_t* cand_nbr , int64_t n_cand, const uint8_t* bits, const int32_t* wprefix,
                            const int32_t* orig , int64_t n_out, int32_t* nbr , void* stream);
 int pcgc_kmap_k3_prune_parent_sel(const int32_t* parent_nbr , int64_t n_parent, const uint8_t* bits, const int32_t* wprefix,
diff --git a/pcgcv2_amd/_build.py b/pcgcv2_amd/_build.py
--- a/pcgcv2_amd/_build.py
+++ b/pcgcv2_amd/_build.py
@@ -10,7 +10,7 @@
 LIB = os.path.join(HERE, 'libpcgc_hip' + ('_' + VARIANT if VARIANT else '') + '.so')
 SOURCES = ['coords.hip', 'select.hip', 'conv.hip', 'child_conv.hip', 'child_conv32.hip', 'child_cls_w.hip', 'child_irn.hip', 'child_irn_a16.hip', 'child_irn_b16.hip',
            'child_irn_a32.hip', 'child_irn_b32.hip', 'child_q4.hip', 'rows_irn.hip', 'rows_q4.hip', 'conv_packed.hip', 'entropy.hip', 'loss.hip', 'grad.hip', 'metric.hip', 'colour.hip', 'normals.hip', 'mesh.hip', 'collate.hip', 'hostcodec.cpp', 'ply.cpp', 'mesh_io.cpp']
-HEADERS = [os.path.join(CSRC, 'pcgc_common.h'), os.path.join(CSRC, 'mfma_util.h'), os.path.join(CSRC, 'child_kernels.h'), os.path.join(CSRC, 'child_q4.h'), os.path.join(CSRC, 'q4x.h'), os.path.join(CSRC, 'q4x_sched.h'), os.path.join(CSRC, 'rows_q4_policy.h'), os.path.join(CSRC, 'eb_logits.h'), os.path.join(HERE, '..', 'include', 'pcgc_hip.h')]
+HEADERS = [os.path.join(CSRC, 'pcgc_common.h'), os.path.join(CSRC, 'mfma_util.h'), os.path.join(CSRC, 'child_kernels.h'), os.path.join(CSRC, 'child_q4.h'), os.path.join(CSRC, 'q4x.h'), os.path.join(CSRC, 'q4x_sched.h'), os.path.join(CSRC, 'rows_q4_policy.h'), os.path.join(CSRC, 'eb_logits.h'), os.path.join(CSRC, 'topk_key.h'), os.path.join(HERE, '..', 'include', 'pcgc_hip.h')]
 FLAGS = ['--offload-arch=gfx950', '-O3', '-std=c++17', '-ffp-contract=off', '-fPIC', '-Wall', '-Wno-unused-result'] + \
         os.environ.get('PCGC_EXTRA_HIPCC_FLAGS', '').split()
 
diff --git a/pcgcv2_amd/_lib.py b/pcgcv2_amd/_lib.py
--- a/pcgcv2_amd/_lib.py
+++ b/pcgcv2_amd/_lib.py
@@ -63,6 +63,14 @@
     'pcgc_topk_mask_segments': (ci, [vp, ci, ci, vp, vp, vp, vp, sz, vp]),
     'pcgc_topk_select_workspace_bytes': (sz, [i64]),
     'pcgc_topk_select': (ci, [vp, ci, ci, vp, vp, vp, vp, i32, vp, vp, vp, vp, vp, sz, vp]),
+    'pcgc_set_topk_fused': (ci, [ci]),
+    'pcgc_topk_fused_enabled': (ci, []),
+    'pcgc_topk_fused_state_bytes': (sz, []),
+    'pcgc_topk_fused_hist0_offset': (sz, []),
+    'pcgc_topk_select_hist0_workspace_bytes': (sz, [i64]),
+    'pcgc_topk_select_hist0': (ci, [vp, ci, i64, i64, vp, vp, i32, vp, vp, vp, vp, vp, sz, vp, sz, vp]),
+    'pcgc_cls_child_hist': (ci, [vp, i64, vp, ci, ci, vp, i64, vp, vp, ci, vp, vp]),
+    'pcgc_cls_child_q4_hist': (ci, [vp, i64, vp, ci, ci, vp, i64, vp, vp, vp, vp]),
     'pcgc_kmap_k3_prune_sel': (ci, [vp, i64, vp, vp, vp, i64, vp, vp]),
     'pcgc_kmap_k3_prune_parent_sel': (ci, [vp, i64, vp, vp, vp, i64, vp, vp]),
     'pcgc_gather_rows_f32_ld': (ci, [vp, ci, ci, vp, i64, vp, vp]),
diff --git a/pcgcv2_amd/autoencoder.py b/pcgcv2_amd/autoencoder.py
--- a/pcgcv2_amd/autoencoder.py
+++ b/pcgcv2_amd/autoencoder.py
@@ -102,11 +102,13 @@
         if dispatch.select('prune', (data.F.shape[1],), len(data_cls)).family != 'select':
             mask = ops.topk_mask(data_cls.F, keep[0]) if len(nums) == 1 else ops.topk_mask_segments(data_cls.F, rows, keep)
             return self.pruning(data, mask, n_keep=sum(keep), keep_per_item=None if len(nums) == 1 else keep)
+        state = getattr(data_cls, '_topk_state', None)
         if cand._C is None and cand.origin is not None and cand.origin[0] == 'children':
             parent = cand.origin[1]
-            bits, wprefix, orig, coords = ops.topk_select(data_cls.F, rows, keep, parent_coords=parent.C, parent_stride=parent.stride)
+            bits, wprefix, orig, coords = ops.topk_select(data_cls.F, rows, keep, parent_coords=parent.C, parent_stride=parent.stride,
+                                                          topk_state=state)
         else:
-            bits, wprefix, orig, coords = ops.topk_select(data_cls.F, rows, keep, coords=cand.C)
+            bits, wprefix, orig, coords = ops.topk_select(data_cls.F, rows, keep, coords=cand.C, topk_state=state)
         cmap = CoordMap(coords, cand.stride, unique=True, origin=('selected', cand, bits, wprefix, orig))
         if len(nums) > 1:
             cmap._batch_rows = list(keep)
@@ -128,13 +130,22 @@
         mask = isin_mask(cand.C, ground_truth, or_mask=topk)
         return self.pruning(data, mask)
 
+    def _topk_state(self, device):
+        key = (device, torch.cuda.current_stream(device).cuda_stream)
+        states = self.__dict__.setdefault('_topk_states', {})
+        if key not in states:
+            states[key] = ops.topk_fused_state(device)
+        return states[key]
+
     def forward(self, x, nums_list, ground_truth_list=(None, None, None), training=False):
         out, cls_list = x, []
         for l in range(3):
             out = getattr(self, f'up{l}')(out, relu=True)
             out = getattr(self, f'conv{l}')(out, relu=True)
             out = getattr(self, f'block{l}')(out)
-            cls = getattr(self, f'conv{l}_cls')(out)
+            fused = (not training and len(nums_list[l]) == 1 and out.F.is_cuda and ops.topk_fused_on()
+                     and dispatch.select('prune', (out.F.shape[1],), len(out)).family == 'select')
+            cls = getattr(self, f'conv{l}_cls')(out, topk_state=self._topk_state(out.F.device) if fused else None)
             cls_list.append(cls)
             out = self.prune_voxel(out, cls, nums_list[l], ground_truth_list[l], training)
         return cls_list, out
diff --git a/pcgcv2_amd/csrc/child_cls_w.hip b/pcgcv2_amd/csrc/child_cls_w.hip
--- a/pcgcv2_amd/csrc/child_cls_w.hip
+++ b/pcgcv2_amd/csrc/child_cls_w.hip
@@ -4,4 +4,8 @@
                                        int table_bytes, const ChildEpi& ep, hipStream_t s)
 DEF_CONV_LAUNCH(pcgc_child_cls32) { return launch_child_cls<2, 16, 4>(parent_nbr, n_parent, in, in_ld, table, table_bytes, ep, s); }
 DEF_CONV_LAUNCH(pcgc_child_cls64) { return launch_child_cls<4, 7, 4>(parent_nbr, n_parent, in, in_ld, table, table_bytes, ep, s); }
+#define DEF_CLS_HIST_LAUNCH(NAME) int NAME(const int32_t* parent_nbr, int64_t n_parent, const float* in, int in_ld, const float* table, \
+                                           int table_bytes, const ChildEpi& ep, hipStream_t s, uint32_t* hist0)
+DEF_CLS_HIST_LAUNCH(pcgc_child_cls32_hist) { return launch_child_cls<2, 16, 4, 1, 16, true>(parent_nbr, n_parent, in, in_ld, table, table_bytes, ep, s, hist0); }
+DEF_CLS_HIST_LAUNCH(pcgc_child_cls64_hist) { return launch_child_cls<4, 7, 4, 1, 16, true>(parent_nbr, n_parent, in, in_ld, table, table_bytes, ep, s, hist0); }
 CHILD_TIMING_READER(pcgc_child_timing_cls_w)
diff --git a/pcgcv2_amd/csrc/child_conv.hip b/pcgcv2_amd/csrc/child_conv.hip
--- a/pcgcv2_amd/csrc/child_conv.hip
+++ b/pcgcv2_amd/csrc/child_conv.hip
@@ -4,6 +4,9 @@
 #define DECL_CONV_LAUNCH(NAME) int NAME(const int32_t* parent_nbr, int64_t n_parent, const float* in, int in_ld, const float* table, \
                                         int table_bytes, const ChildEpi& ep, hipStream_t s)
 DECL_CONV_LAUNCH(pcgc_child_conv32); DECL_CONV_LAUNCH(pcgc_child_cls32); DECL_CONV_LAUNCH(pcgc_child_cls64);
+#define DECL_CLS_HIST_LAUNCH(NAME) int NAME(const int32_t* parent_nbr, int64_t n_parent, const float* in, int in_ld, const float* table, \
+                                            int table_bytes, const ChildEpi& ep, hipStream_t s, uint32_t* hist0)
+DECL_CLS_HIST_LAUNCH(pcgc_child_cls32_hist); DECL_CLS_HIST_LAUNCH(pcgc_child_cls64_hist);
 
 
 extern "C" int pcgc_conv_child(const int32_t* parent_nbr, int64_t n_parent, const float* in, int Cin, int in_ld,
@@ -42,6 +45,23 @@
 }
 
 
+extern "C" int pcgc_cls_child_hist(const int32_t* parent_nbr, int64_t n_parent, const float* in, int Cin, int in_ld,
+                                   const float* table, int64_t table_bytes, const float* bias, float* out, int out_ld,
+                                   uint32_t* hist0, void* stream) {
+    if (!hist0 || !pcgc_topk_fused_enabled())
+        return pcgc_conv_child(parent_nbr, n_parent, in, Cin, in_ld, table, table_bytes, bias, nullptr, 0, 0, out, 1, out_ld, stream);
+    CHILD_COMMON_CHECKS(in_ld)
+    PCGC_REQUIRE(out != nullptr, "null output");
+    PCGC_REQUIRE(Cin == 32 || Cin == 64, "the heads with a histogram epilogue serve C = 32 and 64");
+    PCGC_REQUIRE(table_bytes == (int64_t)(125 * ((Cin / 16) * 64 + 16) + 1023) / 1024 * 1024, "cls table size");
+    ChildEpi ep{bias, nullptr, 0, 0, out, out_ld, 0};
+    const int rc = Cin == 64 ? pcgc_child_cls64_hist(parent_nbr, n_parent, in, in_ld, table, (int)table_bytes, ep, S(stream), hist0)
+                             : pcgc_child_cls32_hist(parent_nbr, n_parent, in, in_ld, table, (int)table_bytes, ep, S(stream), hist0);
+    if (rc) return rc;
+    PCGC_CHECK_LAUNCH("cls_child_hist");
+    return 0;
+}
+
 #ifdef PCGC_CHILD_TIMING
 extern "C" int pcgc_child_timing(unsigned long long* out8, int reset) {
     hipDeviceSynchronize();
diff --git a/pcgcv2_amd/csrc/child_kernels.h b/pcgcv2_amd/csrc/child_kernels.h
--- a/pcgcv2_amd/csrc/child_kernels.h
+++ b/pcgcv2_amd/csrc/child_kernels.h
@@ -1,6 +1,7 @@
 #pragma once
 #include "pcgc_common.h"
 #include "mfma_util.h"
+#include "topk_key.h"
 #include <type_traits>
 
 #ifdef PCGC_CHILD_TIMING
@@ -533,12 +534,14 @@
     CHILD_TFLUSH;
 }
 
-template <int NB, int NW, int D, int MT = 1>
+template <int NB, int NW, int D, int MT = 1, bool HIST = false>
 __global__ void __launch_bounds__(NW * 64)
 k_child_cls(const int32_t* __restrict__ pnbr, int64_t n_p, const float* __restrict__ in, int in_ld,
-            const float* __restrict__ table, int table_bytes, ChildEpi ep) {
+            const float* __restrict__ table, int table_bytes, ChildEpi ep, uint32_t* __restrict__ hist0) {
     using V = ClsHead<NB>;
     CHILD_KERNEL_PROLOGUE(V, NW, D, D * NB * 64 * MT)
+    uint32_t* hh = (uint32_t*)(lds_raw + table_bytes + NW * (D * NB * 1024 * MT));
+    if constexpr (HIST) { topk_hist0_zero(hh, threadIdx.x, NW * 64); __syncthreads(); }
     const float bv = ep.bias ? ep.bias[0] : 0.0f;
     const int64_t nunits = (n_p + 16 * MT - 1) / (16 * MT);
     for (int i = 0;; ++i) {
@@ -558,6 +561,7 @@
                     float v = acc[m][0][r];
                     if (ep.bias) v = v + bv;
                     ep.out[(8 * p + mi) * ep.out_ld] = v;
+                    if constexpr (HIST) topk_hist0_count(hh, v);
                 }
             }
         }
@@ -565,6 +569,7 @@
         { CHILD_T(t_dr0); asm volatile("s_waitcnt vmcnt(0)" ::: "memory"); CHILD_T(t_it1); CHILD_TADD(5, t_dr0, t_it1); CHILD_TADD(4, t_it0, t_it1); }
 #endif
     }
+    if constexpr (HIST) { __syncthreads(); topk_hist0_flush(hh, hist0, threadIdx.x, NW * 64); }
     CHILD_TFLUSH;
 }
 
@@ -775,15 +780,15 @@
                             const ChildEpi& ep, hipStream_t s) {
     CHILD_LAUNCH_EX((k_child_conv<NB, NT, NW, D, true, 1, false>), NW, D * NB * 1024, ep, 1, 2);
 }
-template <int NB, int NW, int D, int MT = 1, int WPC = 16>
+template <int NB, int NW, int D, int MT = 1, int WPC = 16, bool HIST = false>
 int launch_child_cls(const int32_t* pnbr, int64_t n_p, const float* in, int in_ld, const float* table, int table_bytes,
-                     const ChildEpi& ep, hipStream_t s) {
-    const size_t lds = (size_t)table_bytes + (size_t)NW * (D * NB * 1024 * MT);
-    auto kern = k_child_cls<NB, NW, D, MT>;
+                     const ChildEpi& ep, hipStream_t s, uint32_t* hist0 = nullptr) {
+    const size_t lds = (size_t)table_bytes + (size_t)NW * (D * NB * 1024 * MT) + (HIST ? TOPK_HIST0_BYTES : 0);
+    auto kern = k_child_cls<NB, NW, D, MT, HIST>;
     static ChildLdsGrant granted;
     if (int rc = child_lds_limit(kern, lds, granted)) return rc;
     const int64_t units = (n_p + 16 * MT - 1) / (16 * MT);
-    hipLaunchKernelGGL(kern, dim3(child_grid_units(units, NW, lds, WPC)), dim3(NW * 64), lds, s, pnbr, n_p, in, in_ld, table, table_bytes, ep);
+    hipLaunchKernelGGL(kern, dim3(child_grid_units(units, NW, lds, WPC)), dim3(NW * 64), lds, s, pnbr, n_p, in, in_ld, table, table_bytes, ep, hist0);
     return 0;
 }
 template <int C, int NW, int D, int MT = 1>
diff --git a/pcgcv2_amd/csrc/child_q4.h b/pcgcv2_amd/csrc/child_q4.h
--- a/pcgcv2_amd/csrc/child_q4.h
+++ b/pcgcv2_amd/csrc/child_q4.h
@@ -58,10 +58,11 @@
     __builtin_amdgcn_raw_buffer_store_b128(u, rs, (int)voff, 0, Q4_STORE_AUX);
 }
 
-template <int KIND, int NW, int MT, int D = 2>
+template <int KIND, int NW, int MT, int D = 2, bool HIST = false>
 __global__ void __launch_bounds__(NW * 64)
 k_child_q4(const int32_t* __restrict__ pnbr, int64_t n_p, const float* __restrict__ in, int in_ld,
-           const float* __restrict__ table, int table_bytes, IrnEpi ep) {
+           const float* __restrict__ table, int table_bytes, IrnEpi ep, uint32_t* __restrict__ hist0) {
+    static_assert(!HIST || KIND == Q4_CLS, "the histogram epilogue belongs to the classification head");
     constexpr int TP = 64 * MT, SLOT_F4 = MT * 256;
     constexpr Q4Sched S = q4_sched<KIND, MT, D>();
     constexpr int NACC = KIND == Q4_CLS ? 2 : 8, OUT_ROW_BYTES = KIND == Q4_CLS ? 4 : 32;
@@ -69,6 +70,8 @@
     const int lane = threadIdx.x & 63;
     const int wave = __builtin_amdgcn_readfirstlane(threadIdx.x >> 6);
     float4* ring = (float4*)(lds_raw + table_bytes) + wave * (D * SLOT_F4);
+    uint32_t* hh = (uint32_t*)(lds_raw + table_bytes + NW * (D * MT * 4096));
+    if constexpr (HIST) topk_hist0_zero(hh, threadIdx.x, NW * 64);
     child_stage_table<NW>(table, table_bytes, lds_raw);
     const __amdgpu_buffer_rsrc_t rs_in = __builtin_amdgcn_make_buffer_rsrc((void*)in, 0, (int)(8 * n_p * in_ld * 4), 0x00020000);
     const __amdgpu_buffer_rsrc_t rs_out = __builtin_amdgcn_make_buffer_rsrc((void*)ep.out, 0, (int)(8 * n_p * OUT_ROW_BYTES), 0x00020000);
@@ -267,6 +270,12 @@
 #else
                     q4_store(v, rs_out, ov + (unsigned)(h * 16));
 #endif
+                    if constexpr (HIST) {
+                        if (p_base + 64 * m + lane < n_p) {
+#pragma unroll
+                            for (int r = 0; r < 4; ++r) topk_hist0_count(hh, v[r]);
+                        }
+                    }
                 }
             });
         }
@@ -274,17 +283,18 @@
         q4_store(sink, rs_out, ovq(0));
 #endif
     }
-}
-
-template <int KIND, int NW, int MT, int D = 2>
+    if constexpr (HIST) { __syncthreads(); topk_hist0_flush(hh, hist0, threadIdx.x, NW * 64); }
+}
+
+template <int KIND, int NW, int MT, int D = 2, bool HIST = false>
 int launch_child_q4(const int32_t* pnbr, int64_t n_p, const float* in, int in_ld, const float* table, int table_bytes,
-                    const IrnEpi& ep, hipStream_t s) {
-    const size_t lds = (size_t)table_bytes + (size_t)NW * (D * MT * 4096);
-    auto kern = k_child_q4<KIND, NW, MT, D>;
+                    const IrnEpi& ep, hipStream_t s, uint32_t* hist0 = nullptr) {
+    const size_t lds = (size_t)table_bytes + (size_t)NW * (D * MT * 4096) + (HIST ? TOPK_HIST0_BYTES : 0);
+    auto kern = k_child_q4<KIND, NW, MT, D, HIST>;
     static ChildLdsGrant granted;
     if (int rc = child_lds_limit(kern, lds, granted)) return rc;
     const int64_t units = (n_p + 64 * MT - 1) / (64 * MT);
-    hipLaunchKernelGGL(kern, dim3(child_grid_units(units, NW, lds)), dim3(NW * 64), lds, s, pnbr, n_p, in, in_ld, table, table_bytes, ep);
+    hipLaunchKernelGGL(kern, dim3(child_grid_units(units, NW, lds)), dim3(NW * 64), lds, s, pnbr, n_p, in, in_ld, table, table_bytes, ep, hist0);
     return 0;
 }
 
diff --git a/pcgcv2_amd/csrc/child_q4.hip b/pcgcv2_amd/csrc/child_q4.hip
--- a/pcgcv2_amd/csrc/child_q4.hip
+++ b/pcgcv2_amd/csrc/child_q4.hip
@@ -26,15 +26,24 @@
     return 0;
 }
 
-extern "C" int pcgc_cls_child_q4(const int32_t* parent_nbr, int64_t n_parent, const float* in, int Cin, int in_ld,
-                                 const float* table, int64_t table_bytes, const float* bias, float* out, void* stream) {
+static int cls_child_q4(const int32_t* parent_nbr, int64_t n_parent, const float* in, int Cin, int in_ld,
+                        const float* table, int64_t table_bytes, const float* bias, float* out, uint32_t* hist0, void* stream) {
     CHILD_COMMON_CHECKS(in_ld)
     PCGC_REQUIRE(Cin == 16, "the quad-block classification head serves C = 16");
     PCGC_REQUIRE(out && (((uintptr_t)out) & 15) == 0, "the output must be 16-byte aligned");
     PCGC_REQUIRE(table_bytes == 96 * 64 * 4, "cls table size");
     IrnEpi ep{bias, nullptr, nullptr, nullptr, 0, out, 1};
-    const int rc = launch_child_q4<Q4_CLS, 8, 2>(parent_nbr, n_parent, in, in_ld, table, (int)table_bytes, ep, S(stream));
+    const int rc = hist0 ? launch_child_q4<Q4_CLS, 8, 2, 2, true>(parent_nbr, n_parent, in, in_ld, table, (int)table_bytes, ep, S(stream), hist0)
+                         : launch_child_q4<Q4_CLS, 8, 2>(parent_nbr, n_parent, in, in_ld, table, (int)table_bytes, ep, S(stream));
     if (rc) return rc;
     PCGC_CHECK_LAUNCH("cls_child_q4");
     return 0;
 }
+extern "C" int pcgc_cls_child_q4(const int32_t* parent_nbr, int64_t n_parent, const float* in, int Cin, int in_ld,
+                                 const float* table, int64_t table_bytes, const float* bias, float* out, void* stream) {
+    return cls_child_q4(parent_nbr, n_parent, in, Cin, in_ld, table, table_bytes, bias, out, nullptr, stream);
+}
+extern "C" int pcgc_cls_child_q4_hist(const int32_t* parent_nbr, int64_t n_parent, const float* in, int Cin, int in_ld,
+                                      const float* table, int64_t table_bytes, const float* bias, float* out, uint32_t* hist0, void* stream) {
+    return cls_child_q4(parent_nbr, n_parent, in, Cin, in_ld, table, table_bytes, bias, out, pcgc_topk_fused_enabled() ? hist0 : nullptr, stream);
+}
diff --git a/pcgcv2_amd/csrc/select.hip b/pcgcv2_amd/csrc/select.hip
--- a/pcgcv2_amd/csrc/select.hip
+++ b/pcgcv2_amd/csrc/select.hip
@@ -1,6 +1,7 @@
 #include <algorithm>
 #include <cstring>
 #include "pcgc_common.h"
+#include "topk_key.h"
 #include <rocprim/rocprim.hpp>
 
 constexpr int SCAN_TILE = 2048;
@@ -150,14 +151,6 @@
 constexpr int TOPK_MAX_SEGS = 16;
 struct TopkSegs { int n; long long off[TOPK_MAX_SEGS + 1]; long long k[TOPK_MAX_SEGS]; };
 
-__device__ static inline uint32_t order_key(float f) {
-    f = f + 0.0f;
-    uint32_t b = __float_as_uint(f);
-    return (b & 0x80000000u) ? ~b : (b | 0x80000000u);
-}
-constexpr int TOPK_PASSES = 3, TOPK_BINS = 2048;
-__host__ __device__ static inline int topk_shift(int pass) { return pass == 0 ? 21 : (pass == 1 ? 10 : 0); }
-__host__ __device__ static inline int topk_bits(int pass) { return pass == 2 ? 10 : 11; }
 __global__ void __launch_bounds__(256) k_topk_init(TopkState* st, uint32_t* hist, TopkSegs segs, unsigned long long* scan_ws, int64_t scan_words, uint32_t* any_tie) {
     const int y = blockIdx.x;
     if (threadIdx.x == 0) { st[y].prefix = 0; st[y].tie = 0; st[y].k_remaining = segs.k[y]; st[y].done = 0; st[y].count_eq = 0; }
@@ -167,13 +160,166 @@
         for (int64_t i = threadIdx.x; i < scan_words; i += blockDim.x) scan_ws[i] = 0;
     }
 }
+__device__ static inline bool topk_pick_digit(const uint32_t (&mine)[TOPK_BINS / 256], int PER, int64_t need, int64_t* S ,
+                                              int& d_out, uint32_t& cnt_out, int64_t& rem_out) {
+    const int t = threadIdx.x;
+    const bool own = t < 256;
+    int64_t gsum = 0;
+#pragma unroll
+    for (int e = 0; e < TOPK_BINS / 256; ++e) gsum += (own && e < PER) ? mine[e] : 0u;
+    if (own) S[t] = gsum;
+    if (t == 0) S[256] = 0;
+    __syncthreads();
+    for (int off = 1; off < 256; off <<= 1) {
+        const int64_t add = (own && t + off < 256) ? S[t + off] : 0;
+        __syncthreads();
+        if (own) S[t] += add;
+        __syncthreads();
+    }
+    const bool group_hit = own && (t == 0 ? (S[1] < need) : (S[t] >= need && (S[t + 1] < need || t == 255)));
+    if (group_hit) {
+        int64_t above = S[t + 1];
+        int d = t * PER;
+        uint32_t cnt = mine[0];
+        bool found = false;
+#pragma unroll
+        for (int e = TOPK_BINS / 256 - 1; e >= 0; --e) {
+            if (e < PER && !found) {
+                if (above + mine[e] >= need || (t == 0 && e == 0)) { d = t * PER + e; cnt = mine[e]; found = true; }
+                else above += mine[e];
+            }
+        }
+        d_out = d; cnt_out = cnt; rem_out = need - above;
+    }
+    __syncthreads();
+    return group_hit;
+}
+
+constexpr uint32_t TOPK_CAND_CAP = 32768;
+struct TopkFused { uint32_t count0; uint32_t cand_count; };
+struct TopkFusedArgs { TopkFused* fu; uint32_t* hist0; const uint32_t* cand; };
+
+__global__ void __launch_bounds__(256) k_topk_pick0(const float* __restrict__ v, int ld, int64_t n, int64_t k, const uint32_t* __restrict__ hist0,
+                                                    TopkState* st, uint32_t* any_tie, TopkFused* fu, uint32_t* __restrict__ cand,
+                                                    unsigned long long* scan_ws, int64_t scan_words) {
+    __shared__ int64_t S[257];
+    __shared__ uint32_t d_s, cnt_s;
+    const int t = threadIdx.x, lane = t & 63;
+    const int64_t step = (int64_t)gridDim.x * blockDim.x;
+    for (int64_t i = (int64_t)blockIdx.x * blockDim.x + t; i < scan_words; i += step) scan_ws[i] = 0;
+    uint32_t mine[TOPK_BINS / 256];
+#pragma unroll
+    for (int e = 0; e < TOPK_BINS / 256; ++e) mine[e] = hist0[t * (TOPK_BINS / 256) + e];
+    int d; uint32_t cnt; int64_t rem;
+    if (topk_pick_digit(mine, TOPK_BINS / 256, k, S, d, cnt, rem)) {
+        d_s = (uint32_t)d; cnt_s = cnt;
+        if (blockIdx.x == 0) {
+            st->prefix = (uint32_t)d << topk_shift(0); st->tie = 0; st->k_remaining = rem; st->done = 0; st->count_eq = 0;
+            *any_tie = 0;
+            fu->count0 = cnt;
+        }
+    }
+    __syncthreads();
+    if (cnt_s > TOPK_CAND_CAP) return;
+    const uint32_t d0 = d_s;
+    const unsigned long long lt = (1ull << lane) - 1ull;
+    int64_t i = (int64_t)blockIdx.x * blockDim.x + t;
+    for (; i + 7 * step < n; i += 8 * step) {
+        float f[8];
+#pragma unroll
+        for (int u = 0; u < 8; ++u) f[u] = v[(i + u * step) * ld];
+        uint32_t key[8];
+        unsigned long long bal[8];
+        uint32_t total = 0;
+#pragma unroll
+        for (int u = 0; u < 8; ++u) { key[u] = order_key(f[u]); bal[u] = __ballot((key[u] >> topk_shift(0)) == d0); total += (uint32_t)__popcll(bal[u]); }
+        if (total) {
+            const int leader = (int)__ffsll((long long)__ballot(1)) - 1;
+            uint32_t base = 0;
+            if (lane == leader) base = atomicAdd(&fu->cand_count, total);
+            base = __shfl(base, leader, 64);
+#pragma unroll
+            for (int u = 0; u < 8; ++u) {
+                const uint32_t slot = base + (uint32_t)__popcll(bal[u] & lt);
+                if (((bal[u] >> lane) & 1ull) && slot < TOPK_CAND_CAP) cand[slot] = key[u];
+                base += (uint32_t)__popcll(bal[u]);
+            }
+        }
+    }
+    for (; i < n; i += step) {
+        const uint32_t key = order_key(v[i * ld]);
+        const bool m = (key >> topk_shift(0)) == d0;
+        const unsigned long long bal = __ballot(m);
+        if (bal) {
+            const int leader = (int)__ffsll((long long)bal) - 1;
+            uint32_t base = 0;
+            if (lane == leader) base = atomicAdd(&fu->cand_count, (uint32_t)__popcll(bal));
+            base = __shfl(base, leader, 64);
+            const uint32_t slot = base + (uint32_t)__popcll(bal & lt);
+            if (m && slot < TOPK_CAND_CAP) cand[slot] = key;
+        }
+    }
+}
+__device__ static void topk_finish_block(const TopkFusedArgs fa, TopkState* st, uint32_t* any_tie, uint32_t* h , int64_t* S) {
+    __shared__ uint32_t prefix_s, cnt_s;
+    __shared__ int64_t need_s;
+    const int t = threadIdx.x;
+    uint32_t nc = fa.fu->count0 < fa.fu->cand_count ? fa.fu->count0 : fa.fu->cand_count;
+    if (nc > TOPK_CAND_CAP) nc = TOPK_CAND_CAP;
+    uint32_t prefix = st->prefix;
+    int64_t need = st->k_remaining;
+    uint32_t cnt = 0;
+    __syncthreads();
+    for (int b = t; b < TOPK_BINS; b += 256) fa.hist0[b] = 0;
+    if (t == 0) fa.fu->cand_count = 0;
+    const uint4* __restrict__ c4 = (const uint4*)fa.cand;
+    for (int pass = 1; pass < TOPK_PASSES; ++pass) {
+        const int shift = topk_shift(pass), nb = 1 << topk_bits(pass), PER = nb >> 8;
+        const uint32_t dmask = (uint32_t)nb - 1u, pmask = 0xFFFFFFFFu << (shift + topk_bits(pass));
+        for (int b = t; b < nb; b += 256) h[b] = 0;
+        __syncthreads();
+        for (uint32_t i = t; i < nc / 4; i += 256) {
+            const uint4 q = c4[i];
+            if ((q.x & pmask) == prefix) atomicAdd(&h[(q.x >> shift) & dmask], 1u);
+            if ((q.y & pmask) == prefix) atomicAdd(&h[(q.y >> shift) & dmask], 1u);
+            if ((q.z & pmask) == prefix) atomicAdd(&h[(q.z >> shift) & dmask], 1u);
+            if ((q.w & pmask) == prefix) atomicAdd(&h[(q.w >> shift) & dmask], 1u);
+        }
+        for (uint32_t i = (nc & ~3u) + t; i < nc; i += 256) {
+            const uint32_t key = fa.cand[i];
+            if ((key & pmask) == prefix) atomicAdd(&h[(key >> shift) & dmask], 1u);
+        }
+        __syncthreads();
+        uint32_t mine[TOPK_BINS / 256];
+#pragma unroll
+        for (int e = 0; e < TOPK_BINS / 256; ++e) mine[e] = e < PER ? h[t * PER + e] : 0u;
+        int d; uint32_t c; int64_t rem;
+        if (topk_pick_digit(mine, PER, need, S, d, c, rem)) { prefix_s = prefix | ((uint32_t)d << shift); need_s = rem; cnt_s = c; }
+        __syncthreads();
+        prefix = prefix_s; need = need_s; cnt = cnt_s;
+        __syncthreads();
+    }
+    if (t == 0) {
+        st->prefix = prefix; st->k_remaining = need; st->done = 0;
+        st->count_eq = cnt;
+        st->tie = need < (int64_t)cnt ? 1u : 0u;
+        *any_tie = need < (int64_t)cnt ? 1u : 0u;
+    }
+}
+
 __global__ void __launch_bounds__(256) k_topk_hist(const float* __restrict__ v_all, int ld, TopkSegs segs, TopkState* st_all,
-                                                   int pass, uint32_t* hist_all, uint32_t* any_tie) {
+                                                   int pass, uint32_t* hist_all, uint32_t* any_tie, TopkFusedArgs fa) {
     __shared__ uint32_t h[TOPK_BINS];
     __shared__ int64_t S[257];
     __shared__ bool last_s;
-    __shared__ int pick_s;
     const int t = threadIdx.x, y = blockIdx.y;
+    if (fa.fu) {
+        if (fa.fu->count0 <= TOPK_CAND_CAP) {
+            if (pass == 1 && blockIdx.x == 0) topk_finish_block(fa, st_all, any_tie, h, S);
+            return;
+        }
+        if (pass == 1 && blockIdx.x == 0) for (int b = t; b < TOPK_BINS; b += 256) fa.hist0[b] = 0;
+    }
     const float* __restrict__ v = v_all + segs.off[y] * ld;
     const int64_t n = segs.off[y + 1] - segs.off[y];
     TopkState* st = st_all + y;
@@ -210,37 +356,12 @@
     if (!last_s) return;
     const int PER = nb >> 8;
     uint32_t mine[TOPK_BINS / 256];
-    int64_t gsum = 0;
-#pragma unroll
-    for (int e = 0; e < TOPK_BINS / 256; ++e) {
+#pragma unroll
+    for (int e = 0; e < TOPK_BINS / 256; ++e)
         mine[e] = e < PER ? __hip_atomic_load(&hist[t * PER + e], __ATOMIC_RELAXED, __HIP_MEMORY_SCOPE_AGENT) : 0u;
-        gsum += mine[e];
-    }
-    S[t] = gsum;
-    if (t == 0) { S[256] = 0; pick_s = -1; }
-    __syncthreads();
-    for (int off = 1; off < 256; off <<= 1) {
-        const int64_t add = t + off < 256 ? S[t + off] : 0;
-        __syncthreads();
-        S[t] += add;
-        __syncthreads();
-    }
     const int64_t need = st->k_remaining;
-    __syncthreads();
-    const bool group_hit = t == 0 ? (S[1] < need) : (S[t] >= need && (S[t + 1] < need || t == 255));
-    if (group_hit) {
-        int64_t above = S[t + 1];
-        int d = t * PER;
-        uint32_t cnt = mine[0];
-        bool found = false;
-#pragma unroll
-        for (int e = TOPK_BINS / 256 - 1; e >= 0; --e) {
-            if (e < PER && !found) {
-                if (above + mine[e] >= need || (t == 0 && e == 0)) { d = t * PER + e; cnt = mine[e]; found = true; }
-                else above += mine[e];
-            }
-        }
-        const int64_t rem = need - above;
+    int d; uint32_t cnt; int64_t rem;
+    if (topk_pick_digit(mine, PER, need, S, d, cnt, rem)) {
         st->prefix = prefix | ((uint32_t)d << shift);
         st->k_remaining = rem;
         st->done = 0;
@@ -304,7 +425,7 @@
     hipLaunchKernelGGL(k_topk_init, dim3(segs.n), dim3(256), 0, S(stream), st, hist, segs, (unsigned long long*)scan_ws,
                        (int64_t)(pcgc_scan_workspace_bytes(n) / 8), any_tie);
     for (int pass = 0; pass < TOPK_PASSES; ++pass)
-        hipLaunchKernelGGL(k_topk_hist, dim3(g, segs.n), dim3(256), 0, S(stream), logits, ld, segs, st, pass, hist, any_tie);
+        hipLaunchKernelGGL(k_topk_hist, dim3(g, segs.n), dim3(256), 0, S(stream), logits, ld, segs, st, pass, hist, any_tie, TopkFusedArgs{nullptr, nullptr, nullptr});
     hipLaunchKernelGGL(k_topk_mask, dim3(grid_for(nmax, 256), segs.n), dim3(256), 0, S(stream), logits, ld, segs, st, mask, eq);
     launch_scan(eq, n, rank, total, scan_ws, any_tie, S(stream));
     hipLaunchKernelGGL(k_topk_tie_fix, dim3(grid_for(nmax, 256), segs.n), dim3(256), 0, S(stream), st, segs, eq, rank, g_topk_tie_high, mask);
@@ -482,11 +603,55 @@
     unsigned g = grid_for(nmax, 256 * 8); if (g > 256) g = 256; if (g < 1) g = 1;
     hipLaunchKernelGGL(k_topk_init, dim3(nseg), dim3(256), 0, S(stream), st, hist, segs, desc, (int64_t)(pcgc_scan_workspace_bytes(n) / 8), any_tie);
     for (int pass = 0; pass < TOPK_PASSES; ++pass)
-        hipLaunchKernelGGL(k_topk_hist, dim3(g, nseg), dim3(256), 0, S(stream), logits, ld, segs, st, pass, hist, any_tie);
+        hipLaunchKernelGGL(k_topk_hist, dim3(g, nseg), dim3(256), 0, S(stream), logits, ld, segs, st, pass, hist, any_tie, TopkFusedArgs{nullptr, nullptr, nullptr});
     hipLaunchKernelGGL(k_topk_select, dim3((unsigned)tiles), dim3(256), 0, S(stream), logits, ld, segs, st, (const int4*)coords,
                        (const int4*)parent_coords, parent_stride / 2, g_topk_tie_high, n, tiles, desc, (int32_t*)(desc + tiles),
                        bits, wprefix, orig, (int4*)out_coords);
     PCGC_CHECK_LAUNCH("topk_select");
+    return 0;
+}
+static int g_topk_fused = 1;
+extern "C" int pcgc_set_topk_fused(int on) { g_topk_fused = on ? 1 : 0; return 0; }
+extern "C" int pcgc_topk_fused_enabled(void) { return g_topk_fused; }
+constexpr size_t TOPK_FUSED_COUNTERS = 512, TOPK_FUSED_HIST = 1024, TOPK_FUSED_HIST0 = TOPK_FUSED_HIST + TOPK_BINS * 4,
+                 TOPK_FUSED_CAND = TOPK_FUSED_HIST0 + TOPK_BINS * 4;
+extern "C" size_t pcgc_topk_fused_state_bytes(void) { return TOPK_FUSED_CAND + (size_t)TOPK_CAND_CAP * 4; }
+extern "C" size_t pcgc_topk_fused_hist0_offset(void) { return TOPK_FUSED_HIST0; }
+extern "C" size_t pcgc_topk_select_hist0_workspace_bytes(int64_t n) { return pcgc_topk_select_workspace_bytes(n); }
+extern "C" int pcgc_topk_select_hist0(const float* logits, int ld, int64_t n, int64_t k,
+                                      const int32_t* coords, const int32_t* parent_coords, int32_t parent_stride,
+                                      uint8_t* bits, int32_t* wprefix, int32_t* orig, int32_t* out_coords,
+                                      void* state, size_t state_bytes, void* workspace, size_t workspace_bytes, void* stream) {
+    if (!g_topk_fused)
+        return pcgc_topk_select(logits, ld, 1, &n, &k, coords, parent_coords, parent_stride, bits, wprefix, orig, out_coords, workspace,
+                                workspace_bytes, stream);
+    PCGC_REQUIRE(n >= 0 && n < (1ll << 31), "too many rows");
+    PCGC_REQUIRE((coords != nullptr) != (parent_coords != nullptr), "exactly one of coords / parent_coords");
+    PCGC_REQUIRE(!parent_coords || (parent_stride >= 2 && (parent_stride & 1) == 0), "parent stride must be even");
+    PCGC_REQUIRE(!parent_coords || (n & 7) == 0, "a children level has 8 rows per parent");
+    PCGC_REQUIRE(state && ((uintptr_t)state & 15) == 0 && state_bytes >= pcgc_topk_fused_state_bytes(), "state too small or unaligned");
+    PCGC_REQUIRE(((uintptr_t)bits & 7) == 0 && ((uintptr_t)workspace & 7) == 0, "bits and workspace must be 8-byte aligned");
+    PCGC_REQUIRE(workspace_bytes >= align256(pcgc_scan_workspace_bytes(n)), "workspace too small");
+    if (n == 0) return 0;
+    TopkSegs segs{};
+    segs.n = 1; segs.off[0] = 0; segs.off[1] = n; segs.k[0] = k < 0 ? 0 : (k > n ? n : k);
+    char* sp = (char*)state;
+    TopkState* st = (TopkState*)sp;
+    uint32_t* any_tie = (uint32_t*)(sp + 768);
+    uint32_t* hist = (uint32_t*)(sp + TOPK_FUSED_HIST);
+    uint32_t* cand = (uint32_t*)(sp + TOPK_FUSED_CAND);
+    const TopkFusedArgs fa{(TopkFused*)(sp + TOPK_FUSED_COUNTERS), (uint32_t*)(sp + TOPK_FUSED_HIST0), cand};
+    unsigned long long* desc = (unsigned long long*)workspace;
+    const int64_t tiles = scan_tiles(n);
+    unsigned g = grid_for(n, 256 * 8); if (g > 256) g = 256; if (g < 1) g = 1;
+    hipLaunchKernelGGL(k_topk_pick0, dim3(g), dim3(256), 0, S(stream), logits, ld, n, (int64_t)segs.k[0], fa.hist0, st, any_tie, fa.fu, cand,
+                       desc, (int64_t)(pcgc_scan_workspace_bytes(n) / 8));
+    for (int pass = 1; pass < TOPK_PASSES; ++pass)
+        hipLaunchKernelGGL(k_topk_hist, dim3(g, 1), dim3(256), 0, S(stream), logits, ld, segs, st, pass, hist, any_tie, fa);
+    hipLaunchKernelGGL(k_topk_select, dim3((unsigned)tiles), dim3(256), 0, S(stream), logits, ld, segs, st, (const int4*)coords,
+                       (const int4*)parent_coords, parent_stride / 2, g_topk_tie_high, n, tiles, desc, (int32_t*)(desc + tiles),
+                       bits, wprefix, orig, (int4*)out_coords);
+    PCGC_CHECK_LAUNCH("topk_select_hist0");
     return 0;
 }
 __global__ void k_gather_rows_f32x4(const float* __restrict__ in, int C4, int in_ld, const int32_t* __restrict__ orig, int64_t n_out,
diff --git a/pcgcv2_amd/csrc/topk_key.h b/pcgcv2_amd/csrc/topk_key.h
--- /dev/null
+++ b/pcgcv2_amd/csrc/topk_key.h
@@ -0,0 +1,22 @@
+#pragma once
+#include <hip/hip_runtime.h>
+#include <cstdint>
+
+__device__ static inline uint32_t order_key(float f) {
+    f = f + 0.0f;
+    uint32_t b = __float_as_uint(f);
+    return (b & 0x80000000u) ? ~b : (b | 0x80000000u);
+}
+constexpr int TOPK_PASSES = 3, TOPK_BINS = 2048;
+__host__ __device__ static inline int topk_shift(int pass) { return pass == 0 ? 21 : (pass == 1 ? 10 : 0); }
+__host__ __device__ static inline int topk_bits(int pass) { return pass == 2 ? 10 : 11; }
+
+constexpr int TOPK_HIST0_BYTES = TOPK_BINS * 4;
+__device__ __forceinline__ void topk_hist0_zero(uint32_t* h, int tid, int nthreads) {
+    for (int b = tid; b < TOPK_BINS; b += nthreads) h[b] = 0;
+}
+__device__ __forceinline__ void topk_hist0_count(uint32_t* h, float logit) { atomicAdd(&h[order_key(logit) >> topk_shift(0)], 1u); }
+__device__ __forceinline__ void topk_hist0_flush(const uint32_t* h, uint32_t* __restrict__ hist0, int tid, int nthreads) {
+    for (int b = tid; b < TOPK_BINS; b += nthreads) { const uint32_t c = h[b]; if (c) atomicAdd(&hist0[b], c); }
+}
+extern "C" int pcgc_topk_fused_enabled(void);
diff --git a/pcgcv2_amd/dispatch.py b/pcgcv2_amd/dispatch.py
--- a/pcgcv2_amd/dispatch.py
+++ b/pcgcv2_amd/dispatch.py
@@ -36,7 +36,7 @@
          'tile = 16 coarse rows walking the 8 child offsets: 121 -> ~65 us for the three down convs of a vox10 frame (rows = COARSE rows)'),
     Rule('down', None, None, 0, INF, None, 'gather', 'pcgc_conv_gather, K = 8', 'other shapes / tiny levels'),
     Rule('conv1', None, None, 0, INF, None, 'gather', 'pcgc_conv_gather, K = 1 (k_conv_gather_valu)', 'k1 convs outside fused blocks'),
-    Rule('prune', (8, 16, 32, 64), None, 0, INF, 'ONE_SWEEP_PRUNE', 'select', 'k_topk_init + 3 x k_topk_hist + k_topk_select',
+    Rule('prune', (8, 16, 32, 64), None, 0, INF, 'ONE_SWEEP_PRUNE', 'select', 'k_topk_init + 3 x k_topk_hist + k_topk_select; one cloud behind a head with a histogram epilogue: k_topk_pick0 + 2 x k_topk_hist + k_topk_select',
          'thresholds by radix select, then ONE scan writes coordinates, survivor rows and a rank bitmap: 10 -> 5 launches per decoder stage'),
     Rule('prune', None, None, 0, INF, None, 'mask', 'pcgc_topk_mask(_segments) + pcgc_mask_scan + pcgc_compact_*', 'byte mask + int32 prefix per row'),
     Rule('up', None, None, 0, INF, None, 'up2', 'k_conv_up2_mfma<64,32> / <32,16>, k_conv_up2_rows otherwise', 'generative transpose, one kernel per shape'),
diff --git a/pcgcv2_amd/nn.py b/pcgcv2_amd/nn.py
--- a/pcgcv2_amd/nn.py
+++ b/pcgcv2_amd/nn.py
@@ -27,7 +27,7 @@
 
 class MinkowskiConvolution(_ConvBase):
 
-    def forward(self, x, relu=False, out=None, residual=None):
+    def forward(self, x, relu=False, out=None, residual=None, topk_state=None):
         k, s = self.kernel_size, self.stride
         cin, cout = self.in_channels, self.out_channels
         plain_out = out is None and residual is None
@@ -37,11 +37,13 @@
                                   unit_input=cin == 1 and x.has_unit_features(), plain_output=plain_out).family
             if fam == 'child':
                 if cout == 1 and cin == 16 and ops.PATH.CHILD_Q4 and plain_out and not relu and x.F.shape[0] >= 8 * ops.PATH.CHILD_Q4_MIN_PARENTS:
-                    y = ops.cls_child_q4(x.cmap.origin[1].k3, x.F, self._table(ops.child_q4_cls_table), self.bias)
-                    return SparseTensor(y, coordinate_map=x.cmap)
+                    y = ops.cls_child_q4(x.cmap.origin[1].k3, x.F, self._table(ops.child_q4_cls_table), self.bias, topk_state=topk_state)
+                    return self._head_output(y, x.cmap, topk_state)
                 table = self._table(ops.child_cls_table if cout == 1 else ops.child_conv_table)
-                y = ops.conv_child(x.cmap.origin[1].k3, x.F, table, self.bias, cout, out=out, residual=residual, relu=relu)
-                return SparseTensor(y, coordinate_map=x.cmap)
+                if not (cout == 1 and cin in (32, 64) and plain_out and not relu):
+                    topk_state = None
+                y = ops.conv_child(x.cmap.origin[1].k3, x.F, table, self.bias, cout, out=out, residual=residual, relu=relu, topk_state=topk_state)
+                return self._head_output(y, x.cmap, topk_state)
             if fam == 'unit':
                 cm = x.cmap
                 if cm.mapless_unit_conv() and cout in (4, 8, 16) and not ops.PROFILE.counting:
@@ -69,6 +71,13 @@
             raise NotImplementedError(f'MinkowskiConvolution(kernel_size={k}, stride={s}) is not on the PCGCv2 path')
         y = ops.conv_gather(nbr, x.F, self.kernel, self.bias, out=out, residual=residual, relu=relu)
         return SparseTensor(y, coordinate_map=cmap)
+
+    @staticmethod
+    def _head_output(y, cmap, topk_state):
+        out = SparseTensor(y, coordinate_map=cmap)
+        if topk_state is not None:
+            out._topk_state = topk_state
+        return out
 
     def _table(self, build):
         stamp = (self.kernel.data_ptr(), self.kernel._version)
diff --git a/pcgcv2_amd/ops.py b/pcgcv2_amd/ops.py
--- a/pcgcv2_amd/ops.py
+++ b/pcgcv2_amd/ops.py
@@ -826,7 +826,23 @@
     return _gather_table(_TABLE_INDEX[key], W.detach().reshape(-1))
 
 
-def cls_child_q4(parent_nbr, x, table, bias):
+def set_topk_fused(on):
+    check(lib().pcgc_set_topk_fused(1 if on else 0), 'set_topk_fused')
+
+
+def topk_fused_on():
+    return bool(PATH.TOPK_FUSED) and bool(lib().pcgc_topk_fused_enabled())
+
+
+def topk_fused_state(device):
+    return torch.zeros(int(lib().pcgc_topk_fused_state_bytes()), dtype=torch.uint8, device=device)
+
+
+def _hist0_ptr(state):
+    return None if state is None else state.data_ptr() + int(lib().pcgc_topk_fused_hist0_offset())
+
+
+def cls_child_q4(parent_nbr, x, table, bias, topk_state=None):
     _f32(x, 'x')
     n_p = parent_nbr.shape[1]
     if x.shape[0] != 8 * n_p:
@@ -841,7 +857,11 @@
                                  lambda P, a=Cin: P * a * 4 + P * 8 + n * 4, lambda P, a=Cin: 2 * P * a,
                                  compulsory=n * Cin * 4 + 27 * n_p * 4 + n * 4, mfma_issued=((n_p + 63) // 64) * 96 * 16 * 512)
         e0.record()
-    check(lib().pcgc_cls_child_q4(_p(parent_nbr), n_p, _p(x), Cin, _ld(x), _p(table), table.numel() * 4, _p(bias), _p(out), _stream(x)), 'cls_child_q4')
+    if topk_state is None:
+        check(lib().pcgc_cls_child_q4(_p(parent_nbr), n_p, _p(x), Cin, _ld(x), _p(table), table.numel() * 4, _p(bias), _p(out), _stream(x)), 'cls_child_q4')
+    else:
+        check(lib().pcgc_cls_child_q4_hist(_p(parent_nbr), n_p, _p(x), Cin, _ld(x), _p(table), table.numel() * 4, _p(bias), _p(out),
+                                           _hist0_ptr(topk_state), _stream(x)), 'cls_child_q4_hist')
     if prof:
         e1.record()
     elif PROFILE.counting:
@@ -999,7 +1019,7 @@
     return out
 
 
-def conv_child(parent_nbr, x, table, bias, Cout, out=None, residual=None, relu=False):
+def conv_child(parent_nbr, x, table, bias, Cout, out=None, residual=None, relu=False, topk_state=None):
     _f32(x, 'x')
     n_p = parent_nbr.shape[1]
     if x.shape[0] != 8 * n_p:
@@ -1020,8 +1040,14 @@
                                  compulsory=n * Cin * 4 + 27 * n_p * 4 + n * Cout * 4 + (0 if residual is None else n * Cout * 4),
                                  mfma_issued=tiles * per_tile * 2048)
         e0.record()
-    check(lib().pcgc_conv_child(_p(parent_nbr), n_p, _p(x), Cin, _ld(x), _p(table), table.numel() * 4, _p(bias), res_p, res_ld,
-                                int(relu), _p(out), Cout, _ld(out), _stream(x)), 'conv_child')
+    if topk_state is not None:
+        if Cout != 1 or Cin not in (32, 64) or residual is not None or relu:
+            raise PcgcError('conv_child: the histogram epilogue belongs to the heads 32 -> 1 and 64 -> 1')
+        check(lib().pcgc_cls_child_hist(_p(parent_nbr), n_p, _p(x), Cin, _ld(x), _p(table), table.numel() * 4, _p(bias), _p(out), _ld(out),
+                                        _hist0_ptr(topk_state), _stream(x)), 'cls_child_hist')
+    else:
+        check(lib().pcgc_conv_child(_p(parent_nbr), n_p, _p(x), Cin, _ld(x), _p(table), table.numel() * 4, _p(bias), res_p, res_ld,
+                                    int(relu), _p(out), Cout, _ld(out), _stream(x)), 'conv_child')
     if prof:
         e1.record()
     elif PROFILE.counting:
@@ -1180,11 +1206,13 @@
 
 
 
-def topk_select(logits, seg_rows, seg_k, coords=None, parent_coords=None, parent_stride=0):
+def topk_select(logits, seg_rows, seg_k, coords=None, parent_coords=None, parent_stride=0, topk_state=None):
     _f32(logits, 'logits')
     n = logits.shape[0]
     if sum(seg_rows) != n:
         raise PcgcError(f'topk_select: segments cover {sum(seg_rows)} of {n} rows')
+    if topk_state is not None and len(seg_rows) != 1:
+        raise PcgcError('topk_select: the path behind a head\'s histogram serves one segment')
     if len(seg_rows) > 16:
         raise PcgcError('topk_select: at most 16 segments')
     K = sum(int(min(max(k, 0), r)) for r, k in zip(seg_rows, seg_k))
@@ -1196,6 +1224,12 @@
     out = torch.empty((K, 4), dtype=torch.int32, device=dev)
     ws_bytes = int(lib().pcgc_topk_select_workspace_bytes(n))
     ws = torch.empty(ws_bytes, dtype=torch.uint8, device=dev)
+    if topk_state is not None:
+        check(lib().pcgc_topk_select_hist0(_p(logits), logits.stride(0), n, int(seg_k[0]),
+                                           _p(None if coords is None else _i32(coords)), _p(None if parent_coords is None else _i32(parent_coords)),
+                                           int(parent_stride), _p(bits), _p(wprefix), _p(orig), _p(out), _p(topk_state), topk_state.numel(),
+                                           _p(ws), ws_bytes, _stream(logits)), 'topk_select_hist0')
+        return bits, wprefix, orig, out
     check(lib().pcgc_topk_select(_p(logits), logits.stride(0), len(seg_rows), _i64_array(seg_rows), _i64_array(seg_k),
                                  _p(None if coords is None else _i32(coords)), _p(None if parent_coords is None else _i32(parent_coords)),
                                  int(parent_stride), _p(bits), _p(wprefix), _p(orig), _p(out), _p(ws), ws_bytes, _stream(logits)), 'topk_select')
diff --git a/pcgcv2_amd/pathconfig.py b/pcgcv2_amd/pathconfig.py
--- a/pcgcv2_amd/pathconfig.py
+++ b/pcgcv2_amd/pathconfig.py
@@ -28,6 +28,7 @@
     ROWS_DOWN: bool = True
     ROWS_DOWN_MIN: int = 1024
     ONE_SWEEP_PRUNE: bool = True
+    TOPK_FUSED: bool = True
     D1_CELLS: bool = True
 
     @classmethod
```
